# pablode/gatling

Hardware: AMD Instinct MI355X
Metric: Msamples/s (spp x pixels / s) at 8 bounces, 1920x1080 (higher is better)
Workload: dtype f32; 1 GPU; C2: cornell.usda 1920x1080 spp=1024 max-bounces=8 UsdPreviewSurface (diffuse + GGX specular), NEE off; width=1920, height=1080, spp=1024, max_bounces=8, parallelism=single, triangles=46, bvh8_nodes=4

## Files before the change

gatling_amd/build.py:

```python
from __future__ import annotations

import os
import subprocess
from concurrent.futures import ThreadPoolExecutor

_HERE = os.path.dirname(os.path.abspath(__file__))
CSRC = os.path.join(_HERE, "csrc")
OBJDIR = os.path.join(CSRC, "build")
LIB = os.path.join(_HERE, "libgatling_gi.so")
HOST_SOURCES = ["gi_c.cpp", "gi_scene.cpp", "gi_textures.cpp", "gi_lights.cpp", "gi_build.cpp", "gi_render.cpp", "gi_debug.cpp", "gi_denoise_host.cpp"]
SOURCES = HOST_SOURCES + ["gi_image.cpp", "bvh8.cpp", "leaf_lift.cpp", "gi_kernels.hip", "gi_trace.hip", "gi_shade.hip", "gi_aov.hip", "gi_aov2.hip", "gi_path.hip", "gi_bvh_build.hip", "gi_patch.hip", "gi_refit.hip", "gi_tlas.hip", "gi_blas.hip", "gi_append.hip", "gi_instances.hip", "gi_compact.hip", "gi_tlas_build.hip", "gi_tlas_build_host.cpp", "gi_blas_build.hip", "gi_blas_build_host.cpp", "gi_denoise.hip", "gi_moments.hip", "gi_denoise_var.hip", "gtl_shim.cpp"]
HEADERS = ["gi_host.h", "gi_types.h", "gi_kernels.h", "gi_device_math.h", "gi_queues.h", "gi_traversal.h", "gi_texture.h", "gi_shading.h", "gi_stages.h", "gi_image.h", "gi_options.h", "gi_miss_rect.h", "bvh8.h", "gi_bvh_build.h", "gi_refit.h", "gi_tlas.h", "gi_blas.h", "gi_pack.h", "gi_vispatch.h", "gi_aov_body.h", "gi_append.h", "gi_instances.h", "gi_compact.h", "gi_bvh_stages.h", "gi_tlas_build.h", "gi_blas_build.h", "gi_denoise.h", "gi_moments.h",
           os.path.join("..", "..", "include", "gi_c.h"), os.path.join("..", "..", "include", "gtl", "gi", "Gi.h"),
           os.path.join("..", "..", "include", "gtl", "gb", "ParamTypes.h")]
INCLUDE = os.path.join(_HERE, "..", "include")
FLAGS = ["--offload-arch=gfx950", "-O3", "-std=c++17", "-fPIC", "-ffp-contract=off", "-Wall", "-I", INCLUDE]
KERNEL_FLAGS = ["-fno-slp-vectorize"]


def materialx_include():
    roots = [os.environ.get(k) for k in ("MATERIALX_ROOT", "PXR_USD_LOCATION", "USD_ROOT")] + ["/usr", "/usr/local", "/opt/local"]
    for r in roots:
        if r and os.path.exists(os.path.join(r, "include", "MaterialXFormat", "XmlIo.h")):
            return os.path.join(r, "include")
    return None


def _mtime(path: str) -> float:
    return os.path.getmtime(path) if os.path.exists(path) else 0.0


def _headers_mtime() -> float:
    return max([_mtime(os.path.join(CSRC, h)) for h in HEADERS] + [_mtime(os.path.abspath(__file__))])


def _obj(src: str) -> str:
    return os.path.join(OBJDIR, src + ".o")


def _stale(src: str, force: bool) -> bool:
    return force or _mtime(_obj(src)) < max(_mtime(os.path.join(CSRC, src)), _headers_mtime())


def needs_build() -> bool:
    return _mtime(LIB) == 0.0 or any(_stale(s, False) or _mtime(_obj(s)) > _mtime(LIB) for s in SOURCES)


def build(force: bool = False, verbose: bool = False) -> str:
    if not (force or needs_build()):
        return LIB
    hipcc = os.environ.get("HIPCC", "/opt/rocm/bin/hipcc")
    os.makedirs(OBJDIR, exist_ok=True)

    def compile_one(src: str) -> None:
        cmd = [hipcc] + FLAGS + (KERNEL_FLAGS if src.endswith(".hip") else []) + (["-fvisibility=hidden"] if src in HOST_SOURCES else []) + (["-I", mtlx] if mtlx and src == "gtl_shim_mtlx.cpp" else []) + ["-c", src, "-o", _obj(src)]
        if verbose:
            print(" ".join(cmd))
        subprocess.check_call(cmd, cwd=CSRC)

    sources = list(SOURCES)
    mtlx = materialx_include()
    if mtlx:
        sources.append("gtl_shim_mtlx.cpp")
    todo = [s for s in sources if _stale(s, force)]
    with ThreadPoolExecutor(max_workers=min(len(todo), os.cpu_count() or 2) or 1) as pool:
        list(pool.map(compile_one, todo))
    link = [hipcc, "--offload-arch=gfx950", "-shared", "-fPIC", "-o", LIB] + [_obj(s) for s in sources] + ["-lz"]
    if verbose:
        print(" ".join(link))
    subprocess.check_call(link, cwd=CSRC)
    return LIB


if __name__ == "__main__":
    print(build(force=True, verbose=True))
```

gatling_amd/capi.py:

```python
from __future__ import annotations

import ctypes as C
import os

import numpy as np

from .scene import P_COUNT, SceneDesc, RenderSettings

_HERE = os.path.dirname(os.path.abspath(__file__))
LIB_PATH = os.path.join(_HERE, "libgatling_gi.so")
if os.environ.get("GATLING_GI_LIB"):
    LIB_PATH = os.path.abspath(os.environ["GATLING_GI_LIB"])

GI_C_OK = 0
AOV_COLOR = 0
AOV_EXT_MOMENTS = 0x100
FORMAT_INT32, FORMAT_FLOAT32, FORMAT_FLOAT32_VEC4 = 0, 1, 2
OPTION_COUNT_TRAVERSAL, OPTION_KERNEL_TIMERS, OPTION_POOL_SLOTS, OPTION_SAMPLE_BUFFER_MB, OPTION_TRACE_DYNAMIC, OPTION_TWO_LEVEL, OPTION_FUSED_PATH, OPTION_DEVICES = 1, 2, 3, 4, 5, 6, 7, 8
OPTION_SAMPLE_LOOKAHEAD = 10
OPTION_VERTEX_UPDATES = 12
OPTION_VISIBILITY_UPDATES = 11
OPTION_TOPOLOGY_UPDATES = 13
OPTION_RESYNC_REFITS = 14
OPTION_INSTANCE_UPDATES = 15
# ... 86 lines not shown
                ("scale", C.c_float * 4), ("bias", C.c_float * 4)]


class GiCPrimvarData(C.Structure):
    _fields_ = [("name", C.c_char_p), ("type", C.c_int32), ("interpolation", C.c_int32), ("data", C.c_void_p), ("dataSize", C.c_uint64)]



ASSET_OPEN = C.CFUNCTYPE(C.c_void_p, C.c_void_p, C.c_char_p)
ASSET_SIZE = C.CFUNCTYPE(C.c_uint64, C.c_void_p, C.c_void_p)
ASSET_DATA = C.CFUNCTYPE(C.c_void_p, C.c_void_p, C.c_void_p)
ASSET_CLOSE = C.CFUNCTYPE(None, C.c_void_p, C.c_void_p)


class GiCAssetReader(C.Structure):
    _fields_ = [("user", C.c_void_p), ("open", ASSET_OPEN), ("size", ASSET_SIZE), ("data", ASSET_DATA), ("close", ASSET_CLOSE)]


class GiCDecodedImage(C.Structure):
    _fields_ = [("format", C.c_uint32), ("width", C.c_uint32), ("height", C.c_uint32), ("reserved", C.c_uint32), ("pixels", C.c_void_p), ("handle", C.c_void_p)]


IMAGE_LOAD = C.CFUNCTYPE(C.c_int32, C.c_void_p, C.c_char_p, C.c_void_p, C.c_uint64, C.c_int32, C.POINTER(GiCDecodedImage))
IMAGE_RELEASE = C.CFUNCTYPE(None, C.c_void_p, C.POINTER(GiCDecodedImage))
IMAGE_RGBA8_UNORM, IMAGE_RGB16_FLOAT, IMAGE_RGBA16_FLOAT, IMAGE_R32_FLOAT, IMAGE_RGBA32_FLOAT = 1, 2, 3, 4, 5


class GiCImageLoader(C.Structure):
    _fields_ = [("user", C.c_void_p), ("load", IMAGE_LOAD), ("release", IMAGE_RELEASE)]


SYMBOLS = [
    ("giCInitialize", C.c_int, [C.c_int]), ("giCInitializeDevices", C.c_int, [C.POINTER(C.c_int32), C.c_uint32]), ("giCGetDeviceCount", C.c_uint32, []), ("giCGetApiVersion", C.c_uint32, []), ("giCGetDevicePeerAccess", C.c_int32, [C.c_uint32]), ("giCTerminate", None, []), ("giCGetLastError", C.c_char_p, []),
    ("giCCreateMaterial", _P, [_P, C.c_char_p, C.POINTER(GiCMaterialDesc)]), ("giCDestroyMaterial", None, [_P]),
    ("giCCreateMesh", _P, [_P, C.POINTER(GiCMeshDesc)]), ("giCSetMeshTransform", None, [_P, _FP]),
    ("giCSetMeshInstanceTransforms", None, [_P, _U, _FP]), ("giCSetMeshInstanceIds", None, [_P, _U, C.POINTER(C.c_int32)]),
    ("giCSetMeshMaterial", None, [_P, _P]), ("giCSetMeshVisibility", None, [_P, _I]), ("giCSetMeshVertices", C.c_int, [_P, _U, _P]), ("giCDestroyMesh", None, [_P]),
    ("giCRender", C.c_int, [C.POINTER(GiCRenderParams)]),
    ("giCCreateScene", _P, []), ("giCDestroyScene", None, [_P]),
    ("giCCreateSphereLight", _P, [_P]), ("giCDestroySphereLight", None, [_P, _P]), ("giCSetSphereLightPosition", None, [_P, _FP]),
    ("giCSetSphereLightBaseEmission", None, [_P, _FP]), ("giCSetSphereLightRadius", None, [_P, _F, _F, _F]),
    ("giCSetSphereLightDiffuseSpecular", None, [_P, _F, _F]),
    ("giCCreateDistantLight", _P, [_P]), ("giCDestroyDistantLight", None, [_P, _P]), ("giCSetDistantLightDirection", None, [_P, _FP]),
    ("giCSetDistantLightBaseEmission", None, [_P, _FP]), ("giCSetDistantLightAngle", None, [_P, _F]),
    ("giCSetDistantLightDiffuseSpecular", None, [_P, _F, _F]),
    ("giCCreateRectLight", _P, [_P]), ("giCDestroyRectLight", None, [_P, _P]), ("giCSetRectLightOrigin", None, [_P, _FP]),
    ("giCSetRectLightTangents", None, [_P, _FP, _FP]), ("giCSetRectLightBaseEmission", None, [_P, _FP]),
    ("giCSetRectLightDimensions", None, [_P, _F, _F]), ("giCSetRectLightDiffuseSpecular", None, [_P, _F, _F]),
    ("giCCreateDiskLight", _P, [_P]), ("giCDestroyDiskLight", None, [_P, _P]), ("giCSetDiskLightOrigin", None, [_P, _FP]),
    ("giCSetDiskLightTangents", None, [_P, _FP, _FP]), ("giCSetDiskLightBaseEmission", None, [_P, _FP]),
    ("giCSetDiskLightRadius", None, [_P, _F, _F]), ("giCSetDiskLightDiffuseSpecular", None, [_P, _F, _F]),
    ("giCCreateDomeLight", _P, [_P, C.c_char_p]), ("giCDestroyDomeLight", None, [_P]), ("giCSetDomeLightRotation", None, [_P, _FP]),
    ("giCSetDomeLightBaseEmission", None, [_P, _FP]), ("giCSetDomeLightDiffuseSpecular", None, [_P, _F, _F]),
    ("giCSetDomeLightTexture", None, [_P, _P]),
    ("giCCreateTexture", _P, [_P, C.POINTER(GiCTextureDesc)]), ("giCDestroyTexture", None, [_P]),
    ("giCCreateTextureFromFile", _P, [_P, C.c_char_p, _I]),
    ("giCDebugDecodeImage", C.c_int, [C.c_char_p, _I, C.POINTER(C.c_uint32), C.POINTER(C.c_uint32), _FP, C.c_uint64]),
    ("giCRegisterAssetReader", None, [C.POINTER(GiCAssetReader)]), ("giCSetImageLoader", None, [C.POINTER(GiCImageLoader)]),
    ("giCSetMaterialTexture", C.c_int, [_P, _I, C.POINTER(GiCTextureBinding)]),
    ("giCSetMaterialTextureTransform", C.c_int, [_P, _I, _FP]),
    ("giCSetMeshPrimvars", C.c_int, [_P, _U, C.POINTER(GiCPrimvarData)]), ("giCSetMeshInstancerPrimvars", C.c_int, [_P, _U, C.POINTER(GiCPrimvarData)]),
    ("giCSetMaterialPrimvarInput", C.c_int, [_P, _I, C.c_char_p]),
    ("giCCreateRenderBuffer", _P, [_U, _U, _I]), ("giCDestroyRenderBuffer", None, [_P]), ("giCGetRenderBufferMem", _P, [_P]),
    ("giCGetRenderBufferDeviceMem", _P, [_P]), ("giCSetRenderBufferDeviceOnly", None, [_P, _I]),
    ("giCCreateHostRenderBuffer", _P, [_U, _U, _I]),
    ("giCDenoiseVarianceDefaults", None, [C.POINTER(GiCDenoiseVarianceParams)]), ("giCDenoiseVariance", C.c_int, [C.POINTER(GiCDenoiseVarianceParams)]),
    ("giCDenoiseDefaults", None, [C.POINTER(GiCDenoiseParams)]), ("giCDenoise", C.c_int, [C.POINTER(GiCDenoiseParams)]),
    ("giCGetDenoiseStats", C.c_int, [C.POINTER(GiCDenoiseStats)]),
    ("giCGetRenderStats", C.c_int, [_P, C.POINTER(GiCRenderStats)]), ("giCSetSceneOption", C.c_int, [_P, _I, _I]),
    ("giCGetLookaheadStats", C.c_int, [_P, C.POINTER(GiCLookaheadStats)]),
    ("giCTraceRays", C.c_int, [_P, _U, _FP, _FP, _F, _F, _FP, C.POINTER(C.c_int32)]),
    ("giCDebugEvalBsdf", C.c_int, [C.POINTER(GiCMaterialDesc), _U, _FP, _FP]),
    ("giCDebugShadeClass", C.c_int, [C.POINTER(GiCMaterialDesc)]),
    ("giCDebugCheckSqrt", C.c_int64, [C.c_uint32, C.c_uint64]),
    ("giCDebugCheckDiv", C.c_int64, [C.c_uint32, C.c_uint64, C.c_uint32, C.POINTER(C.c_uint32)]),
    ("giCDebugValidateBvh", C.c_int, [_FP, _U, C.POINTER(C.c_uint32), C.POINTER(C.c_uint32)]),
    ("giCDebugValidatePartitionedBvh", C.c_int, [_FP, _U, _U, C.POINTER(C.c_uint32), C.POINTER(C.c_uint32)]),
    ("giCDebugValidateSceneBvh", C.c_int, [_P, _U, C.POINTER(C.c_uint32), C.POINTER(C.c_uint32), C.POINTER(C.c_int32), C.POINTER(C.c_uint64)]),
    ("giCDebugTexRuntime", C.c_int, [_FP, _U, _U, _U, _U, _FP, _FP]),
    ("giCDebugEditDirtyFlags", C.c_int32, [_I, _I]), ("giCDebugSceneUpdateCounts", C.c_int, [_P, C.POINTER(C.c_uint64)]),
    ("giCDebugSceneVisibilityUpdateCount", C.c_int, [_P, C.POINTER(C.c_uint64)]), ("giCDebugSceneClassState", C.c_int, [_P, C.POINTER(C.c_uint32)]),
    ("giCDebugSceneUpsPlain", C.c_int, [_P, C.POINTER(C.c_uint32)]), ("giCDebugUpsTraits", C.c_int, [C.POINTER(GiCMaterialDesc), _U, C.c_int, C.POINTER(C.c_uint32)]),
    ("giCDebugSceneLeafLift", C.c_int, [_P, C.POINTER(C.c_uint32)]),
    ("giCDebugLeafLift", C.c_int, [_FP, _U, C.c_int32, _P, _U, _U, _P, _U, C.POINTER(C.c_uint32), C.POINTER(C.c_uint32), C.POINTER(C.c_double)]),
    ("giCDebugSceneVertexUpdateCount", C.c_int, [_P, C.POINTER(C.c_uint64)]), ("giCDebugRefitBvh", C.c_int, [_FP, _FP, _U, C.POINTER(C.c_uint32), C.POINTER(C.c_uint32)]),
    ("giCDebugSceneRefitCheck", C.c_int, [_P, _U, C.POINTER(C.c_uint32)]),
    ("giCDebugSceneTopologyUpdateCount", C.c_int, [_P, C.POINTER(C.c_uint64)]),
    ("giCDebugSceneResyncCount", C.c_int, [_P, C.POINTER(C.c_uint64)]), ("giCDebugGatherShade", C.c_int, [_P, _U, _P, _U]),
    ("giCDebugSceneShadeCheck", C.c_int, [_P, _U, C.POINTER(C.c_uint32)]),
    ("giCDebugSceneInstanceUpdateCount", C.c_int, [_P, C.POINTER(C.c_uint64)]), ("giCDebugCloneInstance", C.c_int, [_P, _U, _P, _U, _I, _FP, _FP]),
    ("giCDebugSceneTlasUpdateCount", C.c_int, [_P, C.POINTER(C.c_uint64)]), ("giCDebugSceneTlasCheck", C.c_int, [_P, _U, C.POINTER(C.c_uint32)]),
    ("giCDebugInstanceBounds", C.c_int, [_P, _U, _P, _U, _FP, _U, _FP, C.POINTER(C.c_uint32)]),
    ("giCDebugSceneBlasUpdateCount", C.c_int, [_P, C.POINTER(C.c_uint64)]), ("giCDebugSceneBlasCheck", C.c_int, [_P, _U, C.POINTER(C.c_uint32)]),
    ("giCDebugBlasRefit", C.c_int, [_P, _P, _U, _P, _U, C.POINTER(C.c_uint32), C.POINTER(C.c_uint32)]),
    ("giCDebugBlasRefitHost", C.c_int, [_P, _P, _U, _P, _U, C.POINTER(C.c_uint32), C.POINTER(C.c_uint32)]),
    ("giCDebugSceneTlasVisibilityUpdateCount", C.c_int, [_P, C.POINTER(C.c_uint64)]), ("giCDebugSceneFlatIdCheck", C.c_int, [_P, _U, C.POINTER(C.c_uint32)]),
    ("giCDebugSceneFlatTreeState", C.c_int, [_P, _U, C.POINTER(C.c_uint64)]),
    ("giCDebugSceneTlasTopologyUpdateCount", C.c_int, [_P, C.POINTER(C.c_uint64)]),
    ("giCDebugAppendRecords", C.c_int, [_P, _U, _P, _U, _P, _U, _U, _FP, _U, _U, _U, _U, _U]),
    ("giCDebugAppendRecordsHost", C.c_int, [_P, _U, _P, _U, _P, _U, _U, _FP, _U, _U, _U, _U, _U]),
    ("giCDebugInstanceRecords", C.c_int, [_P, _U, _P, _U]),
    ("giCDebugInstanceRecordsHost", C.c_int, [_P, _U, _P, _U]),
    ("giCDebugSceneTlasInstanceUpdateStats", C.c_int, [_P, C.POINTER(C.c_uint64)]),
    ("giCDebugSceneCompactionCount", C.c_int, [_P, C.POINTER(C.c_uint64)]),
    ("giCDebugCompactRanges", C.c_int, [_U, _P, _U, _P, _U, C.POINTER(C.c_uint32)]),
    ("giCDebugCompactRangesHost", C.c_int, [_U, _P, _U, _P, _U, C.POINTER(C.c_uint32)]),
    ("giCDebugBuildTlasHost", C.c_int, [_FP, _U, _U, _U, C.POINTER(C.c_double)]),
    ("giCDebugBuildTlas", C.c_int, [_FP, _U, _U, _U, C.POINTER(C.c_double)]),
    ("giCDebugBuildBlasHost", C.c_int, [_P, _U, _P, _U, _U, _U, C.POINTER(C.c_double)]),
    ("giCDebugBuildBlas", C.c_int, [_P, _U, _P, _U, _U, _U, C.POINTER(C.c_double)]),
    ("giCDebugSceneBlasBuildStats", C.c_int, [_P, C.POINTER(C.c_uint64)]),
    ("giCDebugSceneTlasBuildStats", C.c_int, [_P, C.POINTER(C.c_uint64)]),
    ("giCDebugPatchVisibilityTwoLevel", C.c_int, [C.POINTER(C.c_uint32), C.POINTER(C.c_uint8), C.POINTER(C.c_uint8), _U, _U, C.POINTER(C.c_uint32)]),
    ("giCDebugPathWalkStats", C.c_int, [_P, C.POINTER(C.c_uint64)]),
    ("giCDebugPathLobeStats", C.c_int, [_P, C.POINTER(C.c_uint64)]),
    ("giCDebugPathRingStats", C.c_int, [_P, C.POINTER(C.c_uint64)]),
    ("giCDebugPathLot", C.c_int, [C.c_uint32, C.c_uint32, C.c_uint32, C.POINTER(C.c_uint32)]),
    ("giCDebugTraversalStackHigh", C.c_int, [_P, C.POINTER(C.c_uint32)]),
    ("giCDebugBvhStackReach", C.c_int, [_FP, _U, _FP, _FP, _U, C.POINTER(C.c_uint32)]),
    ("giCDebugSampleMoments", C.c_int, [_P, _FP, _FP, C.POINTER(C.c_uint32), _FP, _FP]),
    ("giCDebugSampleMomentsHost", C.c_int, [_P, _FP, _FP, C.POINTER(C.c_uint32), _FP, _FP]),
    ("giCDebugMissRect", C.c_int, [_FP, C.POINTER(GiCCameraDesc), C.POINTER(GiCRenderSettings), _U, _U, C.POINTER(C.c_uint32)]),
]

_lib = None


def load_library():
    global _lib
    if _lib is None:
        if not os.path.exists(LIB_PATH):
            raise RuntimeError(f"{LIB_PATH} is missing: build it with `python -c 'import __graft_entry__ as g; g.build()'` "
                               "(hipcc --offload-arch=gfx950); there is no CPU fallback")
        L = C.CDLL(LIB_PATH)
        for name, res, args in SYMBOLS:
            fn = getattr(L, name)
            fn.restype = res
            fn.argtypes = args
        _lib = L
    return _lib


def _fp(values):
    arr = (C.c_float * len(values))(*[float(v) for v in values])
    return arr


class GiError(RuntimeError):
    pass


def denoise_params(**params) -> GiCDenoiseParams:
    p = GiCDenoiseParams()
    load_library().giCDenoiseDefaults(C.byref(p))
    for k, v in params.items():
        if k not in ("iterations", "normalSquarings", "sigmaColor", "sigmaDepth", "backgroundDepth", "albedoFloor", "source"):
            raise TypeError(f"denoise: unknown parameter {k!r}")
        setattr(p, k, v)
    return p


def denoise_stats() -> dict:
    s = GiCDenoiseStats()
    if load_library().giCGetDenoiseStats(C.byref(s)) != GI_C_OK:
        raise GiError("giCGetDenoiseStats failed")
    out = {name: getattr(s, name) for name, _ in GiCDenoiseStats._fields_ if name != "passMs"}
# ... 20 lines not shown

def denoise(color, normal, depth, albedo=None, host_form=False, _moments=None, **params):
    L = load_library()
    color = np.ascontiguousarray(color, np.float32)
    h, w = color.shape[:2]
    arrays = {"color": color, "normal": np.ascontiguousarray(normal, np.float32), "depth": np.ascontiguousarray(depth, np.float32)}
    if albedo is not None:
        arrays["albedo"] = np.ascontiguousarray(albedo, np.float32)
    if _moments is not None:
        arrays["moments"] = np.ascontiguousarray(_moments, np.float32)
    create = L.giCCreateHostRenderBuffer if host_form else L.giCCreateRenderBuffer
    bufs = {}
    try:
        for name, a in list(arrays.items()) + [("output", None)]:
            fmt = FORMAT_FLOAT32 if name == "depth" else FORMAT_FLOAT32_VEC4
            if a is not None and a.shape != ((h, w) if name == "depth" else (h, w, 4)):
                raise ValueError(f"denoise: {name} has shape {a.shape}")
            rb = create(w, h, fmt)
            if not rb:
                raise GiError("render buffer creation failed: " + L.giCGetLastError().decode())
            bufs[name] = rb
            if a is not None and a.nbytes:
                C.memmove(L.giCGetRenderBufferMem(rb), a.ctypes.data, a.nbytes)
        source = DENOISE_SOURCE_HOST_FORM if host_form else DENOISE_SOURCE_HOST
        vp = denoise_variance_params(source=source, **params) if _moments is not None else None
        p = vp.base if vp is not None else denoise_params(source=source, **params)
        p.color, p.normal, p.depth, p.albedo, p.output = bufs["color"], bufs["normal"], bufs["depth"], bufs.get("albedo"), bufs["output"]
        if vp is not None:
            vp.moments = bufs["moments"]
            if L.giCDenoiseVariance(C.byref(vp)) != GI_C_OK:
                raise GiError("giCDenoiseVariance failed: " + L.giCGetLastError().decode())
        elif L.giCDenoise(C.byref(p)) != GI_C_OK:
            raise GiError("giCDenoise failed: " + L.giCGetLastError().decode())
        out = np.empty((h, w, 4), np.float32)
        if out.nbytes:
            C.memmove(out.ctypes.data, L.giCGetRenderBufferMem(bufs["output"]), out.nbytes)
        return out
    finally:
        for rb in bufs.values():
            L.giCDestroyRenderBuffer(rb)


def debug_sample_moments(samples, pixel_major, width, rows, first=0, count=None, prev=None, rect=None, miss_rgb=None, host_only=False):
    L = load_library()
    samples = np.ascontiguousarray(samples, np.float32)
    pixels = int(width) * int(rows)
    S = samples.shape[1] if pixel_major else samples.shape[0]
    assert samples.shape == ((pixels, S, 4) if pixel_major else (S, pixels, 4)), samples.shape
    d = (C.c_uint32 * 6)(int(width), int(rows), S, int(first), int(S - first if count is None else count), int(bool(pixel_major)))
    ptr = lambda a: None if a is None else a.ctypes.data_as(_FP)
    prev_a = None if prev is None else np.ascontiguousarray(prev, np.float32).reshape(pixels, 4)
    rect_a = None if rect is None else (C.c_uint32 * 4)(*[int(v) for v in rect])
    miss_a = None if miss_rgb is None else np.ascontiguousarray(miss_rgb, np.float32)
    out = np.empty((pixels, 4), np.float32)
    fn = L.giCDebugSampleMomentsHost if host_only else L.giCDebugSampleMoments
    if fn(d, ptr(samples), ptr(prev_a), rect_a, ptr(miss_a), ptr(out)) != GI_C_OK:
        raise GiError("giCDebugSampleMoments failed: " + L.giCGetLastError().decode())
    return out


def miss_rect(bounds, camera, rs: "RenderSettings", width: int, height: int):
    L = load_library()
    out = (C.c_uint32 * 4)()
    cam, st = _camera(camera), _settings(rs)
    if L.giCDebugMissRect(_fp(bounds), C.byref(cam), C.byref(st), int(width), int(height), out) != GI_C_OK:
        raise GiError("giCDebugMissRect failed: " + L.giCGetLastError().decode())
    return tuple(int(v) for v in out)


def leaf_lift(tri_verts, mode: int = 1, tree_nodes=None, tree_depth: int = 0) -> dict:
    import numpy as np
    L = load_library()
    v = np.ascontiguousarray(tri_verts, np.float32).reshape(-1, 9)
    given = None if tree_nodes is None else np.ascontiguousarray(np.frombuffer(bytes(tree_nodes), np.uint8)).reshape(-1, 80)
    cap = max(len(v), 1) + 1 if given is None else len(given)
    nodes = np.zeros((cap, 80), np.uint8); order = np.zeros(max(len(v), 1), np.uint32); info = np.zeros(4, np.uint32); cost = np.zeros(2, np.float64)
    rc = L.giCDebugLeafLift(v.ctypes.data_as(_FP), len(v), mode, None if given is None else given.ctypes.data_as(_P), 0 if given is None else len(given), tree_depth,
                            nodes.ctypes.data_as(_P), cap, order.ctypes.data_as(C.POINTER(C.c_uint32)), info.ctypes.data_as(C.POINTER(C.c_uint32)),
                            cost.ctypes.data_as(C.POINTER(C.c_double)))
    if rc < 0:
        raise GiError(f"giCDebugLeafLift failed ({rc})")
    return {"violations": rc, "nodes": nodes[:int(info[0])].copy(), "order": order[:len(v)].copy(), "depth": int(info[1]), "lifted": int(info[2]),
            "active": int(info[3]), "cost_before": float(cost[0]), "cost_after": float(cost[1])}


def bvh_stack_reach(tri_verts, origins, dirs):
    import numpy as np
    L = load_library()
    v = np.ascontiguousarray(tri_verts, np.float32).reshape(-1, 9)
    o = np.ascontiguousarray(origins, np.float32).reshape(-1, 3)
    d = np.ascontiguousarray(dirs, np.float32).reshape(-1, 3)
    assert o.shape == d.shape
    out = np.zeros(2 + len(o), np.uint32)
    if L.giCDebugBvhStackReach(v.ctypes.data_as(_FP), len(v), o.ctypes.data_as(_FP), d.ctypes.data_as(_FP), len(o), out.ctypes.data_as(C.POINTER(C.c_uint32))) != 0:
        raise GiError("giCDebugBvhStackReach failed")
    return int(out[0]), int(out[1]), out[2:].copy()


def debug_gather_shade(vertices, faces) -> int:
    from .scene import VERTEX_DTYPE
    L = load_library()
    v = np.ascontiguousarray(vertices, VERTEX_DTYPE)
    f = np.ascontiguousarray(faces, np.uint32).reshape(-1, 3)
    n = L.giCDebugGatherShade(v.ctypes.data, len(v), f.ctypes.data, len(f))
    if n < 0:
        raise GiError("giCDebugGatherShade refused the mesh")
    return int(n)


def debug_clone_instance(vertices, faces, xform_a, xform_b, left_handed=False) -> int:
    from .scene import VERTEX_DTYPE
    L = load_library()
    v = np.ascontiguousarray(vertices, VERTEX_DTYPE)
    f = np.ascontiguousarray(faces, np.uint32).reshape(-1, 3)
    a, b = (np.ascontiguousarray(x, np.float32).reshape(16) for x in (xform_a, xform_b))
    n = L.giCDebugCloneInstance(v.ctypes.data, len(v), f.ctypes.data, len(f), int(bool(left_handed)), a.ctypes.data_as(_FP), b.ctypes.data_as(_FP))
    if n < 0:
        raise GiError("giCDebugCloneInstance refused the mesh or a transform")
    return int(n)


OPTION_BLAS_DEVICE_BUILD = 23
OPTION_TLAS_COMPACTION = 24
OPTION_LEAF_LIFT = 25
TLAS_BUILD_TOO_DEEP = -2


def debug_build_tlas(boxes, depth_budget=7, radius=16, host_only=False) -> dict:
    L = load_library()
    b = np.ascontiguousarray(boxes, np.float32).reshape(-1, 6)
    out = (C.c_double * 8)()
    fn = L.giCDebugBuildTlasHost if host_only else L.giCDebugBuildTlas
    v = fn(b.ctypes.data_as(_FP), len(b), int(depth_budget), int(radius), out)
    if v < 0 and v != TLAS_BUILD_TOO_DEEP:
        raise GiError("giCDebugBuildTlas failed: " + L.giCGetLastError().decode())
    return {"violations": int(v), "nodes": int(out[0]), "depth": int(out[1]), "passes": int(out[2]), "cost": float(out[3]), "host_cost": float(out[4]),
            "host_waits": int(out[5]), "host_depth": int(out[6]), "active": int(out[7])}


def debug_build_blas(vertices, faces, depth_budget=12, radius=16, host_only=False) -> dict:
    from .scene import VERTEX_DTYPE
    L = load_library()
    v = np.ascontiguousarray(vertices, VERTEX_DTYPE)
    f = np.ascontiguousarray(faces, np.uint32).reshape(-1, 3)
    out = (C.c_double * 16)()
    fn = L.giCDebugBuildBlasHost if host_only else L.giCDebugBuildBlas
    r = fn(v.ctypes.data, len(v), f.ctypes.data, len(f), int(depth_budget), int(radius), out)
    if r < 0 and r != TLAS_BUILD_TOO_DEEP:
        raise GiError("giCDebugBuildBlas failed: " + L.giCGetLastError().decode())
    return {"violations": int(r), "nodes": int(out[0]), "depth": int(out[1]), "passes": int(out[2]), "cost": float(out[3]), "host_cost": float(out[4]),
            "host_waits": int(out[5]), "host_depth": int(out[6]), "active": int(out[7]), "conservative": int(out[8]), "rules": int(out[9]), "levels": int(out[10]),
            "bounds_bytes": int(out[11]), "tlas_records": int(out[12]), "refit_bytes": int(out[13]), "budget": int(out[14]), "differing_bytes": int(out[15])}


def debug_instance_bounds(vertices, faces, xforms):
    from .scene import VERTEX_DTYPE
    L = load_library()
    v = np.ascontiguousarray(vertices, VERTEX_DTYPE)
    f = np.ascontiguousarray(faces, np.uint32).reshape(-1, 3)
    x = np.ascontiguousarray(xforms, np.float32).reshape(-1, 16)
    boxes = np.zeros((len(x), 6), np.float32)
    status = np.zeros(len(x), np.uint32)
    n = L.giCDebugInstanceBounds(v.ctypes.data, len(v), f.ctypes.data, len(f), x.ctypes.data_as(_FP), len(x), boxes.ctypes.data_as(_FP),
                                 status.ctypes.data_as(C.POINTER(C.c_uint32)))
    if n < 0:
        raise GiError("giCDebugInstanceBounds failed: " + L.giCGetLastError().decode())
# ... 454 lines not shown
        else:
            m.primvar_inputs.pop(slot, None)
        if self.L.giCSetMaterialPrimvarInput(self.materials[material_index], int(slot), name.encode() if name else None) != GI_C_OK:
            raise GiError("giCSetMaterialPrimvarInput failed: " + self.L.giCGetLastError().decode())

    def _set_primvars(self, fn, h, pvs):
        arr, keep = (GiCPrimvarData * max(len(pvs), 1))(), []
        for k, pv in enumerate(pvs):
            d = np.ascontiguousarray(pv.data, np.int32 if int(pv.type) >= 4 else np.float32).reshape(-1)
            keep.append(d)
            arr[k] = GiCPrimvarData(pv.name.encode(), int(pv.type), int(pv.interpolation), d.ctypes.data, d.nbytes)
        if fn(h, len(pvs), arr) != GI_C_OK:
            raise GiError("giCSetMesh*Primvars failed: " + self.L.giCGetLastError().decode())

    def set_mesh_primvars(self, mesh_index: int, primvars):
        self.desc.meshes[mesh_index].primvars = list(primvars)
        self._set_primvars(self.L.giCSetMeshPrimvars, self.meshes[mesh_index], list(primvars))

    def set_mesh_instancer_primvars(self, mesh_index: int, primvars):
        self.desc.meshes[mesh_index].instancer_primvars = list(primvars)
        self._set_primvars(self.L.giCSetMeshInstancerPrimvars, self.meshes[mesh_index], list(primvars))

    def set_mesh_visibility(self, mesh_index: int, visible: bool):
        self.desc.meshes[mesh_index].visible = bool(visible)
        self.L.giCSetMeshVisibility(self.meshes[mesh_index], int(bool(visible)))

    def set_mesh_vertices(self, mesh_index: int, vertices):
        from .scene import VERTEX_DTYPE
        v = np.ascontiguousarray(vertices, VERTEX_DTYPE)
        if self.L.giCSetMeshVertices(self.meshes[mesh_index], len(v), v.ctypes.data) != GI_C_OK:
            raise GiError("giCSetMeshVertices failed: " + self.L.giCGetLastError().decode())
        self.desc.meshes[mesh_index].vertices = v.copy()

    def vertex_update_count(self) -> int:
        n = C.c_uint64(0)
        if self.L.giCDebugSceneVertexUpdateCount(self.handle, C.byref(n)) != GI_C_OK:
            raise GiError("giCDebugSceneVertexUpdateCount failed")
        return int(n.value)

    def refit_check(self, device: int = 0) -> dict:
        nodes = C.c_uint32(0)
        v = self.L.giCDebugSceneRefitCheck(self.handle, device, C.byref(nodes))
        if v < 0:
            raise GiError("giCDebugSceneRefitCheck failed: " + self.L.giCGetLastError().decode())
        return {"differing": v, "nodes": nodes.value}

    def shade_check(self, device: int = 0) -> int:
        records = C.c_uint32(0)
        v = self.L.giCDebugSceneShadeCheck(self.handle, device, C.byref(records))
        if v < 0:
            raise GiError("giCDebugSceneShadeCheck failed: " + self.L.giCGetLastError().decode())
        return int(v)

    def resync_count(self) -> int:
        n = C.c_uint64(0)
        if self.L.giCDebugSceneResyncCount(self.handle, C.byref(n)) != GI_C_OK:
            raise GiError("giCDebugSceneResyncCount failed")
        return int(n.value)

    def update_counts(self) -> dict:
        c = (C.c_uint64 * 3)()
        if self.L.giCDebugSceneUpdateCounts(self.handle, c) != GI_C_OK:
            raise GiError("giCDebugSceneUpdateCounts failed")
        return {"full": int(c[0]), "transform": int(c[1]), "material": int(c[2])}

    def visibility_update_count(self) -> int:
        n = C.c_uint64(0)
        if self.L.giCDebugSceneVisibilityUpdateCount(self.handle, C.byref(n)) != GI_C_OK:
            raise GiError("giCDebugSceneVisibilityUpdateCount failed")
        return int(n.value)

    def class_state(self) -> dict:
        c = (C.c_uint32 * 5)()
        if self.L.giCDebugSceneClassState(self.handle, c) != GI_C_OK:
            raise GiError("giCDebugSceneClassState failed")
        return {"classMask": int(c[0]), "classTextured": int(c[1]), "shadeClassMask": int(c[2]), "shadeClassTextured": int(c[3]), "hasCutouts": bool(c[4])}

    def ups_plain(self) -> dict:
        c = (C.c_uint32 * 2)()
        if self.L.giCDebugSceneUpsPlain(self.handle, c) != GI_C_OK:
            raise GiError("giCDebugSceneUpsPlain failed")
        return {"traits": int(c[0]), "launched": int(c[1])}

    def leaf_lift(self) -> dict:
        c = (C.c_uint32 * 2)()
        if self.L.giCDebugSceneLeafLift(self.handle, c) != GI_C_OK:
            raise GiError("giCDebugSceneLeafLift failed")
        return {"lifted": int(c[0]), "depth": int(c[1])}

    def path_walk_stats(self) -> dict:
        c = (C.c_uint64 * 18)()
        if self.L.giCDebugPathWalkStats(self.handle, c) != GI_C_OK:
            raise GiError("giCDebugPathWalkStats failed")
        return {"phaseTrips": int(c[0]), "stepTrips": [int(v) for v in c[1:9]], "stepLanes": [int(v) for v in c[9:17]], "fewLaneSteps": int(c[17])}

    def path_lobe_stats(self) -> dict:
        c = (C.c_uint64 * 9)()
        if self.L.giCDebugPathLobeStats(self.handle, c) != GI_C_OK:
            raise GiError("giCDebugPathLobeStats failed")
        keys = ("shaded", "glossy", "glossyTrips", "liteTrips", "fullTrips", "parked", "adopted", "reruns", "rerunHits")
        return {k: int(v) for k, v in zip(keys, c)}

    def path_ring_stats(self) -> dict:
        c = (C.c_uint64 * 5)()
        if self.L.giCDebugPathRingStats(self.handle, c) != GI_C_OK:
            raise GiError("giCDebugPathRingStats failed")
        keys = ("batches", "pairs", "partialBatches", "flushes", "ballotSteps")
        return {k: int(v) for k, v in zip(keys, c)}

    def traversal_stack_high(self) -> dict:
        c = (C.c_uint32 * 4)()
        if self.L.giCDebugTraversalStackHigh(self.handle, c) != GI_C_OK:
            raise GiError("giCDebugTraversalStackHigh failed")
        return {k: int(v) for k, v in zip(("closest", "shadow", "rows", "spill"), c)}

    def set_option(self, option: int, value: int):
        if self.L.giCSetSceneOption(self.handle, option, value) != GI_C_OK:
            raise GiError("giCSetSceneOption failed")

    def color_buffer(self, width, height):
        key = ("color", width, height)
        if key not in self._buffers:
            rb = self.L.giCCreateRenderBuffer(width, height, FORMAT_FLOAT32_VEC4)
            if not rb:
                raise GiError("giCCreateRenderBuffer failed: " + self.L.giCGetLastError().decode())
            self._buffers[key] = rb
        return self._buffers[key]

    def render(self, settings: RenderSettings, width: int, height: int, rows=None, device_only=False, row_stride=1, copy=True):
        L = self.L
        rb = self.color_buffer(width, height)
        L.giCSetRenderBufferDeviceOnly(rb, int(device_only))
        binding = GiCAovBinding()
        binding.aovId = AOV_COLOR
        clear = np.asarray(settings.clear_color, np.float32)
        C.memmove(binding.clearValue, clear.ctypes.data, 16)
        binding.renderBuffer = rb
        p = GiCRenderParams()
        p.aovBindings = C.pointer(binding)
        p.aovBindingCount = 1
        p.camera = _camera(self.desc.camera)
        p.domeLight = self.dome
        p.renderSettings = _settings(settings)
        p.scene = self.handle
        r0, r1 = rows if rows is not None else (0, height)
        p.rowBegin, p.rowEnd, p.rowStride = r0, r1, row_stride
        if L.giCRender(C.byref(p)) != GI_C_OK:
            raise GiError("giCRender failed: " + L.giCGetLastError().decode())
        if device_only:
            return None
        mem = L.giCGetRenderBufferMem(rb)
        full = np.ctypeslib.as_array(C.cast(mem, C.POINTER(C.c_float)), shape=(height, width, 4))
        return full[r0:r1:row_stride].copy() if copy else full[r0:r1:row_stride]

    AOVS = {"normal": (1, FORMAT_FLOAT32_VEC4), "nee": (2, FORMAT_FLOAT32_VEC4), "barycentrics": (3, FORMAT_FLOAT32_VEC4),
            "texcoords": (4, FORMAT_FLOAT32_VEC4), "bounces": (5, FORMAT_FLOAT32_VEC4), "clockCycles": (6, FORMAT_FLOAT32_VEC4), "opacity": (7, FORMAT_FLOAT32_VEC4),
            "tangents": (8, FORMAT_FLOAT32_VEC4), "bitangents": (9, FORMAT_FLOAT32_VEC4), "thinWalled": (10, FORMAT_FLOAT32_VEC4),
            "objectId": (11, FORMAT_INT32), "depth": (12, FORMAT_FLOAT32), "faceId": (13, FORMAT_INT32), "instanceId": (14, FORMAT_INT32),
            "doubleSided": (15, FORMAT_FLOAT32_VEC4), "albedo": (16, FORMAT_FLOAT32_VEC4),
            "moments": (AOV_EXT_MOMENTS, FORMAT_FLOAT32_VEC4)}

    def render_aovs(self, settings: RenderSettings, width: int, height: int, names, clear_values=None, with_color=True, rows=None, row_stride=1):
        L = self.L
        r0, r1 = rows if rows is not None else (0, height)
        bindings = []
        bufs = {}
# ... 163 lines not shown
```

gatling_amd/csrc/gi_debug.cpp:

```cpp
#include "gi_host.h"
#include "gi_refit.h"
#include "gi_tlas_build.h"
#include "gi_blas.h"
#include "gi_blas_build.h"
#include "gi_bvh_stages.h"
#include "gi_compact.h"
#include "gi_moments.h"
#include "bvh8.h"

static int giCTraceRaysImpl(GiCScene* s, uint32_t count, const float* origins, const float* dirs, float tMin, float tMax, float* outTUV, int32_t* outInstPrim);
extern "C" int giCTraceRays(GiCScene* s, uint32_t count, const float* origins, const float* dirs, float tMin, float tMax, float* outTUV, int32_t* outInstPrim)
{
  try { return giCTraceRaysImpl(s, count, origins, dirs, tMin, tMax, outTUV, outInstPrim); }
  catch (const std::exception& e) { setError(std::string("giCTraceRays: ") + e.what()); return -1; }
}
static int giCTraceRaysImpl(GiCScene* s, uint32_t count, const float* origins, const float* dirs, float tMin, float tMax, float* outTUV, int32_t* outInstPrim)
{
  if (!g_ctx.initialized || !s || (count && (!origins || !dirs || !outTUV || !outInstPrim))) { setError("giCTraceRays: bad arguments"); return -1; }
  if (count == 0) return 0;
  std::lock_guard<std::mutex> guard(s->mutex);
  hipStream_t st = g_ctx.stream;
  if (syncSceneGeometry(s) != GI_C_OK) return -1;
  const bool inLds = sceneFitsLds(s->nodeCount, s->triCount);
  const uint32_t blocks = std::min<uint32_t>((count + 255u) / 256u, (uint32_t)g_ctx.cuCount * (inLds ? 3u : 8u));
  if (ensurePathState(s, count, blocks, blocks) != GI_C_OK) return -1;
  const size_t qn = (size_t)s->queueCap * NSHARD;
  std::vector<uint32_t> qslot(qn, 0u); std::vector<F4> qa(qn), qb(qn);
  Counters c{};
  const uint32_t per = (count + NSHARD - 1u) / NSHARD;
  for (uint32_t k = 0; k < NSHARD; k++) { uint32_t lo = k * per; c.count[Q_TRACE_A][k].v = lo < count ? std::min(per, count - lo) : 0u; }
  for (uint32_t i = 0; i < count; i++) {
    size_t r = (size_t)(i / per) * s->queueCap + (i % per);
    qslot[r] = i;
    qa[r] = F4{origins[3 * i], origins[3 * i + 1], origins[3 * i + 2], tMin};
    qb[r] = F4{dirs[3 * i], dirs[3 * i + 1], dirs[3 * i + 2], tMax};
  }
  if (hipMemcpyAsync(s->qSlot[Q_TRACE_A].ptr, qslot.data(), qn * 4, hipMemcpyHostToDevice, st) != hipSuccess ||
      hipMemcpyAsync(s->qA[Q_TRACE_A].ptr, qa.data(), qn * sizeof(F4), hipMemcpyHostToDevice, st) != hipSuccess ||
      hipMemcpyAsync(s->qB[Q_TRACE_A].ptr, qb.data(), qn * sizeof(F4), hipMemcpyHostToDevice, st) != hipSuccess ||
      hipMemcpyAsync(s->dCounters.ptr, &c, sizeof(c), hipMemcpyHostToDevice, st) != hipSuccess) { setError("giCTraceRays: upload failed"); return -1; }
  if (hipMemsetAsync(s->slots.ptr, 0, (size_t)count * sizeof(Slot), st) != hipSuccess) { setError("giCTraceRays: clearing the slots failed"); return -1; }
  PathState ps{s->slots.ptr, nullptr, 0u, nullptr, 0u, nullptr};
  launchTrace(st, blocks, false, false, makeView(s), ps, makeQueueSet(s), s->dCounters.ptr, Q_TRACE_A, Q_REGEN_B, traceDynRefill(s), blocks, FrameUniforms{},
      nullptr);
  std::vector<TriRec> tris(s->triCount);
  if (hipMemcpyAsync(&c, s->dCounters.ptr, sizeof(c), hipMemcpyDeviceToHost, st) != hipSuccess ||
      (s->triCount && hipMemcpyAsync(tris.data(), s->dTris.ptr, s->triCount * sizeof(TriRec), hipMemcpyDeviceToHost, st) != hipSuccess) ||
      hipStreamSynchronize(st) != hipSuccess) { setError("giCTraceRays: readback failed"); return -1; }
  std::vector<F4> hit(count, F4{tMax, 0.0f, 0.0f, 0.0f});
  for (uint32_t i = 0; i < count; i++) { uint32_t m = 0xffffffffu; memcpy(&hit[i].w, &m, 4); }
  std::vector<uint32_t> hitIdx(qn);
  if (hipMemcpy(qa.data(), s->qA[Q_TRACE_A].ptr, qn * sizeof(F4), hipMemcpyDeviceToHost) != hipSuccess) {
    setError("giCTraceRays: readback failed");
    return -1;
  }
  for (uint32_t klass = 0; klass < MAT_CLASS_COUNT; klass++) {
    if (hipMemcpy(hitIdx.data(), s->qSlot[Q_HIT + klass].ptr, qn * 4, hipMemcpyDeviceToHost) != hipSuccess) {
      setError("giCTraceRays: readback failed");
      return -1;
    }
    for (uint32_t k = 0; k < NSHARD; k++)
      for (uint32_t j = 0; j < c.count[Q_HIT + klass][k].v; j++) {
        const uint32_t ri = hitIdx[(size_t)k * s->queueCap + j] & 0x3fffffffu;
        if (ri < qn && qslot[ri] < count) { F4 h = qa[ri]; uint32_t w; memcpy(&w, &h.w, 4); w &= 0x0fffffffu; memcpy(&h.w, &w, 4); hit[qslot[ri]] = h; }
      }
  }
  int hits = 0;
  for (uint32_t i = 0; i < count; i++) {
    uint32_t tri; memcpy(&tri, &hit[i].w, 4);
    outTUV[3 * i] = hit[i].x; outTUV[3 * i + 1] = hit[i].y; outTUV[3 * i + 2] = hit[i].z;
    if (tri == 0xffffffffu || tri >= s->triCount) { outInstPrim[2 * i] = -1; outInstPrim[2 * i + 1] = -1; }
    else { outInstPrim[2 * i] = (int32_t)tris[tri].instance; outInstPrim[2 * i + 1] = (int32_t)tris[tri].prim; hits++; }
  }
  return hits;
}

static int validateTree(const std::vector<Node8>& nodes, const std::vector<TriRec>& trisArr, uint32_t triCount, const std::vector<uint8_t>* left = nullptr)
{
  int violations = 0;
  std::vector<uint8_t> seen(triCount, 0);
  struct Item { uint32_t node; float lo[3], hi[3]; };
  std::vector<Item> stack;
  Item root; root.node = 0; for (int a = 0; a < 3; a++) { root.lo[a] = -3.0e38f; root.hi[a] = 3.0e38f; }
  stack.push_back(root);
  while (!stack.empty()) {
    Item it = stack.back(); stack.pop_back();
    if (it.node >= nodes.size()) { violations++; continue; }
    const Node8& n = nodes[it.node];
    uint32_t rel = 0;
    for (int s = 0; s < 8; s++) {
// ... 384 lines not shown
extern "C" int giCDebugShadeClass(const GiCMaterialDesc* desc)
{
  if (!desc) return -1;
  MaterialRec m{}; m.klass = desc->klass; m.flags = desc->flags & ~(MAT_FLAG_TEXTURED | MAT_FLAG_OPACITY_TEX); memcpy(m.p, desc->p, sizeof(m.p));
  deriveMaterialConstants(m);
  return (int)shadeClassOf(m);
}

extern "C" int giCDebugEvalBsdf(const GiCMaterialDesc* desc, uint32_t count, const float* in, float* out)
{
  if (!g_ctx.initialized || !desc || (count && (!in || !out))) { setError("giCDebugEvalBsdf: bad arguments"); return GI_C_ERROR; }
  if (count == 0) return GI_C_OK;
  MaterialRec m{}; m.klass = desc->klass; m.flags = desc->flags & ~(MAT_FLAG_TEXTURED | MAT_FLAG_OPACITY_TEX); memcpy(m.p, desc->p, sizeof(m.p));
  deriveMaterialConstants(m);
  const uint32_t shadeClass = shadeClassOf(m);
  MaterialRec* dm = nullptr; float* din = nullptr; float* dout = nullptr;
  hipStream_t st = g_ctx.stream;
  int rc = GI_C_ERROR;
  if (hipMalloc((void**)&dm, sizeof(m)) == hipSuccess && hipMalloc((void**)&din, (size_t)count * 22 * 4) == hipSuccess &&
      hipMalloc((void**)&dout, (size_t)count * 15 * 4) == hipSuccess &&
      hipMemcpyAsync(dm, &m, sizeof(m), hipMemcpyHostToDevice, st) == hipSuccess &&
      hipMemcpyAsync(din, in, (size_t)count * 22 * 4, hipMemcpyHostToDevice, st) == hipSuccess) {
    launchDebugBsdf(st, dm, shadeClass, count, din, dout);
    if (hipMemcpyAsync(out, dout, (size_t)count * 15 * 4, hipMemcpyDeviceToHost, st) == hipSuccess && hipStreamSynchronize(st) == hipSuccess) rc = GI_C_OK;
  }
  if (rc != GI_C_OK) setError("giCDebugEvalBsdf: HIP failure");
  if (dm) (void)hipFree(dm); if (din) (void)hipFree(din); if (dout) (void)hipFree(dout);
  return rc;
}

extern "C" int giCDebugTexRuntime(const float* rgba, uint32_t width, uint32_t height, uint32_t depth, uint32_t count, const float* queries, float* out)
{
  if (!g_ctx.initialized || !rgba || !width || !height || !depth || (count && (!queries || !out))) { setError("giCDebugTexRuntime: bad arguments");
      return GI_C_ERROR; }
  if (count == 0) return GI_C_OK;
  const size_t texFloats = (size_t)width * height * depth * 4;
  float* dt = nullptr; float* dq = nullptr; float* dout = nullptr;
  hipStream_t st = g_ctx.stream;
  int rc = GI_C_ERROR;
  if (hipMalloc((void**)&dt, texFloats * 4) == hipSuccess && hipMalloc((void**)&dq, (size_t)count * 32) == hipSuccess
      && hipMalloc((void**)&dout, (size_t)count * 16) == hipSuccess &&
      hipMemcpyAsync(dt, rgba, texFloats * 4, hipMemcpyHostToDevice, st) == hipSuccess
          && hipMemcpyAsync(dq, queries, (size_t)count * 32, hipMemcpyHostToDevice, st) == hipSuccess) {
    launchDebugTex(st, dt, width, height, depth, count, dq, dout);
    if (hipMemcpyAsync(out, dout, (size_t)count * 16, hipMemcpyDeviceToHost, st) == hipSuccess && hipStreamSynchronize(st) == hipSuccess) rc = GI_C_OK;
  }
  if (rc != GI_C_OK) setError("giCDebugTexRuntime: HIP failure");
  if (dt) (void)hipFree(dt); if (dq) (void)hipFree(dq); if (dout) (void)hipFree(dout);
  return rc;
}


extern "C" int64_t giCDebugCheckSqrt(uint32_t first, uint64_t count)
{
  if (!g_ctx.initialized) { setError("giCDebugCheckSqrt before giCInitialize"); return -1; }
  unsigned long long* d = nullptr; unsigned long long h = 0ull;
  if (hipMalloc(&d, sizeof(h)) != hipSuccess) { setError("giCDebugCheckSqrt: hipMalloc failed"); return -1; }
  bool ok = hipMemsetAsync(d, 0, sizeof(h), g_ctx.stream) == hipSuccess;
  if (ok) { launchDebugSqrt(g_ctx.stream, first, (unsigned long long)count, d); ok = hipMemcpyAsync(&h, d, sizeof(h), hipMemcpyDeviceToHost, g_ctx.stream) == hipSuccess; }
  ok = ok && hipStreamSynchronize(g_ctx.stream) == hipSuccess;
  (void)hipFree(d);
  if (!ok) { setError("giCDebugCheckSqrt: device error"); return -1; }
  return (int64_t)h;
}

extern "C" int64_t giCDebugCheckDiv(uint32_t mode, uint64_t count, uint32_t seed, const uint32_t* words)
{
  if (!g_ctx.initialized) { setError("giCDebugCheckDiv before giCInitialize"); return -1; }
  const bool given = mode == 0u || mode == 2u;
  if (mode > 4u || (given && (!words || count > (1ull << 28)))) { setError("giCDebugCheckDiv: bad arguments"); return -1; }
  const size_t bytes = given ? (size_t)count * (mode == 0u ? 2u : 4u) * sizeof(uint32_t) : 0u;
  unsigned long long* d = nullptr; unsigned long long h = 0ull; uint32_t* dw = nullptr;
  if (hipMalloc(&d, sizeof(h)) != hipSuccess) { setError("giCDebugCheckDiv: hipMalloc failed"); return -1; }
  bool ok = bytes == 0u || hipMalloc(&dw, bytes) == hipSuccess;
  ok = ok && (bytes == 0u || hipMemcpyAsync(dw, words, bytes, hipMemcpyHostToDevice, g_ctx.stream) == hipSuccess);
  ok = ok && hipMemsetAsync(d, 0, sizeof(h), g_ctx.stream) == hipSuccess;
  if (ok) { launchDebugDiv(g_ctx.stream, mode, (unsigned long long)count, seed, dw, d); ok = hipMemcpyAsync(&h, d, sizeof(h), hipMemcpyDeviceToHost, g_ctx.stream) == hipSuccess; }
  ok = ok && hipStreamSynchronize(g_ctx.stream) == hipSuccess;
  (void)hipFree(d); if (dw) (void)hipFree(dw);
  if (!ok) { setError("giCDebugCheckDiv: device error"); return -1; }
  return (int64_t)h;
}

extern "C" int32_t giCDebugEditDirtyFlags(int32_t edit, int32_t built)
{
  std::unique_ptr<GiCScene> scene(new GiCScene());
  GiCScene* s = scene.get();
  const float texel[4] = {1.0f, 1.0f, 1.0f, 1.0f};
  GiCTextureDesc td{1u, 1u, texel};
  GiCMaterialDesc md{}; md.klass = GI_C_MAT_USD_PREVIEW_SURFACE;
  GiCVertex verts[3] = {}; verts[1].pos[0] = 1.0f; verts[2].pos[1] = 1.0f;
  GiCFace face{}; face.v_i[0] = 0; face.v_i[1] = 1; face.v_i[2] = 2;
  GiCMeshDesc meshDesc{}; meshDesc.faceCount = 1; meshDesc.faces = &face; meshDesc.vertexCount = 3; meshDesc.vertices = verts; meshDesc.name = "debug";
  const float identity[16] = {1, 0, 0, 0, 0, 1, 0, 0, 0, 0, 1, 0, 0, 0, 0, 1};
  GiCTexture* tex = giCCreateTexture(s, &td);
  GiCMaterial* matA = giCCreateMaterial(s, "a", &md);
  GiCMaterial* matB = giCCreateMaterial(s, "b", &md);
  GiCMesh* mesh = giCCreateMesh(s, &meshDesc);
  if (!tex || !matA || !matB || !mesh) return -1;
  giCSetMeshInstanceTransforms(mesh, 1, identity);
  giCSetMeshMaterial(mesh, matA);
  if (built) { s->host.reset(new SceneHost()); mesh->builtInstances = 1; }
  s->dirty = 0;
  GiCMaterial* made = nullptr; GiCTexture* madeTex = nullptr; GiCMesh* madeMesh = nullptr;
  GiCTextureBinding binding{}; binding.texture = tex; for (int i = 0; i < 4; i++) binding.scale[i] = 1.0f;
  const float xf[6] = {1, 0, 0, 0, 1, 0};
  const float one = 1.0f; const int32_t id = 7;
  GiCPrimvarData pv{}; pv.name = "k"; pv.type = GI_C_PRIMVAR_FLOAT; pv.interpolation = GI_C_INTERP_CONSTANT; pv.data = &one; pv.dataSize = 4;
  int32_t result = 0;
  switch (edit) {
    case 0: made = giCCreateMaterial(s, "c", &md); break;
    case 1: giCDestroyMaterial(matB); matB = nullptr; break;
    case 2: giCSetMeshMaterial(mesh, matB); break;
    case 3: giCSetMaterialPrimvarInput(matA, GI_C_TEX_BASE_COLOR, "k"); break;
    case 4: giCSetMaterialTexture(matA, GI_C_TEX_BASE_COLOR, &binding); break;
    case 5: giCSetMaterialTextureTransform(matA, GI_C_TEX_BASE_COLOR, xf); break;
    case 6: madeTex = giCCreateTexture(s, &td); break;
    case 7: giCDestroyTexture(tex); tex = nullptr; break;
    case 8: giCSetMeshPrimvars(mesh, 1, &pv); break;
    case 9: giCSetMeshInstancerPrimvars(mesh, 1, &pv); break;
    case 10: giCSetMeshTransform(mesh, identity); break;
    case 11: giCSetMeshVisibility(mesh, 0); break;
    case 12: giCSetMeshInstanceIds(mesh, 1, &id); break;
    case 13: madeMesh = giCCreateMesh(s, &meshDesc); break;
    case 14: giCDestroyMesh(mesh); mesh = nullptr; break;
    case 15: giCSetMeshInstanceTransforms(mesh, 0, nullptr); break;
    case 16: if (giCSetMeshVertices(mesh, 3, verts) != GI_C_OK) result = -1; break;
    default: result = -1; break;
  }
  if (result == 0) result = (int32_t)s->dirty;
  if (madeMesh) giCDestroyMesh(madeMesh);
  if (mesh) giCDestroyMesh(mesh);
  if (made) giCDestroyMaterial(made);
  if (matA) giCDestroyMaterial(matA);
  if (matB) giCDestroyMaterial(matB);
  if (madeTex) giCDestroyTexture(madeTex);
  if (tex) giCDestroyTexture(tex);
  return result;
}

extern "C" int giCDebugSceneUpdateCounts(const GiCScene* scene, uint64_t* outCounts)
{
  GiCScene* s = const_cast<GiCScene*>(scene);
  if (!s || !outCounts) { setError("giCDebugSceneUpdateCounts: bad arguments"); return GI_C_ERROR; }
  std::lock_guard<std::mutex> guard(s->mutex);
  outCounts[0] = s->updateCounts[UPDATE_FULL]; outCounts[1] = s->updateCounts[UPDATE_TRANSFORM]; outCounts[2] = s->updateCounts[UPDATE_MATERIAL];
  return GI_C_OK;
}

extern "C" int giCDebugSceneVisibilityUpdateCount(const GiCScene* scene, uint64_t* outCount)
{
  GiCScene* s = const_cast<GiCScene*>(scene);
  if (!s || !outCount) { setError("giCDebugSceneVisibilityUpdateCount: bad arguments"); return GI_C_ERROR; }
  std::lock_guard<std::mutex> guard(s->mutex);
  *outCount = s->updateCounts[UPDATE_VISIBILITY];
  return GI_C_OK;
}

extern "C" int giCDebugSceneVertexUpdateCount(const GiCScene* scene, uint64_t* outCount)
{
  GiCScene* s = const_cast<GiCScene*>(scene);
  if (!s || !outCount) { setError("giCDebugSceneVertexUpdateCount: bad arguments"); return GI_C_ERROR; }
  std::lock_guard<std::mutex> guard(s->mutex);
  *outCount = s->updateCounts[UPDATE_VERTEX];
  return GI_C_OK;
}
// ... 577 lines not shown
```

gatling_amd/csrc/gi_host.h:

```cpp

#pragma once

#pragma GCC visibility push(default)
#include "../../include/gi_c.h"
#pragma GCC visibility pop


#include <algorithm>
#include <atomic>
#include <chrono>
#include <cmath>
#include <cstdio>
#include <cstdlib>
#include <cstring>
#include <memory>
#include <condition_variable>
#include <functional>
#include <mutex>
#include <string>
#include <thread>
#include <vector>

#include "bvh8.h"
#include "gi_tlas_build.h"
// ... 217 lines not shown
  Counters* hCounters = nullptr;
  uint64_t memTotalMb = 0;
  static constexpr uint32_t POLL_RING = 4, POLL_LAG = 2;
  PaddedCounter* hPoll = nullptr; hipEvent_t pollEvent[POLL_RING] = {};
  hipEvent_t evShade = nullptr, evShadow = nullptr;
  GiCRenderStats stats{};
  uint64_t pathWalkStats[18] = {};
  uint64_t pathLobeStats[9] = {};
  uint64_t pathRingStats[5] = {};
  uint32_t traversalStackHigh[4] = {};
  std::vector<hipEvent_t> eventPool;
  template <typename Fn> void forEachPathBuffer(Fn&& fn)
  {
    fn(slots); fn(media); fn(sampleBuf);
    for (uint32_t q = 0; q < Q_COUNT; q++) { fn(qSlot[q]); fn(qA[q]); fn(qB[q]); fn(qC[q]); }
    fn(qFresh[0]); fn(qFresh[1]);
  }
  uint64_t pathStateBytes() { uint64_t n = 0; forEachPathBuffer([&](auto& b) { n += b.bytes(); }); return n; }
  void releasePathState() { forEachPathBuffer([](auto& b) { b.release(); }); queueCap = 0; lookahead.drop(); }
  void releaseAll();
};

struct TwoLevelHost { std::vector<Node8> tlasNodes, blasNodes; std::vector<uint32_t> tlasItems; std::vector<BlasTri> blasTris; std::vector<InstTrav> instTrav;
    std::vector<float> instBoxes; std::vector<uint32_t> meshBlasTri; uint32_t tlasDepth = 0, blasDepth = 0;
    std::vector<uint32_t> meshBlasNode; std::vector<std::vector<uint32_t>> meshBlasLevels;
    bool tlasDeviceBuilt = false; uint32_t tlasBuildBudget = 0;
    std::vector<uint32_t> meshBlasBudget; };
struct MeshBuild { const GiCMesh* m; uint32_t vertexOffset, matFlags, instFirst, instCount, triFirst; uint32_t meshIdx; std::vector<int32_t> faceIdAov;
    uint32_t shadeBase = 0;
    std::vector<uint32_t> inst; uint32_t retiredInst = 0;
    struct FreeSlot { uint32_t inst, tri; };
    std::vector<uint32_t> instTri; std::vector<FreeSlot> freeSlots;
    void numberInstances() { inst.resize(instCount); instTri.resize(instCount);
        for (uint32_t ii = 0; ii < instCount; ii++) { inst[ii] = instFirst + ii; instTri[ii] = triFirst + ii * (uint32_t)m->faces.size(); } }
    bool hidden = false; uint32_t idBase = 0; };
struct InstPart { uint32_t meshBuild, instInMesh; uint32_t triFirst, nf; uint32_t nodeOff, nodeCount, nodeCap, depth; float box[6];
    uint32_t activeTris = 0; std::vector<uint32_t> levelStart;
    bool retired = false; };
struct SceneHost {
  std::vector<FVertex> verts; std::vector<InstanceRec> instances; std::vector<MaterialRec> mats; std::vector<MeshRec> meshRecs; std::vector<float> sceneData;
  Bvh8 bvh; std::vector<int32_t> triFaceId; std::vector<uint32_t> flatOfOrig; TwoLevelHost two;
  std::vector<MeshBuild> meshBuilds;
  std::vector<F4> triGeomNormal;
  std::vector<TriShade> triShade; bool shadePacked = false;
  bool partitioned = false; std::vector<InstPart> parts; uint32_t topCap = 0;
  bool deviceBuilt = false;
  bool hostTreeDropped = false;
  bool reordered = false;
  bool treeless = false;
};

enum : uint32_t { UPDATE_FULL = 0, UPDATE_TRANSFORM = 1, UPDATE_MATERIAL = 2, UPDATE_VISIBILITY = 3, UPDATE_VERTEX = 4, UPDATE_TOPOLOGY = 5, UPDATE_TLAS = 6, UPDATE_BLAS = 7, UPDATE_TLAS_VISIBILITY = 8, UPDATE_TLAS_TOPOLOGY = 9 };
struct GiCScene : SceneDevice {
  std::mutex mutex;
  uint32_t dirty = DIRTY_ALL;
  std::vector<GiCMesh*> meshes;
  std::vector<GiCMaterial*> materials;
  std::vector<GiCTexture*> textures;
  uint64_t nextTextureSerial = 1;
  DenseStore<SphereLightRec, GiCSphereLight> sphereLights;
  DenseStore<DistantLightRec, GiCDistantLight> distantLights;
  DenseStore<RectLightRec, GiCRectLight> rectLights;
  DenseStore<DiskLightRec, GiCDiskLight> diskLights;
  uint32_t lightCounts[4] = {0, 0, 0, 0};
  uint32_t sampleOffset = 0;
  uint64_t accumEpoch = 0;
  bool haveOldParams = false;
  GiCCameraDesc oldCamera{};
  GiCRenderSettings oldSettings{};
  uint8_t oldClear[GI_C_MAX_AOV_COMP_SIZE] = {0};
  uint32_t oldRowBegin = 0, oldRowEnd = 0, oldRowStride = 1;
  GiCDomeLight* oldDome = nullptr;
  float oldDomeEmission[3] = {0, 0, 0};
  uint32_t nodeCount = 0, triCount = 0, bvhDepth = 0;
  float bounds[6] = {0, 0, 0, 0, 0, 0}; bool boundsValid = false;
  int optBvhBuild = 0;
  bool twoLevel = false; int optTwoLevel = -1;
  bool hasCutouts = false;
  bool shadePacked = false;
  uint32_t classMask = 0;
  uint32_t classTextured = 0;
  uint32_t shadeClassMask = 0, shadeClassTextured = 0;
  uint32_t upsTraits = 0, upsPlainLaunched = 0;
  std::unique_ptr<SceneHost> host;
  std::vector<std::unique_ptr<SceneDevice>> replicas;
  bool countTraversal = false, kernelTimers = false;
  uint32_t kernelTimerStride = 1;
  uint64_t optPoolSlots = 0, optSampleBufferMb = 0;
  int32_t optFusedPath = -1;
  int32_t optTraceDyn = -1;
  std::atomic<int32_t> shadowOrder{-1};
       uint64_t shadowOrderRays[2] = {0, 0},
      shadowOrderSteps[2] = {0, 0};
  int32_t optDevices = 0;
  uint32_t lastRenderDevices = 0;
  int32_t optLookahead = 0;
  uint64_t generation = 0;
  uint64_t updateCounts[10] = {0, 0, 0, 0, 0, 0, 0, 0, 0, 0};
  int32_t optVisibilityUpdates = 0;
  int32_t optVertexUpdates = 0;
  bool rebuildDue = true;
  int32_t optTopologyUpdates = 0;
  bool topologyDue = false;
  int32_t optResyncRefits = 0; uint64_t resyncCount = 0;
  int32_t optInstanceUpdates = 0; uint64_t instanceCounts[4] = {0, 0, 0, 0};
  bool instancesDue = false;
  int32_t optTlasUpdates = 0;
  int32_t optBlasUpdates = 0;
  int32_t optTlasVisibility = 0;
  int32_t optTlasOnly = 0;
  int32_t optTlasTopology = 0;
  int32_t optTlasInstances = 0; uint64_t tlasInstanceCounts[4] = {0, 0, 0, 0};
  int32_t optTlasDeviceBuild = 0; uint64_t tlasBuildStats[16] = {};
  int32_t optBlasDeviceBuild = 0; uint64_t blasBuildStats[16] = {};
  int32_t optTlasCompaction = 0; uint64_t compactionStats[4] = {0, 0, 0, 0};
  int32_t optLeafLift = -1; uint32_t liftedLeafSlots = 0;
  std::vector<GiCMesh*> retiredMeshes;
  ~GiCScene() { for (GiCMesh* m : retiredMeshes) delete m; }
};
inline void raiseRebuild(GiCScene* s) { s->dirty |= DIRTY_BVH | DIRTY_FRAMEBUFFER; s->rebuildDue = true; }
inline void raiseTopology(GiCScene* s) { s->dirty |= DIRTY_BVH | DIRTY_FRAMEBUFFER; s->topologyDue = true; }
inline void raiseInstances(GiCMesh* m) { m->instEdited = true; m->scene->dirty |= DIRTY_BVH | DIRTY_FRAMEBUFFER; m->scene->instancesDue = true; }


extern "C++" bool loadImage(const char* path, bool srgbToLinear, bool keepHdr, uint32_t& w, uint32_t& h, std::vector<float>& px);
int uploadLights(GiCScene* s);
uint32_t shadeClassOf(const MaterialRec& m);
uint32_t upsTraitsOf(const MaterialRec& m);
uint32_t sceneDeviceCount(const GiCScene* s);
SceneDevice& sceneDevice(GiCScene* s, uint32_t slot);
bool usableVertexPositions(const GiCVertex* v, size_t count);
void nodeBounds(const Node8& n, float box[6]);
bool instanceUpdatesWanted(const GiCScene* s);
bool tlasUpdatesWanted(const GiCScene* s);
bool blasUpdatesWanted(const GiCScene* s);
bool leafLiftWanted(const GiCScene* s);
bool tlasOnlyWanted(const GiCScene* s);
bool tlasVisibilityWanted(const GiCScene* s);
bool topologyUpdatesWanted(const GiCScene* s);
bool tlasTopologyWanted(const GiCScene* s);
bool tlasDeviceBuildWanted(const GiCScene* s);
bool blasDeviceBuildWanted(const GiCScene* s);
void buildMeshBlas(const GiCVertex* vertices, const GiCFace* faces, size_t nf, Bvh8& b, std::vector<uint32_t>& order, float mlo[3], float mhi[3]);
BlasTri makeBlasTri(const GiCVertex* vertices, const GiCFace* faces, uint32_t f);
bool tlasCompactionWanted(const GiCScene* s);
bool tlasInstancesWanted(const GiCScene* s);
int syncSceneGeometry(GiCScene* s);
inline uint32_t materialEditFlags(bool built) { return DIRTY_MATERIALS | DIRTY_FRAMEBUFFER | (built ? 0u : (uint32_t)DIRTY_BVH); }
SceneView makeView(GiCScene* s, SceneDevice& D);
SceneView makeView(GiCScene* s);
uint32_t traceDynRefill(const GiCScene* s);
int ensurePathState(SceneDevice* s, size_t slots, uint32_t gridA, uint32_t gridB);
QueueSet makeQueueSet(SceneDevice* s);
```

gatling_amd/csrc/gi_kernels.h:

```cpp
#pragma once

#include <type_traits>
#include <hip/hip_runtime.h>

#include "gi_types.h"
#include "gi_vispatch.h"

namespace gi {

template <class F>
auto dispatchBools(F&& f) { return f(); }
template <class F, class... Bools>
auto dispatchBools(F&& f, bool b, Bools... rest)
{
  return b ? dispatchBools([&](auto... cs) { return f(std::true_type{}, cs...); }, rest...)
           : dispatchBools([&](auto... cs) { return f(std::false_type{}, cs...); }, rest...);
}

void launchInit(hipStream_t s, const PathState& st, const QueueSet& qs, Counters* cnt, uint32_t n, bool resetStats);
void launchRaygen(hipStream_t s, uint32_t blocks, const FrameUniforms& U, const PathState& st, const QueueSet& qs, Counters* cnt, uint32_t par, F4* sampleBuf);
void launchAccumulate(hipStream_t s, const FrameUniforms& U, const F4* sampleBuf, F4* accum, F4* colorOut, bool firstBatch, bool lastBatch);
void launchFoldWindow(hipStream_t s, const FrameUniforms& U, const F4* sampleBuf, F4* colorOut, uint32_t windowSamples, uint32_t first, bool pixelMajor);
bool traceBlockSync(const SceneView& sc);
bool sceneFitsLds(size_t nodeCount, size_t triCount);
uint32_t traceLdsBytes(uint32_t stackEntries, uint32_t ldsNodes, uint32_t ldsTris);
uint32_t blocksPerCuByLds(uint32_t dynamicBytes, uint32_t staticBytes);
uint32_t traceStaticLdsBytes();
void traceLdsLayout(const SceneView& sc, uint32_t& ldsNodes, uint32_t& ldsTris, uint32_t& bytes);
uint32_t traceStackRows(const SceneView& sc, bool& spills);
void launchTrace(hipStream_t s, uint32_t blocks, bool anyHit, bool count, const SceneView& sc, const PathState& st, const QueueSet& qs, Counters* cnt,
                 uint32_t qIn, uint32_t qMiss, uint32_t dynRefill, uint32_t routeBlocks, const FrameUniforms& U, F4* sampleBuf);
void launchRoute(hipStream_t s, uint32_t blocks, const SceneView& sc, const PathState& st, const QueueSet& qs, Counters* cnt, uint32_t qIn, uint32_t qMiss,
    const FrameUniforms& U,
                 F4* sampleBuf);
constexpr uint32_t APPEND_ITEMS_MAX = 4u;
constexpr uint32_t TRACE_DYN_SLOT_ORDER = 0x200u;
void launchShade(hipStream_t s, uint32_t blocks, uint32_t klass, bool textured ,
    bool volume , const FrameUniforms& U, const SceneView& sc, const PathState& st, const QueueSet& qs, Counters* cnt, uint32_t par);

bool pathKernelSupports(const SceneView& sc);
int launchPath(hipStream_t s, uint32_t cuCount, uint32_t classMask, bool textured, bool count, uint32_t chunk, uint32_t walkCarry, uint32_t lobePark,
               uint32_t ringCarry, uint32_t upsTraits, const FrameUniforms& U, const SceneView& sc, const PathState& st, Counters* cnt, F4* sampleBuf);
inline uint32_t pathUpsVariant(uint32_t classMask, bool textured, bool nee, bool cutout, bool count, uint32_t upsTraits)
{
  return (classMask == 2u && !textured && !cutout && !count && !nee) ? upsTraits : 0u;
}
constexpr long UPS_PLAIN_DEFAULT = 1;
constexpr long WALK_CARRY_DEFAULT = 8;
constexpr long LOBE_PARK_DEFAULT = 8;
constexpr long RING_CARRY_DEFAULT = 1;
constexpr long LEAF_LIFT_DEFAULT = 1;
struct PathLot { uint32_t stack, row, capacity; };
inline PathLot pathLotPlacement(uint32_t bvhDepth)
{
  const uint32_t stack = bvhDepth <= 4u ? 4u : 8u;
  const uint32_t row = bvhDepth < stack ? bvhDepth : stack;
  return PathLot{stack, row, (stack - row) * 8u};
}

void launchAov(hipStream_t s, const FrameUniforms& U, const SceneView& sc, const AovTargets& A);
void launchAov2(hipStream_t s, const FrameUniforms& U, const SceneView& sc, const AovTargets& A);
void launchResolveNee(hipStream_t s, const FrameUniforms& U, const unsigned long long* key, F4* aov, uint32_t pixelCount);
void launchZeroClosest(hipStream_t s, Counters* cnt, uint32_t par);
void launchPatchMatFlags(hipStream_t s, TriRec* tris, uint32_t triCount, const InstanceRec* instances, uint32_t instanceCount, const uint32_t* wordOfMesh,
    uint32_t meshCount);
void launchPatchVisibility(hipStream_t s, TriRec* tris, uint32_t triCount, const InstanceRec* instances, uint32_t instanceCount, const VisPatch* patchOfInstance,
    const TriShade* triShade, uint32_t shadeCount);
void launchPatchVisibility2(hipStream_t s, TriRec* tris, uint32_t triCount, const InstanceRec* instances, uint32_t instanceCount, const VisPatch* patchOfInstance,
    const TriShade* triShade, uint32_t shadeCount, uint32_t* flatOfOrig, uint32_t flatCount);
void launchPatchInstTrav(hipStream_t s, InstTrav* instTrav, uint32_t instanceCount, const VisPatch* patchOfInstance);
void launchPlacePart(hipStream_t s, const Node8* partNodes, uint32_t partNodeCount, Node8* nodes, uint32_t nodeOff, TriRec* tris, uint32_t triFirst, uint32_t nf,
    uint32_t idAdd);
struct CloneEntry { uint32_t threadBase, srcTri, dstTri, nf, srcNode, dstNode, nodeCount, instance, idBase; };
inline uint32_t cloneEntryThreads(uint32_t nf, uint32_t nodeCount) { return ((nf > nodeCount ? nf : nodeCount) + 63u) & ~63u; }
void launchCloneParts(hipStream_t s, const CloneEntry* entries, uint32_t entryCount, uint32_t threads, TriRec* tris, uint32_t triCount, int32_t* triFaceId,
    Node8* nodes, uint32_t nodeCount, const InstanceRec* instances, uint32_t instanceCount, const TriShade* triShade, uint32_t shadeCount);
struct RefitRange { uint32_t threadBase, nodeFirst; };
void launchRefitTris(hipStream_t s, TriRec* tris, uint32_t triCount, const InstanceRec* instances, uint32_t instanceCount, const uint32_t* editedOfInstance,
    const TriShade* triShade, uint32_t shadeCount);
bool gatherShadeRangeOk(uint32_t shadeCount, uint32_t first, uint32_t count);
bool launchGatherShade(hipStream_t s, TriShade* triShade, uint32_t shadeCount, uint32_t first, uint32_t count, const FVertex* verts, uint32_t vertCount);
void launchRefitLevel(hipStream_t s, Node8* nodes, uint32_t nodeCount, float* boxes, const RefitRange* ranges, uint32_t rangeCount, uint32_t threads,
    const TriRec* tris, uint32_t triCount, const InstanceRec* instances, uint32_t instanceCount, const TriShade* triShade, uint32_t shadeCount);
struct InstBoundsJob { float o2w[12]; uint32_t firstTri, faceCount, instance, pad; };
constexpr uint32_t kInstBoundsChunk = 4096u;
uint32_t instBoundsChunks(uint32_t faceCount);
bool launchInstBounds(hipStream_t s, const InstBoundsJob* jobs, uint32_t jobCount, uint32_t chunksPerJob, const BlasTri* blasTris, uint32_t blasTriCount,
    float* partials, uint32_t* out);
bool blasTrisRangeOk(uint32_t blasTriCount, uint32_t first, uint32_t count, uint32_t shadeCount, uint32_t shadeBase);
bool launchBlasTris(hipStream_t s, BlasTri* blasTris, uint32_t blasTriCount, uint32_t first, uint32_t count, const TriShade* triShade, uint32_t shadeCount,
    uint32_t shadeBase);
void launchBlasRefitLevel(hipStream_t s, Node8* nodes, uint32_t nodeCount, float* boxes, const RefitRange* ranges, uint32_t rangeCount, uint32_t threads,
    const BlasTri* blasTris, uint32_t blasTriCount);
struct AppendMesh;
bool launchAppendShadeIndex(hipStream_t s, TriShade* triShade, uint32_t shadeCount, uint32_t shadeBase, const uint32_t* faces3, uint32_t faceCount,
    uint32_t vertexOffset);
bool launchAppendBlasTris(hipStream_t s, BlasTri* blasTris, uint32_t blasTriCount, uint32_t first, const uint32_t* order, uint32_t faceCount,
    const TriShade* triShade, uint32_t shadeCount, uint32_t shadeBase);
bool launchAppendRecords(hipStream_t s, const AppendMesh& M, TriRec* tris, int32_t* triFaceId, uint32_t* flatOfOrig, const InstanceRec* instances,
    const TriShade* triShade, const int32_t* faceIdOfFace);
struct InstanceJob; struct InstanceJobSizes;
bool launchInstanceRecords(hipStream_t s, const InstanceJob* hostJobs, const InstanceJob* deviceJobs, const InstanceJobSizes& Z, TriRec* tris, int32_t* triFaceId,
    uint32_t* flatOfOrig, const InstanceRec* instances, const TriShade* triShade, const int32_t* faceIdTable);
struct CompactRange; struct CompactSizes;
bool launchCompactRanges(hipStream_t s, const CompactRange* hostRanges, const CompactRange* deviceRanges, const CompactSizes& Z, const void* src, void* dst,
    uint32_t* table);
void launchSpin(hipStream_t s, unsigned long long ns);
void launchDebugBsdf(hipStream_t s, const MaterialRec* mat, uint32_t shadeClass, uint32_t count, const float* in, float* out);
void launchDebugSqrt(hipStream_t s, uint32_t first, unsigned long long count, unsigned long long* mismatches);
void launchDebugDiv(hipStream_t s, uint32_t mode, unsigned long long count, uint32_t seed, const uint32_t* words, unsigned long long* mismatches);
void launchDebugTex(hipStream_t s, const float* texels, uint32_t w, uint32_t h, uint32_t d, uint32_t count, const float* queries, float* out);

}
```

gatling_amd/csrc/gi_path.hip:

```cpp

#include <hip/hip_runtime.h>
#include <cassert>

#define GI_LEAN_MATH 1
#include "gi_device_math.h"
#include "gi_kernels.h"
#include "gi_types.h"
#include "gi_queues.h"
#include "gi_traversal.h"
#include "gi_shading.h"
#include "gi_stages.h"

namespace gi {

constexpr uint32_t PRE_FIELDS = 10;
constexpr uint32_t PATH_STACK_MAX = 8;

constexpr int PATH_WAVES = 4;
template <uint32_t KLASS, bool TEXTURED, bool NEE, bool CUTOUT, bool COUNT, uint32_t PATH_STACK, uint32_t UPS = 0u>
__global__ __launch_bounds__(TRACE_BLOCK) __attribute__((amdgpu_waves_per_eu(PATH_WAVES, 8))) void k_path(FrameUniforms U, SceneView sc, PathState st,
    Counters* cnt, F4* __restrict__ sampleBuf, uint32_t ldsNodes, uint32_t ldsTris, uint32_t chunk, uint32_t walkCarry, uint32_t lobePark, uint32_t lotRow,
    uint32_t lotCap, uint32_t ringCarry)
{
  constexpr bool CARRY = !NEE;
  constexpr bool PARK = !NEE && (KLASS == 1u || (KLASS == KLASS_DYNAMIC && COUNT));
  constexpr bool DEFER = PARK || COUNT;
  const StagedScene S = stage_scene<PATH_STACK>(sc, ldsNodes, ldsTris);
  __shared__ WaveTri s_wave[TRACE_BLOCK / 64];
  WaveTri& W = s_wave[threadIdx.x >> 6];

  const uint32_t lane = __lane_id();
  const unsigned long long below = (1ull << lane) - 1ull;
  V3 thr = v3(0.0f, 0.0f, 0.0f), rad = thr, ro = thr, rdv = v3(0.0f, 0.0f, 1.0f);
  float tMin = 0.0f, tMax = 0.0f;
  uint32_t bitfield = 0u, rng = 0u, rec = 0u;
  bool alive = false, tAlive = false;
  uint32_t chunkNext = 0u, chunkEnd = 0u; bool exhausted = false;
  uint32_t nSeg = 0u, nShadow = 0u;
  WalkCounters<COUNT> tc{}, tcs{};
  uint2 overflow[1];
  RayTrav R; R.G = make_uint2(0u, 0u); R.sp = 0u;
  __shared__ uint32_t s_pre[TRACE_BLOCK / 64][PRE_FIELDS][128];
  GI_LDS uint32_t (*pre)[128] = (GI_LDS uint32_t (*)[128])&s_pre[threadIdx.x >> 6][0][0];
  uint32_t preHead = 0u, preTail = 0u;
  const bool boundsRetire = (U.flags & FLAG_BOUNDS_RETIRE) != 0u;

  unsigned long long pc[4] = {0ull, 0ull, 0ull, 0ull}, pl[4] = {0ull, 0ull, 0ull, 0ull}, trips = 0ull, tPrev = COUNT ? __builtin_readcyclecounter() : 0ull;
  uint32_t whLanes[8] = {0u, 0u, 0u, 0u, 0u, 0u, 0u, 0u}, whTrips[8] = {0u, 0u, 0u, 0u, 0u, 0u, 0u, 0u};
  uint32_t whFew = 0u;
  uint32_t lobeN[9] = {0u, 0u, 0u, 0u, 0u, 0u, 0u, 0u, 0u};
  RingStats ringN{0u, 0u, 0u, 0u, 0u};
  const uint32_t lotFit = (PATH_STACK - (lotRow < PATH_STACK ? lotRow : PATH_STACK)) * 8u;
  const uint32_t lotMax = PARK ? (lotCap < lotFit ? lotCap : lotFit) : 0u;
  const uint32_t parkAt = PARK ? (lobePark < lotMax ? lobePark : lotMax) : 0u;
  uint32_t lotCount = 0u;
  auto lot_record = [&](uint32_t k) __attribute__((always_inline)) {
    return (volatile GI_LDS gi_u4*)(GI_LDS gi_u4*)&S.stack[lotRow + (k >> 3)][(threadIdx.x & ~63u) + ((k & 7u) << 3)];
  };
  auto phase = [&](int k,
      unsigned long long lanes) { if (COUNT) { const unsigned long long t = __builtin_readcyclecounter(); pc[k] += t - tPrev; tPrev = t; pl[k] += lanes; } };
  for (;;) {
    __atomic_signal_fence(__ATOMIC_SEQ_CST);
    unsigned long long idle = __ballot(!alive);
    const uint32_t nIdle = (uint32_t)__popcll(idle);
    if (nIdle) {
      while (preTail - preHead < 64u && !exhausted) {
        if (chunkNext == chunkEnd) {
          uint32_t b = 0u;
          if (lane == 0u) b = atomicAdd(&cnt->cursor[0][0].v, chunk);
          b = (uint32_t)__shfl((int)b, 0);
          if (b >= U.workTotal) { exhausted = true; break; }
          chunkNext = b; chunkEnd = (U.workTotal - b) < chunk ? U.workTotal : b + chunk;
        }
        const uint32_t avail = chunkEnd - chunkNext, take = avail < 64u ? avail : 64u;
        uint32_t nKept = 0u;
        if (lane < take) {
          const uint32_t w = chunkNext + lane;
          const uint32_t sl = w / U.activeCount, a = w - sl * U.activeCount;
          const uint32_t ar = a / U.activeWidth, row = U.rectTy0 + ar, px = U.rectX0 + (a - ar * U.activeWidth);
          const uint32_t rec = sl * U.pixelCount + (row * U.imageWidth + px);
          const uint32_t py = U.rowBegin + row * U.rowStride;
          V3 o, d; float t0, t1; uint32_t r;
          make_camera_ray_at(U, px, py, py * U.imageWidth + px, U.sampleOffset + U.batchFirstSample + sl, o, d, t0, t1, r);
          float lo[3] = {U.sceneLo[0], U.sceneLo[1], U.sceneLo[2]}, hi[3] = {U.sceneHi[0], U.sceneHi[1], U.sceneHi[2]};
          asm volatile("" : "+s"(lo[0]), "+s"(lo[1]), "+s"(lo[2]), "+s"(hi[0]), "+s"(hi[1]), "+s"(hi[2]));
          const bool keep = !(boundsRetire && ray_misses_box(lo, hi, o, d, t0, t1));
          const unsigned long long kept = __ballot(keep);
          nKept = (uint32_t)__popcll(kept);
          if (keep) {
            const uint32_t slot = (preTail + (uint32_t)__popcll(kept & below)) & 127u;
            pre[0][slot] = f2u(o.x); pre[1][slot] = f2u(o.y); pre[2][slot] = f2u(o.z); pre[3][slot] = f2u(d.x); pre[4][slot] = f2u(d.y); pre[5][slot] = f2u(d.z);
            pre[6][slot] = f2u(t0); pre[7][slot] = f2u(t1); pre[8][slot] = r; pre[9][slot] = rec;
          } else {
            float bg[3] = {U.background[0], U.background[1], U.background[2]}, maxv = U.maxSampleValue;
            asm volatile("" : "+s"(bg[0]), "+s"(bg[1]), "+s"(bg[2]), "+s"(maxv));
            V3 c = v3(0.0f, 0.0f, 0.0f) + v3(1.0f, 1.0f, 1.0f) * v3(bg[0], bg[1], bg[2]);
            const float mv = fmax2(c.x, fmax2(c.y, c.z));
            if (mv > maxv) c = c * (maxv / mv);
            st4(&sampleBuf[rec], fmax2(0.0f, c.x), fmax2(0.0f, c.y), fmax2(0.0f, c.z), 0.0f);
            nSeg++;
          }
        }
        chunkNext += take; preTail += (uint32_t)__builtin_amdgcn_readfirstlane((int)nKept);
      }
      __atomic_signal_fence(__ATOMIC_SEQ_CST);
      const uint32_t have = preTail - preHead, take = nIdle < have ? nIdle : have;
      const uint32_t rank = (uint32_t)__popcll(idle & below);
      if (!alive && rank < take) {
        const uint32_t slot = (preHead + rank) & 127u;
        ro = v3(u2f(pre[0][slot]), u2f(pre[1][slot]), u2f(pre[2][slot])); rdv = v3(u2f(pre[3][slot]), u2f(pre[4][slot]), u2f(pre[5][slot]));
        tMin = u2f(pre[6][slot]); tMax = u2f(pre[7][slot]); rng = pre[8][slot];
        rec = pre[9][slot];
        thr = v3(1.0f, 1.0f, 1.0f); rad = v3(0.0f, 0.0f, 0.0f); bitfield = 0u;
        alive = true;
      }
      preHead += take;
    }
    if (!__ballot(alive) && (!PARK || lotCount == 0u)) break;
    phase(0, nIdle); trips++;

    {
      const bool carried = CARRY && tAlive;
      const uint2 G = R.G; const uint32_t sp = R.sp;
      trav_init(R, ro, rdv, tMin, alive ? tMax : 0.0f);
      if (carried) { R.G = G; R.sp = sp; R.tBest = u2f(wt_best_t(W, lane)); }
      else wave_ray_begin(W, R.tBest);
    }
    tAlive = alive;
    if (CARRY) {
      unsigned long long walking = __ballot(tAlive);
      const uint32_t stop = (uint32_t)__popcll(walking) > walkCarry ? walkCarry : 0u;
      uint32_t step = 0u;
      uint32_t pend = 0u;
      if ((uint32_t)__popcll(walking) > stop) for (;;) {
        if (COUNT) {
          const uint32_t n = (uint32_t)__popcll(walking);
          whLanes[step] += n; whTrips[step]++; step = step < 7u ? step + 1u : 7u;
          if (n < 8u) whFew++;
        }
        if (wave_step_ring<COUNT, PATH_STACK, STAGED_ALL, CUTOUT>(R, tAlive, W, sc, S, overflow, tc, rng, pend, ringN)) tAlive = false;
        walking = __ballot(tAlive);
        const bool last = (uint32_t)__popcll(walking) <= stop;
        if ((last || ringCarry == 0u) && pend != 0u) {
          if (COUNT && ringCarry != 0u) ringN.flushes++;
          wave_ring_batch<COUNT, STAGED_ALL, CUTOUT>(W, pend, pend, R, rng, sc, S, tc, ringN);
        }
        __atomic_signal_fence(__ATOMIC_SEQ_CST);
        if (alive) wave_ring_refresh(R, W);
        if (last) break;
      }
    } else {
      while (__ballot(tAlive)) {
        if (wave_step<false, COUNT, PATH_STACK, false, STAGED_ALL, CUTOUT>(R, tAlive, W, sc, S, overflow, tc, rng)) tAlive = false;
      }
    }
    const bool walked = CARRY ? alive && !tAlive : alive;
    bool ended = false;
    ShadeIO io; io.shadow = false; io.shadowFirst = false; io.cont = false;
    if (DEFER) { io.lite = false; io.glossyLobe = false; io.deferred = false; }
    phase(1, (unsigned long long)__popcll(__ballot(walked)));
    auto finish_path = [&]() __attribute__((always_inline)) {
      const uint32_t bounces = bitfield & 0x00000fffu;
      if (st.bouncesAov && U.batchFirstSample + rec / U.pixelCount == U.spp - 1u) {
        const uint32_t maxB = U.maxBounces < 0x00000fffu ? U.maxBounces : 0x00000fffu;
        const V3 c = gi_colormap_inferno((float)bounces / (float)maxB);
        F4* dst = &st.bouncesAov[tile_to_image_pixel(U, rec % U.pixelCount)];
        dst->x = c.x; dst->y = c.y; dst->z = c.z;
      }
      if (st.pathSegments) atomicAdd(&st.pathSegments[rec % U.pixelCount], bounces);
      const V3 c = finish_sample(U, rad);
      st4(&sampleBuf[rec], c.x, c.y, c.z, 0.0f);
      alive = false;
    };
    bool shaded = false;
    uint32_t nEarly = 0u;
    if (walked) {
      nSeg++;
      wave_ray_end(W, R);
      if (R.found) {
        if constexpr (!PARK) {
          io.throughput = thr; io.radiance = rad; io.bitfield = bitfield; io.rng = rng;
          const F4 h = F4{R.tBest, R.bestU, R.bestV, u2f(R.bestTri)}, rd = F4{rdv.x, rdv.y, rdv.z, 0.0f};
          shade_segment<KLASS, TEXTURED, false, NEE, false, DEFER, UPS>(U, sc, nullptr, h, rd, io);
          thr = io.throughput; rad = io.radiance; bitfield = io.bitfield; rng = io.rng;
          if (NEE && st.neeKey && io.shadowFirst && !io.shadow) nee_aov_record_px(st, rec % U.pixelCount, rec / U.pixelCount, false);
          ended = !io.cont;
          shaded = true;
        }
      } else {
        rad = rad + thr * v3(U.background);
        if (st.neeKey && (bitfield & 0x00000fffu) == 0u) nee_aov_record_px(st, rec % U.pixelCount, rec / U.pixelCount, false);
        bitfield++;
        ended = true;
      }
    }
    if constexpr (PARK) {
      bool hit = walked && R.found;
      auto shade_hit = [&]() __attribute__((always_inline)) {
        io.throughput = thr; io.radiance = rad; io.bitfield = bitfield; io.rng = rng;
        const F4 h = F4{R.tBest, R.bestU, R.bestV, u2f(R.bestTri)}, rd = F4{rdv.x, rdv.y, rdv.z, 0.0f};
        shade_segment<KLASS, TEXTURED, false, NEE, false, DEFER, UPS>(U, sc, nullptr, h, rd, io);
        if (io.deferred) return;
        thr = io.throughput; rad = io.radiance; bitfield = io.bitfield; rng = io.rng;
        ended = !io.cont;
        shaded = true;
        if (!ended) { ro = io.no; rdv = io.k2; tMin = 0.0f; tMax = io.tMaxNext; }
      };
      bool lite = lotCount < parkAt && !(exhausted && preTail == preHead) && __ballot(hit) != 0ull;
      if (COUNT && parkAt) lobeN[lite ? 3 : 4]++;
      for (;;) {
        if (!lite && lotCount) {
          nEarly += (uint32_t)__popcll(__ballot(ended));
          if (ended) { finish_path(); ended = false; }
          const unsigned long long freeLanes = __ballot(!alive);
          const uint32_t nFree = (uint32_t)__popcll(freeLanes), nAdopt = nFree < lotCount ? nFree : lotCount;
          const uint32_t rank = (uint32_t)__popcll(freeLanes & below);
          __atomic_signal_fence(__ATOMIC_SEQ_CST);
          if (!alive && rank < nAdopt) {
            volatile GI_LDS gi_u4* p = lot_record(lotCount - nAdopt + rank);
            const gi_u4 a = p[0], b = p[1], c = p[2], d = p[3];
            thr = v3(u2f(a.x), u2f(a.y), u2f(a.z)); bitfield = a.w; rad = v3(u2f(b.x), u2f(b.y), u2f(b.z)); rng = b.w;
            rdv = v3(u2f(c.x), u2f(c.y), u2f(c.z)); rec = c.w; R.tBest = u2f(d.x); R.bestU = u2f(d.y); R.bestV = u2f(d.z); R.bestTri = d.w;
            alive = true; hit = true;
// ... 23 lines not shown
        if (COUNT) { lobeN[7]++; lobeN[8] += nDeferred; }
      }
    }
    if (COUNT) {
      const unsigned long long glossy = __ballot(shaded && io.glossyLobe);
      lobeN[0] += (uint32_t)__popcll(__ballot(shaded)); lobeN[1] += (uint32_t)__popcll(glossy); lobeN[2] += glossy ? 1u : 0u;
    }
    phase(2, (unsigned long long)__popcll(__ballot(PARK ? shaded : walked && R.found)));

    if (NEE) {
      bool sAlive = alive && io.shadow;
      if (__ballot(sAlive)) {
        trav_init(R, io.no, io.sdir, 0.01f, sAlive ? io.ld : 0.0f);
        wave_ray_begin(W, R.tBest);
        const bool traced = sAlive;
        while (__ballot(sAlive)) {
          if (wave_step<true, COUNT, PATH_STACK, false, STAGED_ALL, CUTOUT>(R, sAlive, W, sc, S, overflow, tcs, io.rngShadow)) sAlive = false;
        }
        if (traced) {
          nShadow++;
          if (!R.found) rad = rad + io.nee;
          if (st.neeKey && io.shadowFirst) nee_aov_record_px(st, rec % U.pixelCount, rec / U.pixelCount, R.found);
        }
      }
    }

    if constexpr (PARK) { if (ended) finish_path(); }
    else if (walked) {
      if (!ended) { ro = io.no; rdv = io.k2; tMin = 0.0f; tMax = io.tMaxNext; }
      else {
        const uint32_t bounces = bitfield & 0x00000fffu;
        if (st.bouncesAov && U.batchFirstSample + rec / U.pixelCount == U.spp - 1u) {
          const uint32_t maxB = U.maxBounces < 0x00000fffu ? U.maxBounces : 0x00000fffu;
          const V3 c = gi_colormap_inferno((float)bounces / (float)maxB);
          F4* dst = &st.bouncesAov[tile_to_image_pixel(U, rec % U.pixelCount)];
          dst->x = c.x; dst->y = c.y; dst->z = c.z;
        }
        if (st.pathSegments) atomicAdd(&st.pathSegments[rec % U.pixelCount], bounces);
        const V3 c = finish_sample(U, rad);
        st4(&sampleBuf[rec], c.x, c.y, c.z, 0.0f);
        alive = false;
      }
    }
    phase(3, (unsigned long long)__popcll(__ballot(ended)) + nEarly);
  }

  if (COUNT
      && lane == 0u) { for (int k = 0; k < 4; k++) { atomicAdd(&cnt->phaseCycles[k], pc[k]); atomicAdd(&cnt->phaseLanes[k], pl[k]);
      } atomicAdd(&cnt->phaseTrips, trips);
      for (int k = 0; k < 8; k++) { atomicAdd(&cnt->walkStepLanes[k], (unsigned long long)whLanes[k]); atomicAdd(&cnt->walkStepTrips[k], (unsigned long long)whTrips[k]); }
      atomicAdd(&cnt->walkFewLaneSteps, (unsigned long long)whFew);
      for (int k = 0; k < 9; k++) atomicAdd(&cnt->lobeStats[k], (unsigned long long)lobeN[k]);
      if (CARRY) { atomicAdd(&cnt->ringStats[0], (unsigned long long)ringN.batches); atomicAdd(&cnt->ringStats[1], (unsigned long long)ringN.pairs);
        atomicAdd(&cnt->ringStats[2], (unsigned long long)ringN.partial); atomicAdd(&cnt->ringStats[3], (unsigned long long)ringN.flushes);
        atomicAdd(&cnt->ringStats[4], (unsigned long long)ringN.ballotSteps); } }
  unsigned long long a = nSeg, b = nShadow, c = tc.nodes, d = tc.tris, e = tcs.nodes, f = tcs.tris;
  for (int off = 32; off > 0; off >>= 1) {
    a += __shfl_down(a, off); b += __shfl_down(b, off);
    if (COUNT) { c += __shfl_down(c, off); d += __shfl_down(d, off); e += __shfl_down(e, off); f += __shfl_down(f, off); }
  }
  if (lane == 0u) {
    atomicAdd(&cnt->segments, a);
    if (NEE) atomicAdd(&cnt->shadowRays, b);
    if (COUNT) { atomicAdd(&cnt->nodesVisited, c); atomicAdd(&cnt->trisTested, d); atomicAdd(&cnt->shadowNodesVisited, e); atomicAdd(&cnt->shadowTrisTested, f);
        }
  }
  if constexpr (COUNT) {
    uint32_t hc = tc.high, hs = tcs.high;
    for (int off = 32; off > 0; off >>= 1) {
      const uint32_t oc = (uint32_t)__shfl_down((int)hc, off), os = (uint32_t)__shfl_down((int)hs, off);
      hc = oc > hc ? oc : hc; hs = os > hs ? os : hs;
    }
    if (lane == 0u) { atomicMax(&cnt->stackHigh[0], hc); if (NEE) atomicMax(&cnt->stackHigh[1], hs); }
  }
}

bool pathKernelSupports(const SceneView& sc)
{
  return sc.triCount > 0u && sceneFitsLds(sc.nodeCount, sc.triCount) && sc.bvhDepth <= PATH_STACK_MAX && sc.mediumStackSize == 0u
      && sc.domeTexture == 0u && !sc.twoLevel
         && !sc.shadePacked;
}

using PathKernel = void (*)(FrameUniforms, SceneView, PathState, Counters*, F4*, uint32_t, uint32_t, uint32_t, uint32_t, uint32_t, uint32_t, uint32_t, uint32_t);
template <uint32_t STACK>
static PathKernel pickPathKernel(uint32_t classMask, bool textured, bool nee, bool cutout, bool count, uint32_t upsTraits)
{
  const bool hot = (classMask == 1u || classMask == 2u || classMask == 4u) && !textured && !cutout && !count;
  const uint32_t ups = pathUpsVariant(classMask, textured, nee, cutout, count, upsTraits);
  return dispatchBools([&](auto neeC) -> PathKernel {
    constexpr bool NEE = decltype(neeC)::value;
    if (hot) {
      if (classMask == 1u) return k_path<0u, false, NEE, false, false, STACK>;
      if constexpr (!NEE) {
        if (ups == UPS_NOCOAT) return k_path<1u, false, false, false, false, STACK, UPS_NOCOAT>;
      }
      if (classMask == 2u) return k_path<1u, false, NEE, false, false, STACK>;
      return k_path<2u, false, NEE, false, false, STACK>;
    }
    return dispatchBools([](auto countC) -> PathKernel { return k_path<KLASS_DYNAMIC, true, NEE, true, decltype(countC)::value, STACK>; }, count);
  }, nee);
}

int launchPath(hipStream_t s, uint32_t cuCount, uint32_t classMask, bool textured, bool count, uint32_t chunk, uint32_t walkCarry, uint32_t lobePark,
               uint32_t ringCarry, uint32_t upsTraits, const FrameUniforms& U, const SceneView& sc, const PathState& st, Counters* cnt, F4* sampleBuf)
{
  if (U.workTotal == 0u) return 0;
  const uint32_t ldsNodes = sc.nodeCount, ldsTris = sc.triCount;
  const PathLot lot = pathLotPlacement(sc.bvhDepth);
  const uint32_t stack = lot.stack;
  assert(sc.bvhDepth <= stack && lot.row >= sc.bvhDepth && lot.row + (lot.capacity + 7u) / 8u <= stack);
  const uint32_t bytes = traceLdsBytes(stack, ldsNodes, ldsTris);
  const bool neeOn = (U.flags & FLAG_NEE) != 0u;
  PathKernel k = stack == 4u
      ? pickPathKernel<4u>(classMask, textured, neeOn, sc.hasCutouts != 0u, count, upsTraits)
      : pickPathKernel<8u>(classMask, textured, neeOn, sc.hasCutouts != 0u, count, upsTraits);
  int perCu = 2;
  hipFuncAttributes fa{};
  if (hipFuncGetAttributes(&fa, reinterpret_cast<const void*>(k)) == hipSuccess && fa.numRegs > 0) {
    const uint32_t regs = ((uint32_t)fa.numRegs + 7u) & ~7u, byRegs = 512u / regs;
    const uint32_t byLds = blocksPerCuByLds(bytes, (uint32_t)fa.sharedSizeBytes);
    perCu = (int)(byRegs < byLds ? byRegs : byLds);
    if (perCu > 8) perCu = 8;
    if (perCu < 1) perCu = 1;
  }
  const uint64_t chunks = ((uint64_t)U.workTotal + chunk - 1u) / chunk;
  uint64_t blocks = (uint64_t)cuCount * (uint64_t)perCu;
  const uint64_t needed = (chunks + (TRACE_BLOCK / 64u) - 1u) / (TRACE_BLOCK / 64u);
  if (blocks > needed) blocks = needed;
  if (blocks == 0u) blocks = 1u;
  hipLaunchKernelGGL(k, dim3((uint32_t)blocks), dim3(TRACE_BLOCK), bytes, s, U, sc, st, cnt, sampleBuf, ldsNodes, ldsTris, chunk, walkCarry, lobePark, lot.row, lot.capacity, ringCarry);
  return perCu;
}

__global__ void k_debug_sqrt(uint32_t first, unsigned long long count, unsigned long long* mismatches)
{
  unsigned long long bad = 0ull;
  for (unsigned long long i = blockIdx.x * (unsigned long long)blockDim.x + threadIdx.x; i < count; i += (unsigned long long)gridDim.x * blockDim.x) {
    const float x = u2f(first + (uint32_t)i);
    const float a = gi_sqrt(x), b = sqrtf(x);
    if (f2u(a) != f2u(b) && !(a != a && b != b)) bad++;
  }
  if (bad) atomicAdd(mismatches, bad);
}

void launchDebugSqrt(hipStream_t s, uint32_t first, unsigned long long count, unsigned long long* mismatches)
{
  hipLaunchKernelGGL(k_debug_sqrt, dim3(4096), dim3(256), 0, s, first, count, mismatches);
}

__device__ __forceinline__ bool debug_same(float a, float b) { return f2u(a) == f2u(b) || (a != a && b != b); }
__device__ __forceinline__ bool debug_same(V3 a, V3 b) { return debug_same(a.x, b.x) && debug_same(a.y, b.y) && debug_same(a.z, b.z); }
__global__ void k_debug_div(uint32_t mode, unsigned long long count, uint32_t seed, const uint32_t* __restrict__ words, unsigned long long* mismatches)
{
  unsigned long long bad = 0ull;
  for (unsigned long long i = blockIdx.x * (unsigned long long)blockDim.x + threadIdx.x; i < count; i += (unsigned long long)gridDim.x * blockDim.x) {
    uint32_t w[4];
    if (mode == 4u) { w[0] = w[1] = w[2] = w[3] = 0u; }
    else if (mode == 0u) { w[0] = words[2ull * i]; w[1] = words[2ull * i + 1ull]; w[2] = w[3] = 0u; }
    else if (mode == 2u) { for (int k = 0; k < 4; k++) w[k] = words[4ull * i + k]; }
    else {
      for (uint32_t k = 0; k < 4u; k++) w[k] = gi_hash_init(gi_hash_init(seed + k) ^ (uint32_t)i) + gi_hash_init((uint32_t)(i >> 32) + 0x9e3779b9u * (k + 1u));
      if (mode == 3u && (w[3] & 3u)) {
        const uint32_t sel = gi_hash_init(w[0] ^ w[3]);
        for (uint32_t k = 0; k < 4u; k++) {
          const uint32_t e = 103u + ((w[k] >> 23) & 0xffu) % 49u;
          w[k] = (w[k] & 0x807fffffu) | (e << 23);
          const uint32_t c = (sel >> (8u * k)) & 0xffu;
          if ((c & 7u) == 0u) w[k] &= (c & 8u) ? 0x80000000u : 0x807fffffu;
        }
      }
    }
    bool same;
    if (mode == 4u) {
      const float d = u2f(seed + (uint32_t)i), q = 1.0f / d, rs = 1.0f / sqrtf(d);
      same = debug_same(gi_rcp<true>(d), q) && debug_same(gi_rcp<false>(d), q) && debug_same(gi_rsqrt<true>(d), rs) && debug_same(gi_rsqrt<false>(d), rs);
    } else if (mode < 2u) {
      const float n = u2f(w[0]), d = u2f(w[1]), q = n / d, rq = 1.0f / d;
      same = debug_same(gi_div<true>(n, d), q) && debug_same(gi_div<false>(n, d), q) && debug_same(gi_rcp<true>(d), rq) && debug_same(gi_rcp<false>(d), rq);
    } else {
      const V3 a = v3(u2f(w[0]), u2f(w[1]), u2f(w[2])); const float s = u2f(w[3]);
      const V3 nrm = a * (1.0f / sqrtf(dot(a, a))), quo = V3{a.x / s, a.y / s, a.z / s};
      same = debug_same(normalize<true>(a), nrm) && debug_same(normalize<false>(a), nrm) && debug_same(gi_div3<true>(a, s), quo) && debug_same(gi_div3<false>(a, s), quo);
    }
    if (!same) bad++;
  }
  if (bad) atomicAdd(mismatches, bad);
}

void launchDebugDiv(hipStream_t s, uint32_t mode, unsigned long long count, uint32_t seed, const uint32_t* words, unsigned long long* mismatches)
{
  hipLaunchKernelGGL(k_debug_div, dim3(4096), dim3(256), 0, s, mode, count, seed, words, mismatches);
}

}
```

gatling_amd/csrc/gi_render.cpp:

```cpp
#include "gi_host.h"
#include "gi_miss_rect.h"
#include "gi_moments.h"

bool settingsEqual(const GiCRenderSettings& a, const GiCRenderSettings& b) { return memcmp(&a, &b, sizeof(a)) == 0; }

SceneView makeView(GiCScene* s, SceneDevice& D)
{
  SceneView v{};
  v.textures = D.dTextures.ptr; v.meshes = D.dMeshes.ptr; v.sceneData = D.dSceneData.ptr;
  v.nodes = D.dNodes.ptr; v.tris = D.dTris.ptr; v.instances = D.dInstances.ptr;
  v.verts = D.dVerts.ptr; v.triShade = D.dTriShade.ptr; v.triGeomNormal = D.dTriGeomNormal.ptr; v.shadePacked = s->shadePacked ? 1u : 0u;
      v.materials = D.dMaterials.ptr;
      v.sphereLights = D.dSphere.ptr; v.distantLights = D.dDistant.ptr;
  v.tlasNodes = D.dTlasNodes.ptr; v.tlasItems = D.dTlasItems.ptr; v.blasNodes = D.dBlasNodes.ptr; v.blasTris = D.dBlasTris.ptr; v.instTrav = D.dInstTrav.ptr;
      v.flatOfOrig = D.dFlatOfOrig.ptr; v.twoLevel = s->twoLevel ? 1u : 0u;
  v.rectLights = D.dRect.ptr; v.diskLights = D.dDisk.ptr; v.rectFrames = D.dRectFrames.ptr; v.diskFrames = D.dDiskFrames.ptr; v.triFaceId = D.dTriFaceId.ptr;
      v.nodeCount = s->nodeCount; v.triCount = s->triCount;
      v.bvhDepth = s->bvhDepth; v.hasCutouts = s->hasCutouts ? 1u : 0u;
  return v;
}
SceneView makeView(GiCScene* s) { return makeView(s, *s); }

uint32_t traceDynRefill(const GiCScene* s)
{
// ... 274 lines not shown
  p.mediaStride = rs.mediumStackSize ? rs.mediumStackSize * MEDIUM_FLOATS + 4u : 0u;
  p.pinned = optionSet("pool_slots") || s->optPoolSlots || optionSet("sample_buffer_mb") || s->optSampleBufferMb;
  if (!p.pinned) while (planBytes(p, pixels) > (availMb << 20) - std::min<uint64_t>(availMb << 19, 512ull << 20) && shrinkPlan(p, pixels)) sizeGrids(p, in);
  return p;
}

static int allocatePathPlan(GiCScene* s, SceneDevice& D, const GiCRenderSettings& rs, uint64_t samples, const SceneView& view, const PlanInputs& in,
                            PathPlan& plan)
{
  size_t memFree = 0, memTotal = 0; (void)hipMemGetInfo(&memFree, &memTotal);
  if (optionSet("assume_free_mb")) memFree = (size_t)optionValue("assume_free_mb", 0) << 20;
  if (!D.memTotalMb) D.memTotalMb = std::max<uint64_t>(1, (uint64_t)(memTotal >> 20));
  plan = planPathMemory(s, rs, samples, view, in, memFree, D.pathStateBytes(), D.memTotalMb);
  for (int attempt = 0;; attempt++) {
    int rc = plan.fused ? GI_C_OK : ensurePathState(&D, plan.slots, plan.wideBlocks, plan.traceBlocks);
    if (rc == GI_C_OK) rc = D.sampleBuf.alloc(in.pixels * plan.batchSamples);
    if (rc == GI_C_OK) rc = D.accum.alloc(in.pixels);
    if (rc == GI_C_OK && plan.mediaStride) rc = D.media.alloc(plan.slots * plan.mediaStride);
    if (rc == GI_C_OK) { if (attempt > 0) t_lastError.clear(); return GI_C_OK; }
    if (rc != GI_C_OUT_OF_MEMORY_INTERNAL) return GI_C_ERROR;
    D.releasePathState();
    if (attempt >= 40 || !shrinkPlan(plan, in.pixels)) {
      setError("giCRender: out of device memory even with the smallest sample buffer and path pool");
      return GI_C_ERROR;
    }
    sizeGrids(plan, in);
  }
}

struct StageTimers {
  enum Kind { RAYGEN = 0, TRACE = 1, SHADE = 2, SHADOW = 3 };
  struct IterRow { size_t evEnd; uint64_t traced, hits, shadow, ended, cont; };
  SceneDevice& D;
  bool on; uint32_t stride;
  bool iterLog;
  bool sampling = false;
  size_t ev = 0; std::vector<int> evKind;
  std::vector<IterRow> iterRows;
  uint64_t totalIters = 0, sampledIters = 0;

  StageTimers(const GiCScene* s, SceneDevice& d) : D(d), on(s->kernelTimers), stride(std::max(1u, s->kernelTimerStride)),
      iterLog(on && stride == 1u && getenv("GATLING_ITER_LOG") && atoi(getenv("GATLING_ITER_LOG")) != 0) {}
  void beginIteration(bool always = false) { sampling = on && (always || (totalIters % stride) == 0u); if (sampling) sampledIters++; }
  template <typename Fn> void timed(hipStream_t stream, int kind, Fn&& fn)
  {
    if (!sampling) { fn(); return; }
    (void)hipEventRecord(poolEvent(&D, ev), stream); fn(); (void)hipEventRecord(poolEvent(&D, ev + 1), stream);
    ev += 2; evKind.push_back(kind);
  }
  void finish(GiCRenderStats& S) const;
};

void StageTimers::finish(GiCRenderStats& S) const
{
  S.traceMs = S.shadeMs = S.raygenMs = S.shadowMs = 0.0;
  if (!on) return;
  auto elapsed = [&](size_t k) { float ms = 0.0f; (void)hipEventElapsedTime(&ms, D.eventPool[2 * k], D.eventPool[2 * k + 1]); return ms; };
  for (size_t k = 0; k < evKind.size(); k++) {
    const float ms = elapsed(k);
    if (evKind[k] == RAYGEN) S.raygenMs += ms; else if (evKind[k] == TRACE) S.traceMs += ms; else if (evKind[k] == SHADE) S.shadeMs += ms;
    else S.shadowMs += ms;
  }
  size_t k = 0;
  for (size_t r = 0; r < iterRows.size(); r++) {
    const IterRow& row = iterRows[r];
    double ms4[4] = {0.0, 0.0, 0.0, 0.0};
    for (; 2 * k < row.evEnd && k < evKind.size(); k++) ms4[evKind[k]] += elapsed(k);
    fprintf(stderr, "[gatling_gi] iter %3zu: rays %9llu hits %9llu shadow %9llu ended %9llu continuing %9llu | raygen %7.3f trace+route %7.3f shade %7.3f "
                    "shadow %7.3f ms\n", r,
            (unsigned long long)row.traced, (unsigned long long)row.hits, (unsigned long long)row.shadow, (unsigned long long)row.ended,
            (unsigned long long)row.cont, ms4[0], ms4[1], ms4[2], ms4[3]);
  }
  const double scale = sampledIters ? (double)totalIters / (double)sampledIters : 1.0;
  S.raygenMs *= scale; S.traceMs *= scale; S.shadeMs *= scale; S.shadowMs *= scale;
}

struct Schedule {
  bool twoStreamOk = false;
  long twoStreamDelay = 0;
  uint32_t dynRefill = 8u;
  uint32_t walkCarry = 0u;
  uint32_t lobePark = 0u;
  uint32_t ringCarry = 0u;
  uint32_t upsTraits = 0u;
  int32_t shadowOrderNow = -1;
};
struct Frame {
  GiCScene* s; SceneDevice& D; const DevCtx& ctx; const RenderJob& job; const GiCRenderSettings& rs;
  hipStream_t st;
  size_t pixels;
  StageTimers tm;
  FrameUniforms U{}; SceneView view{};
  PathPlan plan; PathState ps{}; QueueSet qs{}; Schedule sch;
  F4* colorOut = nullptr;
  GiCRenderBuffer* moments = nullptr;
  bool stackHighCounted = false;
  uint32_t numBatches = 0;
  uint32_t iters = 0, traceLaunches = 0;
  double tStart = 0.0;
  uint32_t windowCalls = 0;
  bool served = false;
  uint64_t skippedSegments = 0;
};

static int bindPathAovs(Frame& f, const BoundAovs& A)
{
  SceneDevice& D = f.D;
  f.ps = PathState{D.slots.ptr, D.media.ptr, f.plan.mediaStride, nullptr, 0u, nullptr};
  if (A.nee && f.rs.nextEventEstimation) {
    if (D.neeKey.alloc(f.pixels)) return GI_C_ERROR;
    HIP_TRY(hipMemsetAsync(D.neeKey.ptr, 0, f.pixels * sizeof(unsigned long long), f.st));
    f.ps.neeKey = D.neeKey.ptr;
  }
  if (A.bounces) f.ps.bouncesAov = reinterpret_cast<F4*>(rbMem(A.bounces, D.slot));
  if (A.clock) {
    if (D.pathSegments.alloc(f.pixels)) return GI_C_ERROR;
    HIP_TRY(hipMemsetAsync(D.pathSegments.ptr, 0, f.pixels * sizeof(uint32_t), f.st));
    f.ps.pathSegments = D.pathSegments.ptr;
  }
  return GI_C_OK;
}

static Schedule scheduleFrame(Frame& f)
{
  const GiCScene* s = f.s; const GiCRenderSettings& rs = f.rs; FrameUniforms& U = f.U;
  const bool fused = f.plan.fused;
  if (!fused && optionValue("work_order", WORK_ORDER_PIXEL_MAJOR_DEFAULT ? 1 : 0) != 0) U.flags |= FLAG_PIXEL_MAJOR;
  if (!fused && optionValue("defer_slot", 1) != 0 && !f.ps.neeKey && !f.ps.bouncesAov && !f.ps.pathSegments) U.flags |= FLAG_DEFER_SLOT;
  if ((U.flags & FLAG_DEFER_SLOT) && !traceBlockSync(f.view) && !f.view.twoLevel && f.view.domeTexture == 0u && rs.mediumStackSize == 0u && !s->countTraversal
      && s->boundsValid && optionValue("bounds_retire", 1) != 0) {
    U.flags |= FLAG_BOUNDS_RETIRE;
    for (int a = 0; a < 3; a++) { U.sceneLo[a] = s->bounds[a]; U.sceneHi[a] = s->bounds[3 + a]; }
  }
  if (fused && s->boundsValid && optionValue("bounds_retire", 1) != 0 && !s->countTraversal && !f.ps.neeKey && !f.ps.bouncesAov && !f.ps.pathSegments) {
    U.flags |= FLAG_BOUNDS_RETIRE;
    for (int a = 0; a < 3; a++) { U.sceneLo[a] = s->bounds[a]; U.sceneHi[a] = s->bounds[3 + a]; }
  }
  if (fused) {
    U.rectX0 = 0u; U.rectX1 = U.imageWidth; U.rectTy0 = 0u; U.rectTy1 = f.job.tileRows;
    if ((U.flags & FLAG_BOUNDS_RETIRE) && U.maxBounces > 0u && f.windowCalls < 2u && optionValue("miss_rect", 1) != 0) {
      const MissRect r = computeMissRect(U.sceneLo, U.sceneHi, U, U.imageWidth, U.imageHeight);
      uint32_t ty0, ty1; missRectTileRows(r, U.rowBegin, U.rowStride, f.job.tileRows, ty0, ty1);
      if (r.empty() || ty1 <= ty0) { U.rectX0 = U.rectX1 = U.rectTy0 = U.rectTy1 = 0u; }
      else { U.rectX0 = r.x0; U.rectX1 = r.x1; U.rectTy0 = ty0; U.rectTy1 = ty1; }
    }
    U.activeWidth = U.rectX1 - U.rectX0; U.activeCount = U.activeWidth * (U.rectTy1 - U.rectTy0);
    if (U.activeCount < U.pixelCount) U.flags |= FLAG_MISS_RECT;
  }
  Schedule sch;
  sch.walkCarry = s->countTraversal && !optionSet("walk_carry") ? 0u : (uint32_t)std::min(std::max(optionValue("walk_carry", WALK_CARRY_DEFAULT), 0L), 63L);
  sch.lobePark = s->countTraversal && !optionSet("lobe_park") ? 0u : (uint32_t)std::min(std::max(optionValue("lobe_park", LOBE_PARK_DEFAULT), 0L), 64L);
  sch.ringCarry = s->countTraversal && !optionSet("ring_carry") ? 0u : (optionValue("ring_carry", RING_CARRY_DEFAULT) != 0 ? 1u : 0u);
  f.s->upsPlainLaunched = 0u;
  sch.upsTraits = !s->countTraversal && optionValue("ups_plain", UPS_PLAIN_DEFAULT) != 0 ? s->upsTraits : 0u;
  sch.dynRefill = traceDynRefill(s);
  sch.shadowOrderNow = optionSet("shadow_order") ? (int32_t)optionValue("shadow_order", -1) : s->shadowOrder.load();
  sch.twoStreamOk = rs.nextEventEstimation != 0 && rs.mediumStackSize == 0u && f.view.domeTexture == 0u && optionValue("two_stream", 1) != 0
                    && f.ctx.stream2 != nullptr;
  sch.twoStreamDelay = optionValue("two_stream_delay", 0);
  return sch;
}
static bool scheduleBatch(Frame& f, uint64_t rounds)
{
  const GiCScene* s = f.s; FrameUniforms& U = f.U;
  const long mergeOpt = optionValue("merge_shade_variants", -1);
  const bool thinBatch = rounds == 1 && U.workTotal <= (8u << 20);
  if ((mergeOpt < 0 ? thinBatch : mergeOpt != 0) && (s->shadeClassMask & (1u << SHADE_CLASS_OPBR_BASE)) && (s->shadeClassMask & 4u)) {
    U.flags |= FLAG_MERGE_SHADE_VARIANTS;
  } else U.flags &= ~FLAG_MERGE_SHADE_VARIANTS;
  const bool two = f.sch.twoStreamOk && rounds == 1 && !f.tm.iterLog;
  if (two) U.flags |= FLAG_TWO_STREAM; else U.flags &= ~FLAG_TWO_STREAM;
  return two;
}

static void accumulateBatch(Frame& f, uint32_t batch)
{
  if (f.moments) launchMoments(f.st, f.U, f.D.sampleBuf.ptr, reinterpret_cast<F4*>(rbMem(f.moments, f.D.slot)), f.U.batchSamples, 0u,
                               f.windowCalls >= 2u ? f.U.spp : f.U.batchSamples, (f.U.flags & FLAG_PIXEL_MAJOR) != 0u, batch > 0u || f.job.momentsContinue);
  if (f.windowCalls >= 2u) {
    launchFoldWindow(f.st, f.U, f.D.sampleBuf.ptr, f.colorOut, f.U.batchSamples, 0u, (f.U.flags & FLAG_PIXEL_MAJOR) != 0u);
    return;
  }
  launchAccumulate(f.st, f.U, f.D.sampleBuf.ptr, f.D.accum.ptr, f.colorOut, batch == 0, batch + 1 == f.numBatches);
}

static int runFusedBatch(Frame& f, uint32_t batch)
{
  GiCScene* s = f.s; SceneDevice& D = f.D; const FrameUniforms& U = f.U;
  uint32_t chunk = 2048u;
  const uint64_t waves = (uint64_t)f.ctx.cuCount * 16u;
  chunk = (uint32_t)std::min<uint64_t>(chunk, std::max<uint64_t>(64u, ((uint64_t)U.workTotal / (waves * 16u)) & ~63ull));
  f.tm.beginIteration(true);
  f.tm.timed(f.st, StageTimers::TRACE, [&] {
    launchPath(f.st, (uint32_t)f.ctx.cuCount, s->classMask, s->classTextured != 0u, s->countTraversal, chunk, f.sch.walkCarry, f.sch.lobePark, f.sch.ringCarry,
               f.sch.upsTraits, U, f.view, f.ps, D.dCounters.ptr, D.sampleBuf.ptr);
  });
  s->upsPlainLaunched = pathUpsVariant(s->classMask, s->classTextured != 0u, (U.flags & FLAG_NEE) != 0u, f.view.hasCutouts != 0u, s->countTraversal, f.sch.upsTraits);
  f.iters++; f.tm.totalIters++; f.traceLaunches++;
  accumulateBatch(f, batch);
  return GI_C_OK;
}

static int runZeroBounceBatch(Frame& f, uint32_t batch)
{
  HIP_TRY(hipMemsetAsync(f.D.sampleBuf.ptr, 0, f.pixels * f.U.batchSamples * sizeof(F4), f.st));
  accumulateBatch(f, batch);
  return GI_C_OK;
}

static int runWavefrontBatch(Frame& f, uint32_t batch, uint32_t poolNow)
{
  GiCScene* s = f.s; SceneDevice& D = f.D; FrameUniforms& U = f.U; StageTimers& tm = f.tm;
  const GiCRenderSettings& rs = f.rs; const PathPlan& plan = f.plan; const Schedule& sch = f.sch;
  hipStream_t st = f.st, st2 = f.ctx.stream2;
  const uint64_t rounds = ((uint64_t)U.workTotal + poolNow - 1) / poolNow;
  const uint64_t maxIters = (rounds + 2) * (std::max(1u, U.maxBounces) + 1) + 8;
  const bool two = scheduleBatch(f, rounds);
  const bool nee = rs.nextEventEstimation != 0;
  bool shadowInFlight = false;
  struct JoinShadow {
    hipStream_t st2; const bool& inFlight;
    ~JoinShadow() { if (inFlight) (void)hipStreamSynchronize(st2); }
  } joinOnError{st2, shadowInFlight};
  auto joinShadow = [&]() -> hipError_t {
    if (!shadowInFlight) return hipSuccess;
    const hipError_t e = hipStreamWaitEvent(st, D.evShadow, 0);
    if (e == hipSuccess) shadowInFlight = false;
    return e;
  };
  for (uint64_t it = 0; it < maxIters; it++) {
    const uint32_t par = (uint32_t)(it & 1u);
    tm.beginIteration();
    auto raygen = [&] { tm.timed(st, StageTimers::RAYGEN, [&] { launchRaygen(st, plan.wideBlocks, U, f.ps, f.qs, D.dCounters.ptr, par, D.sampleBuf.ptr); }); };
    if (two) launchZeroClosest(st, D.dCounters.ptr, par);
    if (!two || it == 0) raygen();
    else if (rounds == 1 && it == (uint64_t)std::max(1u, U.maxBounces)) { HIP_TRY(joinShadow()); raygen(); }
    if (rounds == 1 && it == (uint64_t)std::max(1u, U.maxBounces) && rs.mediumStackSize == 0u) { tm.totalIters++; break; }
    if (it >= rounds) {
      constexpr uint32_t R = SceneDevice::POLL_RING, LAG = SceneDevice::POLL_LAG;
      constexpr size_t snapshot = (size_t)Q_COUNT * NSHARD;
      HIP_TRY(hipMemcpyAsync(D.hPoll + (it % R) * snapshot, D.dCounters.ptr, sizeof(PaddedCounter) * snapshot, hipMemcpyDeviceToHost, st));
      HIP_TRY(hipEventRecord(D.pollEvent[it % R], st));
      if (it >= rounds + LAG) {
        const uint64_t j = it - LAG;
        HIP_TRY(hipEventSynchronize(D.pollEvent[j % R]));
        const PaddedCounter* snap = D.hPoll + (j % R) * snapshot + (size_t)(Q_TRACE_A + (uint32_t)(j & 1u)) * NSHARD;
        const PaddedCounter* again = D.hPoll + (j % R) * snapshot + (size_t)(Q_REGEN_A + (uint32_t)((j & 1u) ^ 1u)) * NSHARD;
        uint32_t pending = 0; for (uint32_t k = 0; k < NSHARD; k++) pending += snap[k].v + again[k].v;
        if (pending == 0) { tm.totalIters++; break; }
      }
    }
    if (two && sch.twoStreamDelay == 1) launchSpin(st, 300000ull);
    tm.timed(st, StageTimers::TRACE, [&] {
      launchTrace(st, plan.traceBlocks, false, s->countTraversal, f.view, f.ps, f.qs, D.dCounters.ptr, Q_TRACE_A + par, Q_REGEN_A + (par ^ 1u), sch.dynRefill,
                  plan.wideBlocks, U, D.sampleBuf.ptr);
    });
    f.traceLaunches++;
    if (two && it > 0) { HIP_TRY(joinShadow()); raygen(); }
    uint32_t shadeMask = s->shadeClassMask | ((rs.mediumStackSize != 0u && (s->shadeClassMask & (1u << SHADE_CLASS_OPBR_BASE))) ? 4u : 0u);
    if (U.flags & FLAG_MERGE_SHADE_VARIANTS) shadeMask = (shadeMask & ~(1u << SHADE_CLASS_OPBR_BASE)) | ((shadeMask >> SHADE_CLASS_OPBR_BASE) & 1u) << 2;
    for (uint32_t klass = 0; klass < MAT_CLASS_COUNT; klass++) {
      if (!(shadeMask & (1u << klass))) continue;
      tm.timed(st, StageTimers::SHADE, [&] {
        launchShade(st, plan.wideBlocks, klass, (s->shadeClassTextured & (1u << klass)) != 0u, rs.mediumStackSize != 0u, U, f.view, f.ps, f.qs, D.dCounters.ptr,
                    par);
      });
    }
    if (nee) {
      const int32_t order = sch.shadowOrderNow >= 0 ? sch.shadowOrderNow : (int32_t)(tm.totalIters & 1u);
      hipStream_t on = st;
      if (two) {
        HIP_TRY(hipEventRecord(D.evShade, st)); HIP_TRY(hipStreamWaitEvent(st2, D.evShade, 0));
        if (sch.twoStreamDelay == 2) launchSpin(st2, 300000ull);
        on = st2;
      }
      tm.timed(on, StageTimers::SHADOW, [&] {
        launchTrace(on, plan.traceBlocks, true, s->countTraversal, f.view, f.ps, f.qs, D.dCounters.ptr, Q_SHADOW, Q_SHADOW,
                    sch.dynRefill | (order ? TRACE_DYN_SLOT_ORDER : 0u), plan.wideBlocks, U, D.sampleBuf.ptr);
      });
// ... 493 lines not shown
```

gatling_amd/csrc/gi_traversal.h:

```cpp
#pragma once

#include "gi_queues.h"
#include "gi_texture.h"

namespace gi {
GI_MATH_BEGIN

constexpr uint32_t LDS_NODES = 384;
constexpr uint32_t LDS_TRIS = 128;
constexpr uint32_t LDS_NODE_BYTES = 80;
constexpr uint32_t LDS_TRI_BYTES = 48;
constexpr uint32_t OVF_STACK = 40;
constexpr uint32_t TRACE_BLOCK = 256;

struct TraceCounters { uint32_t nodes, tris; };
struct TraceCountersHigh : TraceCounters { uint32_t high; };
template <bool COUNT> struct WalkCountersOf { using type = TraceCounters; };
template <> struct WalkCountersOf<true> { using type = TraceCountersHigh; };
template <bool COUNT> using WalkCounters = typename WalkCountersOf<COUNT>::type;

struct StagedScene {
  uint2 (*stack)[TRACE_BLOCK];
  const uint4* nodes;
  const uint4* tris;
  uint32_t ldsNodes, ldsTris;
};
enum Staged : uint32_t { STAGED_NONE, STAGED_SOME, STAGED_ALL };
__device__ __forceinline__ StagedScene stage_stack()
{
  extern __shared__ uint4 s_dyn[];
  return StagedScene{reinterpret_cast<uint2 (*)[TRACE_BLOCK]>(s_dyn), nullptr, nullptr, 0u, 0u};
}
template <uint32_t STACK>
__device__ __forceinline__ StagedScene stage_scene(const SceneView& sc, uint32_t ldsNodes, uint32_t ldsTris)
{
  extern __shared__ uint4 s_dyn[];
  uint4* s_nodes = s_dyn + (STACK * TRACE_BLOCK * sizeof(uint2)) / sizeof(uint4);
  uint4* s_tris = s_nodes + ldsNodes * 5u;
  for (uint32_t i = threadIdx.x; i < ldsNodes * 5u; i += TRACE_BLOCK) s_nodes[i] = reinterpret_cast<const uint4*>(sc.nodes)[i];
  for (uint32_t i = threadIdx.x; i < ldsTris * 3u; i += TRACE_BLOCK) s_tris[i] = reinterpret_cast<const uint4*>(sc.tris)[(i / 3u) * 4u + (i % 3u)];
  __syncthreads();
  return StagedScene{reinterpret_cast<uint2 (*)[TRACE_BLOCK]>(s_dyn), s_nodes, s_tris, ldsNodes, ldsTris};
}

__device__ __forceinline__ float cutout_random(uint32_t rng, uint32_t triId)
{
  uint32_t st = (rng ^ (triId * 0x9e3779b9u + 0x85ebca6bu)) * 747796405u + 2891336453u;
  uint32_t word = ((st >> ((st >> 28) + 4u)) ^ st) * 277803737u;
  return u2f(0x3f800000u | (((word >> 22) ^ word) >> 9)) - 1.0f;
}

struct RayWalk { V3 o, d; float idx, idy, idz, tMin, tBest; uint32_t octinv; uint2 G; uint32_t sp; };
struct RayTrav : RayWalk {
  uint32_t bestTri, bestOrig, bestMat; float bestU, bestV;
  bool found;
};

__device__ __forceinline__ void walk_set_ray(RayWalk& R, V3 o, V3 d)
{
  R.o = o; R.d = d;
  const float gx = (fabsf(d.x) < 1e-30f) ? (d.x < 0.0f ? -1e-30f : 1e-30f) : d.x;
  const float gy = (fabsf(d.y) < 1e-30f) ? (d.y < 0.0f ? -1e-30f : 1e-30f) : d.y;
  const float gz = (fabsf(d.z) < 1e-30f) ? (d.z < 0.0f ? -1e-30f : 1e-30f) : d.z;
  R.idx = __builtin_amdgcn_rcpf(gx); R.idy = __builtin_amdgcn_rcpf(gy); R.idz = __builtin_amdgcn_rcpf(gz);
  R.octinv = ((d.x >= 0.0f ? 1u : 0u) | (d.y >= 0.0f ? 2u : 0u) | (d.z >= 0.0f ? 4u : 0u)) * 0x01010101u;
}
__device__ __forceinline__ void walk_init(RayWalk& R, V3 o, V3 d, float tMin, float tMax)
{
  R.tMin = tMin; R.tBest = tMax;
  walk_set_ray(R, o, d);
  R.G = make_uint2(0u, 0x80000000u);
  R.sp = 0u;
}
__device__ __forceinline__ void trav_init(RayTrav& R, V3 o, V3 d, float tMin, float tMax)
{
  walk_init(R, o, d, tMin, tMax);
  R.bestTri = 0xffffffffu; R.bestOrig = 0xffffffffu; R.bestMat = 0u; R.bestU = 0.0f; R.bestV = 0.0f; R.found = false;
}

template <uint32_t STACK, bool OVERFLOW, bool ORDERED = true>
__device__ __forceinline__ uint32_t trav_node_pick(RayWalk& R, uint2 (*s_stack)[TRACE_BLOCK], uint2 (&overflow)[OVERFLOW ? OVF_STACK : 1])
{
  const uint32_t tid = threadIdx.x;
  uint2 G = R.G;
  uint32_t sp = R.sp;
  const uint32_t bit = 31u - (uint32_t)__clz((int)(G.y & 0xff000000u));
  G.y &= ~(1u << bit);
  if (G.y & 0xff000000u) {
    if (!OVERFLOW || sp < STACK) s_stack[sp < STACK ? sp : STACK - 1u][tid] = G; else overflow[sp - STACK] = G;
    sp++;
  }
  const uint32_t slot = ORDERED ? (bit - 24u) ^ (R.octinv & 7u) : bit - 24u;
  const uint32_t rel = (uint32_t)__popc((G.y & 0xffu) & ((1u << slot) - 1u));
  R.sp = sp;
  return G.x + rel;
}

typedef float gi_f2 __attribute__((ext_vector_type(2)));
template <bool SLACK = false, bool ORDERED = true>
__device__ __forceinline__ uint2 trav_node_test(RayWalk& R, const uint4& n0, const uint4& n1, const uint4& n2, const uint4& n3, const uint4& n4,
    float slack = 0.0f)
{
  const V3 o = R.o, d = R.d;
  constexpr float WIDEN = 1.00001f;
  const float sx = u2f((n0.w & 0xffu) << 23), sy = u2f(((n0.w >> 8) & 0xffu) << 23), sz = u2f(((n0.w >> 16) & 0xffu) << 23);
  const float ax = sx * R.idx, ay = sy * R.idy, az = sz * R.idz;
  const float bx = (u2f(n0.x) - o.x) * R.idx, by = (u2f(n0.y) - o.y) * R.idy, bz = (u2f(n0.z) - o.z) * R.idz;
  const gi_f2 Ax = {ax, ax * WIDEN}, Ay = {ay, ay * WIDEN}, Az = {az, az * WIDEN};
  const float ex = SLACK ? slack * fabsf(R.idx) : 0.0f, ey = SLACK ? slack * fabsf(R.idy) : 0.0f, ez = SLACK ? slack * fabsf(R.idz) : 0.0f;
  const gi_f2 Bx = SLACK ? gi_f2{bx - ex, (bx + ex) * WIDEN} : gi_f2{bx, bx * WIDEN}, By = SLACK ? gi_f2{by - ey, (by + ey) * WIDEN} : gi_f2{by, by * WIDEN},
              Bz = SLACK ? gi_f2{bz - ez, (bz + ez) * WIDEN} : gi_f2{bz, bz * WIDEN};
  const float tFar = R.tBest * WIDEN, tNear = R.tMin;
  const bool nxn = d.x < 0.0f, nyn = d.y < 0.0f, nzn = d.z < 0.0f;
  const uint32_t qlox[2] = {n2.x, n2.y}, qloy[2] = {n2.z, n2.w}, qloz[2] = {n3.x, n3.y};
  const uint32_t qhix[2] = {n3.z, n3.w}, qhiy[2] = {n4.x, n4.y}, qhiz[2] = {n4.z, n4.w};
  const uint32_t metaw[2] = {n1.z, n1.w};
  const uint32_t oct4 = R.octinv;
  uint32_t hitmask = 0u;
#pragma unroll
  for (int h = 0; h < 2; h++) {
    const uint32_t nearx = nxn ? qhix[h] : qlox[h], farx = nxn ? qlox[h] : qhix[h];
    const uint32_t neary = nyn ? qhiy[h] : qloy[h], fary = nyn ? qloy[h] : qhiy[h];
    const uint32_t nearz = nzn ? qhiz[h] : qloz[h], farz = nzn ? qloz[h] : qhiz[h];
    const uint32_t m4 = metaw[h];
    uint32_t idx4 = m4 & 0x1f1f1f1fu;
    if (ORDERED) {
      const uint32_t inner4 = ((m4 & (m4 << 1)) >> 4) & 0x01010101u;
      uint32_t hi4 = inner4 << 8;
      asm volatile("" : "+v"(hi4));
      idx4 = (m4 ^ (oct4 & (hi4 - inner4))) & 0x1f1f1f1fu;
    }
    const uint32_t bits4 = (m4 >> 5) & 0x07070707u;
#pragma unroll
    for (int k = 0; k < 4; k++) {
      const uint32_t sh = 8u * (uint32_t)k;
      const gi_f2 qx = {(float)((nearx >> sh) & 0xffu), (float)((farx >> sh) & 0xffu)};
      const gi_f2 qy = {(float)((neary >> sh) & 0xffu), (float)((fary >> sh) & 0xffu)};
      const gi_f2 qz = {(float)((nearz >> sh) & 0xffu), (float)((farz >> sh) & 0xffu)};
      const gi_f2 tx = __builtin_elementwise_fma(qx, Ax, Bx), ty = __builtin_elementwise_fma(qy, Ay, By), tz = __builtin_elementwise_fma(qz, Az, Bz);
      const float tn = fmaxf(fmaxf(tx.x, ty.x), fmaxf(tz.x, tNear));
      const float tf = fminf(fminf(tx.y, ty.y), fminf(tz.y, tFar));
      const uint32_t pos = (idx4 >> sh) & 0xffu;
      const uint32_t contrib = ((bits4 >> sh) & 0xffu) << pos;
      hitmask |= (tn <= tf) ? contrib : 0u;
    }
  }
  R.G = make_uint2(n1.x, (hitmask & 0xff000000u) | (n0.w >> 24));
  return make_uint2(n1.y, hitmask & 0x00ffffffu);
}

__device__ __forceinline__ void node_load(const SceneView& sc, uint32_t nodeIdx, uint4& n0, uint4& n1, uint4& n2, uint4& n3, uint4& n4)
{
  uint32_t off = nodeIdx << 4;
  asm volatile("" : "+v"(off));
  off += nodeIdx << 6;
  const uint4* p = reinterpret_cast<const uint4*>(reinterpret_cast<const char*>(sc.nodes) + off);
  n0 = p[0]; n1 = p[1]; n2 = p[2]; n3 = p[3]; n4 = p[4];
}

template <bool COUNT, uint32_t STACK, bool OVERFLOW, Staged STAGED, bool ORDERED = true>
__device__ __forceinline__ uint2 trav_node(RayWalk& R, const SceneView& sc, StagedScene S, uint2 (&overflow)[OVERFLOW ? OVF_STACK : 1],
                                           WalkCounters<COUNT>& tc)
{
  const uint32_t nodeIdx = trav_node_pick<STACK, OVERFLOW, ORDERED>(R, S.stack, overflow);
  uint4 n0, n1, n2, n3, n4;
  if (STAGED == STAGED_ALL || (STAGED == STAGED_SOME && nodeIdx < S.ldsNodes)) { const uint4* p = S.nodes + nodeIdx * 5u; n0 = p[0]; n1 = p[1]; n2 = p[2]; n3 = p[3]; n4 = p[4]; }
  else node_load(sc, nodeIdx, n0, n1, n2, n3, n4);
  if (COUNT) tc.nodes++;
  if constexpr (COUNT) tc.high = R.sp > tc.high ? R.sp : tc.high;
  return trav_node_test<false, ORDERED>(R, n0, n1, n2, n3, n4);
}

template <uint32_t STACK, bool OVERFLOW>
__device__ __forceinline__ bool trav_pop(RayWalk& R, uint2 (*s_stack)[TRACE_BLOCK], uint2 (&overflow)[OVERFLOW ? OVF_STACK : 1], uint32_t base = 0u)
{
  if (R.G.y & 0xff000000u) return false;
  if (R.sp == base) return true;
  const uint32_t sp = --R.sp;
  R.G = (!OVERFLOW || sp < STACK) ? s_stack[sp < STACK ? sp : STACK - 1u][threadIdx.x] : overflow[sp - STACK];
  return false;
}

__device__ __forceinline__ bool tri_test(V3 o, V3 d, float tMin, const uint4& a, const uint4& b, const uint4& c, float& t, float& u, float& v)
{
  const V3 v0 = v3(u2f(a.x), u2f(a.y), u2f(a.z)), e1 = v3(u2f(a.w), u2f(b.x), u2f(b.y)), e2 = v3(u2f(b.z), u2f(b.w), u2f(c.x));
  const V3 pv = cross(d, e2);
  const float det = dot(e1, pv);
  const float inv = gi_rcp(det);
  const V3 tv = o - v0;
  u = dot(tv, pv) * inv;
  const V3 qv = cross(tv, e1);
  v = dot(d, qv) * inv;
  t = dot(e2, qv) * inv;
  return (det != 0.0f) & (u >= 0.0f) & (v >= 0.0f) & (u + v <= 1.0f) & (t > tMin);
}

template <bool ANYHIT, bool COUNT, uint32_t STACK, bool OVERFLOW, Staged STAGED, bool CUTOUT>
__device__ __forceinline__ bool trav_step(RayTrav& R, const SceneView& sc, StagedScene S, uint2 (&overflow)[OVERFLOW ? OVF_STACK : 1], WalkCounters<COUNT>& tc,
                                          uint32_t rng)
{
  uint2 Gt;
  if (R.G.y & 0xff000000u) Gt = trav_node<COUNT, STACK, OVERFLOW, STAGED>(R, sc, S, overflow, tc);
  else { Gt = R.G; R.G = make_uint2(0u, 0u); }
  while (Gt.y) {
    const uint32_t k = (uint32_t)__ffs((int)Gt.y) - 1u;
    Gt.y &= Gt.y - 1u;
    const uint32_t triIdx = Gt.x + k;
    uint4 a, b, c;
    if (STAGED == STAGED_ALL || (STAGED == STAGED_SOME && triIdx < S.ldsTris)) { const uint4* p = S.tris + triIdx * 3u; a = p[0]; b = p[1]; c = p[2]; }
    else { const uint4* p = reinterpret_cast<const uint4*>(sc.tris) + (size_t)triIdx * 4u; a = p[0]; b = p[1]; c = p[2]; }
    if (COUNT) tc.tris++;
    const uint32_t orig = c.y;
    float t, u, v;
    const bool inside = tri_test(R.o, R.d, R.tMin, a, b, c, t, u, v);
    const bool better = (t < R.tBest) | ((t == R.tBest) & (R.bestOrig != 0xffffffffu) & (orig < R.bestOrig));
    bool accept = inside & better;
    if (CUTOUT && accept && (c.w & (1u << 28))) {
      const float opacity = cutout_opacity_at(sc, c.w, triIdx, u, v);
      accept = !(cutout_random(rng, orig) > opacity);
    }
    if (accept) {
      R.tBest = t; R.bestU = u; R.bestV = v; R.bestTri = triIdx; R.bestOrig = orig; R.bestMat = c.w; R.found = true;
      if (ANYHIT) { R.G.y = 0u; R.sp = 0u; break; }
    }
  }
  return trav_pop<STACK, OVERFLOW>(R, S.stack, overflow);
}

constexpr uint32_t TRI_ID_BITS = 26;
struct WaveTri {
  unsigned long long best[64];
  uint4 hit[64];
  uint32_t queue[128];
};
#define GI_LDS __attribute__((address_space(3)))
typedef uint32_t gi_u4 __attribute__((ext_vector_type(4)));
__device__ __forceinline__ void wt_queue_put(WaveTri& W, uint32_t i, uint32_t v) { *(volatile GI_LDS uint32_t*)&((GI_LDS WaveTri*)&W)->queue[i] = v; }
__device__ __forceinline__ uint32_t wt_queue_get(WaveTri& W, uint32_t i) { return *(volatile GI_LDS uint32_t*)&((GI_LDS WaveTri*)&W)->queue[i]; }
__device__ __forceinline__ void wt_best_put(WaveTri& W, uint32_t i, unsigned long long v)
{ *(volatile GI_LDS unsigned long long*)&((GI_LDS WaveTri*)&W)->best[i] = v; }
__device__ __forceinline__ unsigned long long wt_best_get(WaveTri& W, uint32_t i)
{ return *(volatile GI_LDS unsigned long long*)&((GI_LDS WaveTri*)&W)->best[i]; }
__device__ __forceinline__ uint32_t wt_best_t(WaveTri& W, uint32_t i) { return ((volatile GI_LDS uint32_t*)&((GI_LDS WaveTri*)&W)->best[i])[1]; }
__device__ __forceinline__ uint32_t wt_best_id(WaveTri& W, uint32_t i) { return ((volatile GI_LDS uint32_t*)&((GI_LDS WaveTri*)&W)->best[i])[0]; }
__device__ __forceinline__ void wt_best_min(WaveTri& W, uint32_t i, unsigned long long v)
{ __hip_atomic_fetch_min((GI_LDS unsigned long long*)&((GI_LDS WaveTri*)&W)->best[i], v, __ATOMIC_RELAXED, __HIP_MEMORY_SCOPE_WORKGROUP); }
__device__ __forceinline__ void wt_hit_put(WaveTri& W, uint32_t i, uint32_t x, uint32_t y, uint32_t z, uint32_t w)
{ gi_u4 v = {x, y, z, w}; *(volatile GI_LDS gi_u4*)&((GI_LDS WaveTri*)&W)->hit[i] = v; }
typedef uint32_t gi_u3 __attribute__((ext_vector_type(3)));
__device__ __forceinline__ void wt_hit_put3(WaveTri& W, uint32_t i, uint32_t x, uint32_t y, uint32_t z)
{ gi_u3 v = {x, y, z}; *(volatile GI_LDS gi_u3*)&((GI_LDS WaveTri*)&W)->hit[i] = v; }
__device__ __forceinline__ uint32_t wt_helpers_add(WaveTri& W, uint32_t i, uint32_t v)
{ return __hip_atomic_fetch_add(&((GI_LDS uint32_t*)&((GI_LDS WaveTri*)&W)->hit[i])[3], v, __ATOMIC_RELAXED, __HIP_MEMORY_SCOPE_WORKGROUP); }
__device__ __forceinline__ uint4 wt_hit_get(WaveTri& W, uint32_t i)
{ const gi_u4 v = *(volatile GI_LDS gi_u4*)&((GI_LDS WaveTri*)&W)->hit[i]; return make_uint4(v.x, v.y, v.z, v.w); }

template <bool CUTOUT>
__device__ __forceinline__ void owner_ray(uint32_t rl, V3 ro, V3 rd, float rtMin, uint32_t rng, V3& o, V3& d, float& tMin, uint32_t& rrng)
{
  o = v3(__shfl(ro.x, (int)rl), __shfl(ro.y, (int)rl), __shfl(ro.z, (int)rl));
  d = v3(__shfl(rd.x, (int)rl), __shfl(rd.y, (int)rl), __shfl(rd.z, (int)rl));
  tMin = __shfl(rtMin, (int)rl);
  rrng = CUTOUT ? (uint32_t)__shfl((int)rng, (int)rl) : 0u;
}

template <bool CUTOUT, bool RESULT_RECORD>
__device__ __forceinline__ void wave_tri_accept(WaveTri& W, uint32_t rl, uint32_t rrng, const SceneView& sc, bool accept, float t, float u, float v,
                                                const uint4& c, uint32_t flatTri, uint32_t recTri)
{
  if (CUTOUT && accept && (c.w & (1u << 28))) {
    const float opacity = cutout_opacity_at(sc, c.w, flatTri, u, v);
    accept = !(cutout_random(rrng, c.y) > opacity);
  }
  if (accept) {
    const unsigned long long key = ((unsigned long long)f2u(t) << 32) | (unsigned long long)(c.y + 1u);
    wt_best_min(W, rl, key);
    if (wt_best_get(W, rl) == key) {
      if (RESULT_RECORD) wt_hit_put3(W, rl, f2u(u), f2u(v), recTri | (((c.w >> 24) & 0xfu) << 28));
      else wt_hit_put(W, rl, recTri, f2u(u), f2u(v), c.w);
    }
  }
}

template <bool COUNT, Staged STAGED, bool CUTOUT, bool RESULT_RECORD = false, bool LINEAR = false>
__device__ __forceinline__ void wave_tri_batch(WaveTri& W, uint32_t head, uint32_t cnt, const RayWalk& R, uint32_t rng, const SceneView& sc,
                                               StagedScene S, TraceCounters& tc)
{
  const uint32_t lane = __lane_id();
  const bool act = lane < cnt;
  const uint32_t e = act ? wt_queue_get(W, LINEAR ? head + lane : (head + lane) & 127u) : 0u;
  const uint32_t rl = e >> TRI_ID_BITS, triIdx = e & ((1u << TRI_ID_BITS) - 1u);
  V3 o, d; float tMin; uint32_t rrng;
  owner_ray<CUTOUT>(rl, R.o, R.d, R.tMin, rng, o, d, tMin, rrng);
  if (act) {
    uint4 a, b, c;
    if (STAGED == STAGED_ALL || (STAGED == STAGED_SOME && triIdx < S.ldsTris)) { const uint4* p = S.tris + triIdx * 3u; a = p[0]; b = p[1]; c = p[2]; }
    else { const uint4* p = reinterpret_cast<const uint4*>(sc.tris) + (size_t)triIdx * 4u; a = p[0]; b = p[1]; c = p[2]; }
    if (COUNT) tc.tris++;
    float t, u, v;
    const bool inside = tri_test(o, d, tMin, a, b, c, t, u, v);
    wave_tri_accept<CUTOUT, RESULT_RECORD>(W, rl, rrng, sc, inside, t, u, v, c, triIdx, triIdx);
  }
}

__device__ __forceinline__ uint32_t wave_scan_inclusive(uint32_t v)
{
  int scan = (int)v;
  scan += __builtin_amdgcn_update_dpp(0, scan, 0x111, 0xf, 0xf, false);
  scan += __builtin_amdgcn_update_dpp(0, scan, 0x112, 0xf, 0xf, false);
  scan += __builtin_amdgcn_update_dpp(0, scan, 0x114, 0xf, 0xf, false);
  scan += __builtin_amdgcn_update_dpp(0, scan, 0x118, 0xf, 0xf, false);
  scan += __builtin_amdgcn_update_dpp(0, scan, 0x142, 0xa, 0xf, false);
  scan += __builtin_amdgcn_update_dpp(0, scan, 0x143, 0xc, 0xf, false);
  return (uint32_t)scan;
}

template <bool ANYHIT, bool COUNT, uint32_t STACK, bool OVERFLOW, Staged STAGED, bool CUTOUT>
__device__ __forceinline__ bool wave_step(RayTrav& R, bool alive, WaveTri& W, const SceneView& sc, StagedScene S,
                                          uint2 (&overflow)[OVERFLOW ? OVF_STACK : 1], WalkCounters<COUNT>& tc, uint32_t rng)
{
  const uint32_t lane = __lane_id();
  uint2 Gt = make_uint2(0u, 0u);
  if (alive) Gt = trav_node<COUNT, STACK, OVERFLOW, STAGED>(R, sc, S, overflow, tc);
  uint32_t head = 0u, tail = 0u;
  {
    const uint32_t cntL = (uint32_t)__popc(Gt.y);
    const uint32_t scan = wave_scan_inclusive(cntL);
    const uint32_t total = (uint32_t)__builtin_amdgcn_readlane((int)scan, 63);
    if (total <= 128u) {
      uint32_t pos = scan - cntL;
      while (Gt.y) {
        const uint32_t k = (uint32_t)__ffs((int)Gt.y) - 1u;
        Gt.y &= Gt.y - 1u;
        wt_queue_put(W, pos, (lane << TRI_ID_BITS) | (Gt.x + k));
        pos++;
      }
      tail = total;
      while (tail - head >= 64u) { wave_tri_batch<COUNT, STAGED, CUTOUT>(W, head, 64u, R, rng, sc, S, tc); head += 64u; }
    }
  }
  for (;;) {
    const unsigned long long m = __ballot(Gt.y != 0u);
    if (!m) break;
    if (Gt.y) {
      const uint32_t k = (uint32_t)__ffs((int)Gt.y) - 1u;
      Gt.y &= Gt.y - 1u;
      wt_queue_put(W, (tail + (uint32_t)__popcll(m & ((1ull << lane) - 1ull))) & 127u, (lane << TRI_ID_BITS) | (Gt.x + k));
    }
    tail += (uint32_t)__popcll(m);
    if (tail - head >= 64u) { wave_tri_batch<COUNT, STAGED, CUTOUT>(W, head, 64u, R, rng, sc, S, tc); head += 64u; }
  }
  if (tail != head) wave_tri_batch<COUNT, STAGED, CUTOUT>(W, head, tail - head, R, rng, sc, S, tc);
  bool done = false;
  if (alive) {
    const unsigned long long key = wt_best_get(W, lane);
    R.tBest = u2f((uint32_t)(key >> 32));
    R.found = (uint32_t)key != 0u;
    done = (ANYHIT && R.found) ? true : trav_pop<STACK, OVERFLOW>(R, S.stack, overflow);
  }
  return done;
}

struct RingStats { uint32_t batches, pairs, partial, flushes, ballotSteps; };
template <bool COUNT, Staged STAGED, bool CUTOUT>
__device__ __forceinline__ void wave_ring_batch(WaveTri& W, uint32_t& pend, uint32_t n, const RayWalk& R, uint32_t rng, const SceneView& sc, StagedScene S,
                                                TraceCounters& tc, RingStats& rs)
{
  pend -= n;
  wave_tri_batch<COUNT, STAGED, CUTOUT, false, true>(W, pend, n, R, rng, sc, S, tc);
  if (COUNT) { rs.batches++; rs.pairs += n; if (n < 64u) rs.partial++; }
}
template <bool COUNT, uint32_t STACK, Staged STAGED, bool CUTOUT>
__device__ __forceinline__ bool wave_step_ring(RayTrav& R, bool alive, WaveTri& W, const SceneView& sc, StagedScene S, uint2 (&overflow)[1], WalkCounters<COUNT>& tc,
                                               uint32_t rng, uint32_t& pend, RingStats& rs)
{
  const uint32_t lane = __lane_id();
  uint2 Gt = make_uint2(0u, 0u);
  if (alive) Gt = trav_node<COUNT, STACK, false, STAGED>(R, sc, S, overflow, tc);
  const uint32_t cntL = (uint32_t)__popc(Gt.y);
  const uint32_t scan = wave_scan_inclusive(cntL);
  const uint32_t total = (uint32_t)__builtin_amdgcn_readlane((int)scan, 63);
  if (pend + total <= 128u) {
    uint32_t pos = pend + scan - cntL;
    while (Gt.y) {
      const uint32_t k = (uint32_t)__ffs((int)Gt.y) - 1u;
      Gt.y &= Gt.y - 1u;
      wt_queue_put(W, pos, (lane << TRI_ID_BITS) | (Gt.x + k));
      pos++;
    }
    pend += total;
    while (pend >= 64u) wave_ring_batch<COUNT, STAGED, CUTOUT>(W, pend, 64u, R, rng, sc, S, tc, rs);
  } else {
    if (COUNT) rs.ballotSteps++;
    for (;;) {
      const unsigned long long m = __ballot(Gt.y != 0u);
      if (!m) break;
      if (Gt.y) {
        const uint32_t k = (uint32_t)__ffs((int)Gt.y) - 1u;
        Gt.y &= Gt.y - 1u;
        wt_queue_put(W, pend + (uint32_t)__popcll(m & ((1ull << lane) - 1ull)), (lane << TRI_ID_BITS) | (Gt.x + k));
      }
      pend += (uint32_t)__popcll(m);
      if (pend >= 64u) wave_ring_batch<COUNT, STAGED, CUTOUT>(W, pend, 64u, R, rng, sc, S, tc, rs);
    }
  }
  pend = (uint32_t)__builtin_amdgcn_readfirstlane((int)pend);
  return alive ? trav_pop<STACK, false>(R, S.stack, overflow) : false;
}
__device__ __forceinline__ void wave_ring_refresh(RayTrav& R, WaveTri& W)
{
  const unsigned long long key = wt_best_get(W, __lane_id());
  R.tBest = u2f((uint32_t)(key >> 32));
  R.found = (uint32_t)key != 0u;
}

__device__ __forceinline__ void wave_ray_begin(WaveTri& W, float tMax) { wt_best_put(W, __lane_id(), (unsigned long long)f2u(tMax) << 32); }
__device__ __forceinline__ void wave_ray_end(WaveTri& W, RayTrav& R)
{
  __atomic_signal_fence(__ATOMIC_SEQ_CST);
  if (R.found) { const uint4 h = wt_hit_get(W, __lane_id()); R.bestTri = h.x; R.bestU = u2f(h.y); R.bestV = u2f(h.z); R.bestMat = h.w; }
}

template <bool ANYHIT, bool COUNT, uint32_t STACK, bool OVERFLOW, Staged STAGED, bool CUTOUT>
__device__ __forceinline__ bool traverse(const SceneView& sc, StagedScene S, V3 o, V3 d, float tMin, float tMax, float& outT, float& outU, float& outV,
                                         uint32_t& outTri, uint32_t& outMat, WalkCounters<COUNT>& tc, uint32_t rng = 0u)
{
  RayTrav R; trav_init(R, o, d, tMin, tMax);
  uint2 overflow[OVERFLOW ? OVF_STACK : 1];
  while (!trav_step<ANYHIT, COUNT, STACK, OVERFLOW, STAGED, CUTOUT>(R, sc, S, overflow, tc, rng)) {}
  outT = R.tBest; outU = R.bestU; outV = R.bestV; outTri = R.bestTri; outMat = R.bestMat;
  return R.found;
}

constexpr uint32_t TLAS_ITEM_TAG = 0x80000000u, NO_INSTANCE = 0xffffffffu;
struct RayTrav2 : RayWalk { V3 wo, wd; uint32_t inst, spBase; float slack; };

__device__ __forceinline__ void trav2_init(RayTrav2& R, V3 o, V3 d, float tMin, float tMax)
{
  walk_init(R, o, d, tMin, tMax);
  R.wo = o; R.wd = d; R.inst = NO_INSTANCE; R.spBase = 0u; R.slack = 0.0f;
}
__device__ __forceinline__ void trav2_enter(RayTrav2& R, const SceneView& sc, uint32_t inst)
{
  const float4* ip = reinterpret_cast<const float4*>(&sc.instTrav[inst]);
  const float4 r0 = ip[0], r1 = ip[1], r2 = ip[2], r3 = ip[3], r4 = ip[4], r5 = ip[5], r6 = ip[6];
  const V3 rel = v3(R.wo.x - r0.w, R.wo.y - r1.w, R.wo.z - r2.w);
  const float w[9] = {r3.x, r3.y, r3.z, r3.w, r4.x, r4.y, r4.z, r4.w, r5.x};
  const V3 o = v3((w[0] * rel.x + w[1] * rel.y) + w[2] * rel.z, (w[3] * rel.x + w[4] * rel.y) + w[5] * rel.z, (w[6] * rel.x + w[7] * rel.y) + w[8] * rel.z);
  const V3 d = v3((w[0] * R.wd.x + w[1] * R.wd.y) + w[2] * R.wd.z, (w[3] * R.wd.x + w[4] * R.wd.y) + w[5] * R.wd.z,
      (w[6] * R.wd.x + w[7] * R.wd.y) + w[8] * R.wd.z);
  const float m0 = (fabsf(w[0] * rel.x) + fabsf(w[1] * rel.y)) + fabsf(w[2] * rel.z), m1 = (fabsf(w[3] * rel.x) + fabsf(w[4] * rel.y)) + fabsf(w[5] * rel.z),
              m2 = (fabsf(w[6] * rel.x) + fabsf(w[7] * rel.y)) + fabsf(w[8] * rel.z);
  R.slack = 4.0e-6f * ((m0 + m1) + (m2 + r6.x));
  walk_set_ray(R, o, d);
  R.inst = inst; R.spBase = R.sp;
  R.G = make_uint2(f2u(r5.y), 0x80000000u);
}
__device__ __forceinline__ void trav2_leave(RayTrav2& R)
{
  walk_set_ray(R, R.wo, R.wd);
  R.inst = NO_INSTANCE; R.slack = 0.0f;
// ... 96 lines not shown
```

include/gi_c.h:

```cpp
#ifndef GATLING_GI_C_H
#define GATLING_GI_C_H

#include <stdint.h>
#include <stddef.h>

#ifdef __cplusplus
extern "C" {
#endif

#define GI_C_OK 0
#define GI_C_ERROR 1

#define GI_C_MAX_AOV_COMP_SIZE 16

typedef enum GiCAovId {
  GI_C_AOV_COLOR = 0, GI_C_AOV_NORMAL, GI_C_AOV_NEE, GI_C_AOV_BARYCENTRICS, GI_C_AOV_TEXCOORDS, GI_C_AOV_BOUNCES,
  GI_C_AOV_CLOCK_CYCLES, GI_C_AOV_OPACITY, GI_C_AOV_TANGENTS, GI_C_AOV_BITANGENTS, GI_C_AOV_THIN_WALLED,
  GI_C_AOV_OBJECT_ID, GI_C_AOV_DEPTH, GI_C_AOV_FACE_ID, GI_C_AOV_INSTANCE_ID, GI_C_AOV_DOUBLE_SIDED, GI_C_AOV_ALBEDO,
  GI_C_AOV_COUNT
} GiCAovId;

#define GI_C_AOV_EXT_MOMENTS 0x100

typedef enum GiCRenderBufferFormat { GI_C_FORMAT_INT32 = 0, GI_C_FORMAT_FLOAT32 = 1, GI_C_FORMAT_FLOAT32_VEC4 = 2 } GiCRenderBufferFormat;
// ... 364 lines not shown
#define GI_C_SCENE_OPTION_BLAS_UPDATES 17
#define GI_C_SCENE_OPTION_TLAS_VISIBILITY 18
#define GI_C_SCENE_OPTION_TLAS_ONLY 19
#define GI_C_SCENE_OPTION_TLAS_TOPOLOGY 20
#define GI_C_SCENE_OPTION_TLAS_INSTANCES 21
#define GI_C_SCENE_OPTION_TLAS_DEVICE_BUILD 22
#define GI_C_SCENE_OPTION_BLAS_DEVICE_BUILD 23
#define GI_C_SCENE_OPTION_TLAS_COMPACTION 24
#define GI_C_SCENE_OPTION_LEAF_LIFT 25
int giCGetLookaheadStats(const GiCScene* scene, GiCLookaheadStats* out);
int giCSetSceneOption(GiCScene* scene, int32_t option, int32_t value);
int giCTraceRays(GiCScene* scene, uint32_t count, const float* origins , const float* dirs ,
                 float tMin, float tMax, float* outTUV , int32_t* outInstPrim );

int giCDebugEvalBsdf(const GiCMaterialDesc* desc, uint32_t count, const float* in, float* out);
int giCDebugShadeClass(const GiCMaterialDesc* desc);
int64_t giCDebugCheckSqrt(uint32_t first, uint64_t count);
int64_t giCDebugCheckDiv(uint32_t mode, uint64_t count, uint32_t seed, const uint32_t* words);
int giCDebugTexRuntime(const float* rgba, uint32_t width, uint32_t height, uint32_t depth, uint32_t count, const float* queries, float* out);
int giCDebugValidateBvh(const float* triVerts, uint32_t triCount, uint32_t* outNodeCount, uint32_t* outMaxDepth);
int giCDebugBvhStackReach(const float* triVerts, uint32_t triCount, const float* origins, const float* dirs, uint32_t rayCount, uint32_t* out );
int giCDebugValidatePartitionedBvh(const float* triVerts, uint32_t triCount, uint32_t partCount, uint32_t* outNodeCount, uint32_t* outMaxDepth);
int giCDebugRefitBvh(const float* triVertsA, const float* triVertsB, uint32_t triCount, uint32_t* outNodeCount, uint32_t* outMaxDepth);
int giCDebugSceneRefitCheck(const GiCScene* scene, uint32_t deviceIndex, uint32_t* outNodes);
int giCDebugValidateSceneBvh(const GiCScene* scene, uint32_t deviceIndex, uint32_t* outNodeCount, uint32_t* outMaxDepth, int32_t* outBuiltOnDevice,
                             uint64_t* outDigest);

int32_t giCDebugEditDirtyFlags(int32_t edit, int32_t built);
int giCDebugSceneUpdateCounts(const GiCScene* scene, uint64_t* outCounts );
int giCDebugSceneVisibilityUpdateCount(const GiCScene* scene, uint64_t* outCount);
int giCDebugSceneVertexUpdateCount(const GiCScene* scene, uint64_t* outCount);
int giCDebugSceneTopologyUpdateCount(const GiCScene* scene, uint64_t* outCount);
int giCDebugSceneResyncCount(const GiCScene* scene, uint64_t* outCount);
int giCDebugGatherShade(const GiCVertex* vertices, uint32_t vertexCount, const GiCFace* faces, uint32_t faceCount);
int giCDebugSceneInstanceUpdateCount(const GiCScene* scene, uint64_t* out );
int giCDebugCloneInstance(const GiCVertex* vertices, uint32_t vertexCount, const GiCFace* faces, uint32_t faceCount, int32_t isLeftHanded, const float* xformA,
                          const float* xformB);
int giCDebugSceneShadeCheck(const GiCScene* scene, uint32_t deviceIndex, uint32_t* outRecords);
int giCDebugSceneTlasUpdateCount(const GiCScene* scene, uint64_t* outCount);
int giCDebugSceneTlasCheck(const GiCScene* scene, uint32_t deviceIndex, uint32_t* out );
#define GI_C_TLAS_BUILD_TOO_DEEP (-2)
int giCDebugBuildTlasHost(const float* boxes6, uint32_t count, uint32_t depthBudget, uint32_t radius, double* out );
int giCDebugBuildTlas(const float* boxes6, uint32_t count, uint32_t depthBudget, uint32_t radius, double* out );
int giCDebugSceneTlasBuildStats(const GiCScene* scene, uint64_t out[16]);
int giCDebugBuildBlasHost(const GiCVertex* vertices, uint32_t vertexCount, const GiCFace* faces, uint32_t faceCount, uint32_t depthBudget, uint32_t radius,
                          double* out );
int giCDebugBuildBlas(const GiCVertex* vertices, uint32_t vertexCount, const GiCFace* faces, uint32_t faceCount, uint32_t depthBudget, uint32_t radius,
                      double* out );
int giCDebugSceneBlasBuildStats(const GiCScene* scene, uint64_t out[16]);
int giCDebugInstanceBounds(const GiCVertex* vertices, uint32_t vertexCount, const GiCFace* faces, uint32_t faceCount, const float* xforms16, uint32_t xformCount,
                           float* outBoxes6, uint32_t* outStatus);
int giCDebugSceneBlasUpdateCount(const GiCScene* scene, uint64_t* outCount);
int giCDebugSceneBlasCheck(const GiCScene* scene, uint32_t deviceIndex, uint32_t* out );
int giCDebugBlasRefit(const GiCVertex* a, const GiCVertex* b, uint32_t vertexCount, const GiCFace* faces, uint32_t faceCount, uint32_t* outNodes,
                      uint32_t* outViolations);
int giCDebugBlasRefitHost(const GiCVertex* a, const GiCVertex* b, uint32_t vertexCount, const GiCFace* faces, uint32_t faceCount, uint32_t* outNodes,
                          uint32_t* outViolations);
int giCDebugSceneTlasVisibilityUpdateCount(const GiCScene* scene, uint64_t* outCount);
int giCDebugSceneTlasTopologyUpdateCount(const GiCScene* scene, uint64_t* outCount);
int giCDebugAppendRecords(const GiCVertex* vertices, uint32_t vertexCount, const GiCFace* faces, uint32_t faceCount, const int32_t* faceIds, uint32_t maxFaceId,
                          uint32_t flags, const float* xforms16, uint32_t xformCount, uint32_t vertexOffset, uint32_t shadeBase, uint32_t idBase, uint32_t matFlags);
int giCDebugAppendRecordsHost(const GiCVertex* vertices, uint32_t vertexCount, const GiCFace* faces, uint32_t faceCount, const int32_t* faceIds, uint32_t maxFaceId,
                              uint32_t flags, const float* xforms16, uint32_t xformCount, uint32_t vertexOffset, uint32_t shadeBase, uint32_t idBase,
                              uint32_t matFlags);
typedef struct GiCDebugInstanceMesh { const GiCVertex* vertices; const GiCFace* faces; const int32_t* faceIds; uint32_t vertexCount, faceCount, maxFaceId, flags; } GiCDebugInstanceMesh;
typedef struct GiCDebugInstanceJob { uint32_t mesh, instanceSlot, recordSlot, idBase; float transform[16]; } GiCDebugInstanceJob;
int giCDebugInstanceRecords(const GiCDebugInstanceMesh* meshes, uint32_t meshCount, const GiCDebugInstanceJob* jobs, uint32_t jobCount);
int giCDebugInstanceRecordsHost(const GiCDebugInstanceMesh* meshes, uint32_t meshCount, const GiCDebugInstanceJob* jobs, uint32_t jobCount);
int giCDebugSceneTlasInstanceUpdateStats(const GiCScene* scene, uint64_t out[4]);
int giCDebugSceneCompactionCount(const GiCScene* scene, uint64_t out[4]);
typedef struct GiCDebugCompactRange { uint32_t count, live, delta[3], hidden; } GiCDebugCompactRange;
int giCDebugCompactRanges(uint32_t kind, const void* records, uint32_t recordCount, const GiCDebugCompactRange* ranges, uint32_t rangeCount, uint32_t outInfo[4]);
int giCDebugCompactRangesHost(uint32_t kind, const void* records, uint32_t recordCount, const GiCDebugCompactRange* ranges, uint32_t rangeCount, uint32_t outInfo[4]);
int giCDebugSceneFlatTreeState(const GiCScene* scene, uint32_t device, uint64_t out[4]);
int giCDebugSceneFlatIdCheck(const GiCScene* scene, uint32_t deviceIndex, uint32_t* out );
int giCDebugPatchVisibilityTwoLevel(const uint32_t* faceCounts, const uint8_t* hiddenBefore, const uint8_t* hiddenAfter, uint32_t instanceCount, uint32_t seed,
                                    uint32_t* outTris);
int giCDebugSceneClassState(const GiCScene* scene, uint32_t* out );
int giCDebugSceneUpsPlain(const GiCScene* scene, uint32_t* out );
int giCDebugUpsTraits(const GiCMaterialDesc* descs, uint32_t count, int derive, uint32_t* out );
int giCDebugSceneLeafLift(const GiCScene* scene, uint32_t* out );
int giCDebugLeafLift(const float* triVerts, uint32_t triCount, int32_t mode, const void* treeNodes, uint32_t treeNodeCount, uint32_t treeDepth,
                     void* outNodes, uint32_t nodeCap, uint32_t* outOrder, uint32_t* outInfo , double* outCost );
int giCDebugPathWalkStats(const GiCScene* scene, uint64_t* out );
int giCDebugPathLobeStats(const GiCScene* scene, uint64_t* out );
int giCDebugPathRingStats(const GiCScene* scene, uint64_t* out );
int giCDebugTraversalStackHigh(const GiCScene* scene, uint32_t* out );
int giCDebugPathLot(uint32_t bvhDepth, uint32_t nodeCount, uint32_t triCount, uint32_t* out );
int giCDebugMissRect(const float* bounds , const GiCCameraDesc* camera, const GiCRenderSettings* settings, uint32_t width, uint32_t height,
                     uint32_t* out );
typedef struct GiCDebugMomentsDesc {
  uint32_t width, rows, bufferSamples, first, count, pixelMajor;
} GiCDebugMomentsDesc;
int giCDebugSampleMoments(const GiCDebugMomentsDesc* desc, const float* samples, const float* prevM, const uint32_t* rect , const float* missRgb ,
                          float* outM);
int giCDebugSampleMomentsHost(const GiCDebugMomentsDesc* desc, const float* samples, const float* prevM, const uint32_t* rect ,
                              const float* missRgb , float* outM);

#ifdef __cplusplus
}
#endif
#endif
```

Baseline: 14240 Msamples/s.

## Cook BVH8 nodes into LDS records with sorted slots and per-octant child tables

Adds a cooked LDS node layout for the fused path kernel. When it stages the tree, the kernel reorders child slots so occupied ones come first and precomputes per-octant child-bit contribution tables. The node test then reads a table by ray octant instead of decoding meta bits per child, and skips the upper half and the last child pairs when they are empty across the wave. This costs a larger LDS image, extra cooking work at block start, and a new kernel variant.

New measurement: 14850 Msamples/s (median of 6 runs). 4.2% higher.

```diff
diff --git a/gatling_amd/build.py b/gatling_amd/build.py
--- a/gatling_amd/build.py
+++ b/gatling_amd/build.py
@@ -10,7 +10,7 @@
 LIB = os.path.join(_HERE, "libgatling_gi.so")
 HOST_SOURCES = ["gi_c.cpp", "gi_scene.cpp", "gi_textures.cpp", "gi_lights.cpp", "gi_build.cpp", "gi_render.cpp", "gi_debug.cpp", "gi_denoise_host.cpp"]
 SOURCES = HOST_SOURCES + ["gi_image.cpp", "bvh8.cpp", "leaf_lift.cpp", "gi_kernels.hip", "gi_trace.hip", "gi_shade.hip", "gi_aov.hip", "gi_aov2.hip", "gi_path.hip", "gi_bvh_build.hip", "gi_patch.hip", "gi_refit.hip", "gi_tlas.hip", "gi_blas.hip", "gi_append.hip", "gi_instances.hip", "gi_compact.hip", "gi_tlas_build.hip", "gi_tlas_build_host.cpp", "gi_blas_build.hip", "gi_blas_build_host.cpp", "gi_denoise.hip", "gi_moments.hip", "gi_denoise_var.hip", "gtl_shim.cpp"]
-HEADERS = ["gi_host.h", "gi_types.h", "gi_kernels.h", "gi_device_math.h", "gi_queues.h", "gi_traversal.h", "gi_texture.h", "gi_shading.h", "gi_stages.h", "gi_image.h", "gi_options.h", "gi_miss_rect.h", "bvh8.h", "gi_bvh_build.h", "gi_refit.h", "gi_tlas.h", "gi_blas.h", "gi_pack.h", "gi_vispatch.h", "gi_aov_body.h", "gi_append.h", "gi_instances.h", "gi_compact.h", "gi_bvh_stages.h", "gi_tlas_build.h", "gi_blas_build.h", "gi_denoise.h", "gi_moments.h",
+HEADERS = ["gi_host.h", "gi_types.h", "gi_kernels.h", "gi_device_math.h", "gi_queues.h", "gi_traversal.h", "gi_texture.h", "gi_shading.h", "gi_stages.h", "gi_image.h", "gi_options.h", "gi_miss_rect.h", "bvh8.h", "gi_bvh_build.h", "gi_refit.h", "gi_tlas.h", "gi_blas.h", "gi_pack.h", "gi_vispatch.h", "gi_aov_body.h", "gi_append.h", "gi_instances.h", "gi_compact.h", "gi_bvh_stages.h", "gi_tlas_build.h", "gi_blas_build.h", "gi_denoise.h", "gi_moments.h", "gi_node_cook.h",
            os.path.join("..", "..", "include", "gi_c.h"), os.path.join("..", "..", "include", "gtl", "gi", "Gi.h"),
            os.path.join("..", "..", "include", "gtl", "gb", "ParamTypes.h")]
 INCLUDE = os.path.join(_HERE, "..", "include")
diff --git a/gatling_amd/capi.py b/gatling_amd/capi.py
--- a/gatling_amd/capi.py
+++ b/gatling_amd/capi.py
@@ -192,6 +192,9 @@
     ("giCDebugSceneVisibilityUpdateCount", C.c_int, [_P, C.POINTER(C.c_uint64)]), ("giCDebugSceneClassState", C.c_int, [_P, C.POINTER(C.c_uint32)]),
     ("giCDebugSceneUpsPlain", C.c_int, [_P, C.POINTER(C.c_uint32)]), ("giCDebugUpsTraits", C.c_int, [C.POINTER(GiCMaterialDesc), _U, C.c_int, C.POINTER(C.c_uint32)]),
     ("giCDebugSceneLeafLift", C.c_int, [_P, C.POINTER(C.c_uint32)]),
+    ("giCDebugSceneNodeCook", C.c_int, [_P, C.POINTER(C.c_uint32)]),
+    ("giCDebugNodeCook", C.c_int, [_P, _U, C.c_int32, _P, _U, C.POINTER(C.c_uint32)]),
+    ("giCDebugCheckNodeCook", C.c_int64, [_P, _U, _FP, C.c_uint64]),
     ("giCDebugLeafLift", C.c_int, [_FP, _U, C.c_int32, _P, _U, _U, _P, _U, C.POINTER(C.c_uint32), C.POINTER(C.c_uint32), C.POINTER(C.c_double)]),
     ("giCDebugSceneVertexUpdateCount", C.c_int, [_P, C.POINTER(C.c_uint64)]), ("giCDebugRefitBvh", C.c_int, [_FP, _FP, _U, C.POINTER(C.c_uint32), C.POINTER(C.c_uint32)]),
     ("giCDebugSceneRefitCheck", C.c_int, [_P, _U, C.POINTER(C.c_uint32)]),
@@ -378,6 +381,31 @@
         raise GiError(f"giCDebugLeafLift failed ({rc})")
     return {"violations": rc, "nodes": nodes[:int(info[0])].copy(), "order": order[:len(v)].copy(), "depth": int(info[1]), "lifted": int(info[2]),
             "active": int(info[3]), "cost_before": float(cost[0]), "cost_after": float(cost[1])}
+
+
+def node_cook(nodes, oct_blocks: int = -1) -> dict:
+    import numpy as np
+    L = load_library()
+    given = np.ascontiguousarray(np.frombuffer(bytes(nodes), np.uint8)).reshape(-1, 80)
+    n = len(given)
+    blocks = max(n - 1, 0) if oct_blocks < 0 else int(oct_blocks)
+    image = np.zeros(n * 28 + blocks * 64, np.uint32); info = np.zeros(3, np.uint32)
+    if L.giCDebugNodeCook(given.ctypes.data_as(_P), n, int(oct_blocks), image.ctypes.data_as(_P), image.nbytes, info.ctypes.data_as(C.POINTER(C.c_uint32))) != GI_C_OK:
+        raise GiError("giCDebugNodeCook failed: " + L.giCGetLastError().decode())
+    assert int(info[0]) == image.nbytes and int(info[1]) == 112 and int(info[2]) == 256
+    return {"records": image[:n * 28].reshape(n, 28).copy(), "oct": image[n * 28:].reshape(blocks, 8, 8).copy(), "stride": int(info[1]),
+            "oct_block_bytes": int(info[2])}
+
+
+def check_node_cook(nodes, rays) -> int:
+    import numpy as np
+    L = load_library()
+    given = np.ascontiguousarray(np.frombuffer(bytes(nodes), np.uint8)).reshape(-1, 80)
+    r = np.ascontiguousarray(rays, np.float32).reshape(-1, 8)
+    bad = L.giCDebugCheckNodeCook(given.ctypes.data_as(_P), len(given), r.ctypes.data_as(_FP), len(r))
+    if bad < 0:
+        raise GiError("giCDebugCheckNodeCook failed: " + L.giCGetLastError().decode())
+    return int(bad)
 
 
 def bvh_stack_reach(tri_verts, origins, dirs):
@@ -998,6 +1026,12 @@
             raise GiError("giCDebugSceneUpsPlain failed")
         return {"traits": int(c[0]), "launched": int(c[1])}
 
+    def node_cook(self) -> bool:
+        c = (C.c_uint32 * 1)()
+        if self.L.giCDebugSceneNodeCook(self.handle, c) != GI_C_OK:
+            raise GiError("giCDebugSceneNodeCook failed")
+        return bool(c[0])
+
     def leaf_lift(self) -> dict:
         c = (C.c_uint32 * 2)()
         if self.L.giCDebugSceneLeafLift(self.handle, c) != GI_C_OK:
diff --git a/gatling_amd/csrc/gi_debug.cpp b/gatling_amd/csrc/gi_debug.cpp
--- a/gatling_amd/csrc/gi_debug.cpp
+++ b/gatling_amd/csrc/gi_debug.cpp
@@ -6,6 +6,7 @@
 #include "gi_bvh_stages.h"
 #include "gi_compact.h"
 #include "gi_moments.h"
+#include "gi_node_cook.h"
 #include "bvh8.h"
 
 static int giCTraceRaysImpl(GiCScene* s, uint32_t count, const float* origins, const float* dirs, float tMin, float tMax, float* outTUV, int32_t* outInstPrim);
@@ -556,6 +557,52 @@
   return (int64_t)h;
 }
 
+extern "C" int giCDebugSceneNodeCook(const GiCScene* scene, uint32_t* out)
+{
+  const GiCScene* s = scene;
+  if (!s || !out) { setError("giCDebugSceneNodeCook: bad arguments"); return GI_C_ERROR; }
+  out[0] = s->nodeCookLaunched;
+  return GI_C_OK;
+}
+
+extern "C" int giCDebugNodeCook(const void* nodes, uint32_t nodeCount, int32_t octBlocks, void* outImage, uint32_t imageCap, uint32_t* outInfo)
+{
+  if (!nodes || !outImage || !outInfo || nodeCount == 0u || nodeCount > (1u << 16)) { setError("giCDebugNodeCook: bad arguments"); return GI_C_ERROR; }
+  const uint32_t blocks = octBlocks < 0 ? gi::cook_oct_blocks_max(nodeCount) : (uint32_t)octBlocks;
+  if (blocks > (1u << 16)) { setError("giCDebugNodeCook: bad arguments"); return GI_C_ERROR; }
+  const uint32_t bytes = nodeCount * gi::COOK_NODE_BYTES + blocks * gi::COOK_OCT_DWORDS * 4u;
+  if (imageCap < bytes) { setError("giCDebugNodeCook: the image needs more room"); return GI_C_ERROR; }
+  std::vector<gi::Node8> in(nodeCount);
+  memcpy(in.data(), nodes, (size_t)nodeCount * sizeof(gi::Node8));
+  std::vector<uint32_t> image(bytes / 4u, 0u);
+  for (uint32_t i = 0; i < nodeCount; i++) gi::cook_place(in.data(), i, nodeCount, blocks, image.data());
+  memcpy(outImage, image.data(), bytes);
+  outInfo[0] = bytes; outInfo[1] = gi::COOK_NODE_BYTES; outInfo[2] = gi::COOK_OCT_DWORDS * 4u;
+  return GI_C_OK;
+}
+
+extern "C" int64_t giCDebugCheckNodeCook(const void* nodes, uint32_t nodeCount, const float* rays, uint64_t count)
+{
+  if (!g_ctx.initialized) { setError("giCDebugCheckNodeCook before giCInitialize"); return -1; }
+  if (!nodes || !rays || nodeCount == 0u || nodeCount > 64u || count == 0u || count > (1ull << 26)) { setError("giCDebugCheckNodeCook: bad arguments"); return -1; }
+  const size_t nodeBytes = (size_t)nodeCount * sizeof(gi::Node8), rayBytes = (size_t)count * 8u * sizeof(float);
+  unsigned long long* d = nullptr; unsigned long long h = 0ull; gi::Node8* dn = nullptr; float* dr = nullptr;
+  bool ok = hipMalloc(&d, sizeof(h)) == hipSuccess && hipMalloc(&dn, nodeBytes) == hipSuccess && hipMalloc(&dr, rayBytes) == hipSuccess;
+  ok = ok && hipMemcpyAsync(dn, nodes, nodeBytes, hipMemcpyHostToDevice, g_ctx.stream) == hipSuccess;
+  ok = ok && hipMemcpyAsync(dr, rays, rayBytes, hipMemcpyHostToDevice, g_ctx.stream) == hipSuccess;
+  ok = ok && hipMemsetAsync(d, 0, sizeof(h), g_ctx.stream) == hipSuccess;
+  if (ok) {
+    ok = launchDebugNodeCook(g_ctx.stream, dn, nodeCount, dr, (unsigned long long)count, d) == 0;
+    ok = ok && hipMemcpyAsync(&h, d, sizeof(h), hipMemcpyDeviceToHost, g_ctx.stream) == hipSuccess;
+  }
+  ok = hipStreamSynchronize(g_ctx.stream) == hipSuccess && ok;
+  if (d) (void)hipFree(d);
+  if (dn) (void)hipFree(dn);
+  if (dr) (void)hipFree(dr);
+  if (!ok) { setError("giCDebugCheckNodeCook: device error"); return -1; }
+  return (int64_t)h;
+}
+
 extern "C" int32_t giCDebugEditDirtyFlags(int32_t edit, int32_t built)
 {
   std::unique_ptr<GiCScene> scene(new GiCScene());
diff --git a/gatling_amd/csrc/gi_host.h b/gatling_amd/csrc/gi_host.h
--- a/gatling_amd/csrc/gi_host.h
+++ b/gatling_amd/csrc/gi_host.h
@@ -323,6 +323,7 @@
   uint32_t classTextured = 0;
   uint32_t shadeClassMask = 0, shadeClassTextured = 0;
   uint32_t upsTraits = 0, upsPlainLaunched = 0;
+  uint32_t nodeCookLaunched = 0;
   std::unique_ptr<SceneHost> host;
   std::vector<std::unique_ptr<SceneDevice>> replicas;
   bool countTraversal = false, kernelTimers = false;
diff --git a/gatling_amd/csrc/gi_kernels.h b/gatling_amd/csrc/gi_kernels.h
--- a/gatling_amd/csrc/gi_kernels.h
+++ b/gatling_amd/csrc/gi_kernels.h
@@ -40,7 +40,14 @@
 
 bool pathKernelSupports(const SceneView& sc);
 int launchPath(hipStream_t s, uint32_t cuCount, uint32_t classMask, bool textured, bool count, uint32_t chunk, uint32_t walkCarry, uint32_t lobePark,
-               uint32_t ringCarry, uint32_t upsTraits, const FrameUniforms& U, const SceneView& sc, const PathState& st, Counters* cnt, F4* sampleBuf);
+               uint32_t ringCarry, uint32_t upsTraits, uint32_t nodeCook, const FrameUniforms& U, const SceneView& sc, const PathState& st, Counters* cnt,
+               F4* sampleBuf, uint32_t* cooked);
+inline bool pathCookVariant(uint32_t classMask, bool textured, bool nee, bool cutout, bool count)
+{
+  return (classMask == 1u || classMask == 2u) && !textured && !cutout && !count && !nee;
+}
+uint32_t pathCookedLdsBytes(uint32_t stackEntries, uint32_t ldsNodes, uint32_t ldsTris);
+constexpr long NODE_COOK_DEFAULT = 1;
 inline uint32_t pathUpsVariant(uint32_t classMask, bool textured, bool nee, bool cutout, bool count, uint32_t upsTraits)
 {
   return (classMask == 2u && !textured && !cutout && !count && !nee) ? upsTraits : 0u;
@@ -109,6 +116,7 @@
 void launchDebugBsdf(hipStream_t s, const MaterialRec* mat, uint32_t shadeClass, uint32_t count, const float* in, float* out);
 void launchDebugSqrt(hipStream_t s, uint32_t first, unsigned long long count, unsigned long long* mismatches);
 void launchDebugDiv(hipStream_t s, uint32_t mode, unsigned long long count, uint32_t seed, const uint32_t* words, unsigned long long* mismatches);
+int launchDebugNodeCook(hipStream_t s, const Node8* nodes, uint32_t nodeCount, const float* rays, unsigned long long count, unsigned long long* mismatches);
 void launchDebugTex(hipStream_t s, const float* texels, uint32_t w, uint32_t h, uint32_t d, uint32_t count, const float* queries, float* out);
 
 }
diff --git a/gatling_amd/csrc/gi_node_cook.h b/gatling_amd/csrc/gi_node_cook.h
--- /dev/null
+++ b/gatling_amd/csrc/gi_node_cook.h
@@ -0,0 +1,76 @@
+#pragma once
+
+#include <stdint.h>
+
+#include "gi_types.h"
+
+#if defined(__HIP__)
+#define GI_COOK_HD __host__ __device__
+#else
+#define GI_COOK_HD
+#endif
+
+namespace gi {
+
+constexpr uint32_t COOK_NODE_DWORDS = 28, COOK_NODE_BYTES = COOK_NODE_DWORDS * 4u;
+constexpr uint32_t COOK_TABLE_DWORDS = 8, COOK_OCT_DWORDS = 8u * COOK_TABLE_DWORDS;
+constexpr uint32_t COOK_OCT_MASK = 0xe0u;
+constexpr uint32_t COOK_TABLE_AT = 20;
+
+GI_COOK_HD inline uint32_t cook_meta(const uint32_t* w, uint32_t slot) { return (w[6u + (slot >> 2)] >> (8u * (slot & 3u))) & 0xffu; }
+GI_COOK_HD inline bool cook_meta_inner(uint32_t m) { return (m & 0x18u) == 0x18u; }
+GI_COOK_HD inline bool cook_has_inner(const uint32_t* w)
+{
+  for (uint32_t s = 0; s < 8u; s++) if (cook_meta_inner(cook_meta(w, s))) return true;
+  return false;
+}
+GI_COOK_HD inline uint32_t cook_inner_before(const Node8* nodes, uint32_t i)
+{
+  uint32_t n = 0;
+  for (uint32_t j = 0; j < i; j++) n += cook_has_inner(reinterpret_cast<const uint32_t*>(&nodes[j])) ? 1u : 0u;
+  return n;
+}
+GI_COOK_HD inline uint32_t cook_oct_blocks_max(uint32_t n) { return n ? n - 1u : 0u; }
+GI_COOK_HD inline uint32_t cook_image_bytes(uint32_t n) { return n * COOK_NODE_BYTES + cook_oct_blocks_max(n) * COOK_OCT_DWORDS * 4u; }
+GI_COOK_HD inline uint32_t cook_contrib(uint32_t m, uint32_t oct)
+{
+  const uint32_t idx = cook_meta_inner(m) ? (m ^ oct) & 0x1fu : m & 0x1fu;
+  return (m >> 5) << idx;
+}
+
+GI_COOK_HD inline void cook_node(const Node8& node, uint32_t tableOff, uint32_t* rec, uint32_t* oct)
+{
+  const uint32_t* w = reinterpret_cast<const uint32_t*>(&node);
+  uint32_t perm[8], meta[8], n = 0;
+  for (uint32_t s = 0; s < 8u; s++) if (cook_meta(w, s) != 0u) perm[n++] = s;
+  const uint32_t occupied = n;
+  for (uint32_t s = 0; s < 8u; s++) if (cook_meta(w, s) == 0u) perm[n++] = s;
+  for (uint32_t k = 0; k < 8u; k++) meta[k] = cook_meta(w, perm[k]);
+  const bool inner = oct != nullptr && cook_has_inner(w);
+  for (uint32_t i = 0; i < 6u; i++) rec[i] = w[i];
+  rec[6] = (((occupied + 1u) & ~1u) << 16) | (inner ? COOK_OCT_MASK : 0u);
+  rec[7] = tableOff;
+  for (uint32_t plane = 0; plane < 6u; plane++) {
+    for (uint32_t h = 0; h < 2u; h++) {
+      uint32_t v = 0u;
+      for (uint32_t k = 0; k < 4u; k++) {
+        const uint32_t s = perm[4u * h + k];
+        v |= ((w[8u + 2u * plane + (s >> 2)] >> (8u * (s & 3u))) & 0xffu) << (8u * k);
+      }
+      rec[8u + 2u * plane + h] = v;
+    }
+  }
+  for (uint32_t k = 0; k < 8u; k++) rec[COOK_TABLE_AT + k] = inner ? 0u : cook_contrib(meta[k], 0u);
+  if (inner) for (uint32_t o = 0; o < 8u; o++) for (uint32_t k = 0; k < 8u; k++) oct[o * COOK_TABLE_DWORDS + k] = cook_contrib(meta[k], o);
+}
+
+GI_COOK_HD inline void cook_place(const Node8* nodes, uint32_t i, uint32_t n, uint32_t blocks, uint32_t* image)
+{
+  uint32_t* rec = image + i * COOK_NODE_DWORDS;
+  const uint32_t block = cook_has_inner(reinterpret_cast<const uint32_t*>(&nodes[i])) ? cook_inner_before(nodes, i) : 0xffffffffu;
+  if (block >= blocks) { cook_node(nodes[i], COOK_TABLE_AT * 4u, rec, nullptr); return; }
+  uint32_t* oct = image + n * COOK_NODE_DWORDS + block * COOK_OCT_DWORDS;
+  cook_node(nodes[i], (uint32_t)(oct - rec) * 4u, rec, oct);
+}
+
+}
diff --git a/gatling_amd/csrc/gi_path.hip b/gatling_amd/csrc/gi_path.hip
--- a/gatling_amd/csrc/gi_path.hip
+++ b/gatling_amd/csrc/gi_path.hip
@@ -17,7 +17,7 @@
 constexpr uint32_t PATH_STACK_MAX = 8;
 
 constexpr int PATH_WAVES = 4;
-template <uint32_t KLASS, bool TEXTURED, bool NEE, bool CUTOUT, bool COUNT, uint32_t PATH_STACK, uint32_t UPS = 0u>
+template <uint32_t KLASS, bool TEXTURED, bool NEE, bool CUTOUT, bool COUNT, uint32_t PATH_STACK, uint32_t UPS = 0u, bool COOK = false>
 __global__ __launch_bounds__(TRACE_BLOCK) __attribute__((amdgpu_waves_per_eu(PATH_WAVES, 8))) void k_path(FrameUniforms U, SceneView sc, PathState st,
     Counters* cnt, F4* __restrict__ sampleBuf, uint32_t ldsNodes, uint32_t ldsTris, uint32_t chunk, uint32_t walkCarry, uint32_t lobePark, uint32_t lotRow,
     uint32_t lotCap, uint32_t ringCarry)
@@ -25,7 +25,8 @@
   constexpr bool CARRY = !NEE;
   constexpr bool PARK = !NEE && (KLASS == 1u || (KLASS == KLASS_DYNAMIC && COUNT));
   constexpr bool DEFER = PARK || COUNT;
-  const StagedScene S = stage_scene<PATH_STACK>(sc, ldsNodes, ldsTris);
+  static_assert(!COOK || (!NEE && !COUNT), "cooked nodes: the hot variants without NEE (wave_step_ring)");
+  const StagedScene S = COOK ? stage_scene_cooked<PATH_STACK>(sc, ldsNodes, ldsTris) : stage_scene<PATH_STACK>(sc, ldsNodes, ldsTris);
   __shared__ WaveTri s_wave[TRACE_BLOCK / 64];
   WaveTri& W = s_wave[threadIdx.x >> 6];
 
@@ -138,7 +139,7 @@
           whLanes[step] += n; whTrips[step]++; step = step < 7u ? step + 1u : 7u;
           if (n < 8u) whFew++;
         }
-        if (wave_step_ring<COUNT, PATH_STACK, STAGED_ALL, CUTOUT>(R, tAlive, W, sc, S, overflow, tc, rng, pend, ringN)) tAlive = false;
+        if (wave_step_ring<COUNT, PATH_STACK, STAGED_ALL, CUTOUT, COOK>(R, tAlive, W, sc, S, overflow, tc, rng, pend, ringN)) tAlive = false;
         walking = __ballot(tAlive);
         const bool last = (uint32_t)__popcll(walking) <= stop;
         if ((last || ringCarry == 0u) && pend != 0u) {
@@ -328,12 +329,23 @@
          && !sc.shadePacked;
 }
 
+uint32_t pathCookedLdsBytes(uint32_t stackEntries, uint32_t ldsNodes, uint32_t ldsTris)
+{
+  return stackEntries * TRACE_BLOCK * (uint32_t)sizeof(uint2) + cook_image_bytes(ldsNodes) + ldsTris * LDS_TRI_BYTES;
+}
+
 using PathKernel = void (*)(FrameUniforms, SceneView, PathState, Counters*, F4*, uint32_t, uint32_t, uint32_t, uint32_t, uint32_t, uint32_t, uint32_t, uint32_t);
 template <uint32_t STACK>
-static PathKernel pickPathKernel(uint32_t classMask, bool textured, bool nee, bool cutout, bool count, uint32_t upsTraits)
+static PathKernel pickPathKernel(uint32_t classMask, bool textured, bool nee, bool cutout, bool count, uint32_t upsTraits, bool cook = false)
 {
   const bool hot = (classMask == 1u || classMask == 2u || classMask == 4u) && !textured && !cutout && !count;
   const uint32_t ups = pathUpsVariant(classMask, textured, nee, cutout, count, upsTraits);
+  if (cook) {
+    if (!pathCookVariant(classMask, textured, nee, cutout, count)) return nullptr;
+    if (classMask == 1u) return k_path<0u, false, false, false, false, STACK, 0u, true>;
+    if (ups == UPS_NOCOAT) return k_path<1u, false, false, false, false, STACK, UPS_NOCOAT, true>;
+    return k_path<1u, false, false, false, false, STACK, 0u, true>;
+  }
   return dispatchBools([&](auto neeC) -> PathKernel {
     constexpr bool NEE = decltype(neeC)::value;
     if (hot) {
@@ -349,18 +361,34 @@
 }
 
 int launchPath(hipStream_t s, uint32_t cuCount, uint32_t classMask, bool textured, bool count, uint32_t chunk, uint32_t walkCarry, uint32_t lobePark,
-               uint32_t ringCarry, uint32_t upsTraits, const FrameUniforms& U, const SceneView& sc, const PathState& st, Counters* cnt, F4* sampleBuf)
-{
+               uint32_t ringCarry, uint32_t upsTraits, uint32_t nodeCook, const FrameUniforms& U, const SceneView& sc, const PathState& st, Counters* cnt,
+               F4* sampleBuf, uint32_t* cooked)
+{
+  if (cooked) *cooked = 0u;
   if (U.workTotal == 0u) return 0;
   const uint32_t ldsNodes = sc.nodeCount, ldsTris = sc.triCount;
   const PathLot lot = pathLotPlacement(sc.bvhDepth);
   const uint32_t stack = lot.stack;
   assert(sc.bvhDepth <= stack && lot.row >= sc.bvhDepth && lot.row + (lot.capacity + 7u) / 8u <= stack);
-  const uint32_t bytes = traceLdsBytes(stack, ldsNodes, ldsTris);
+  uint32_t bytes = traceLdsBytes(stack, ldsNodes, ldsTris);
   const bool neeOn = (U.flags & FLAG_NEE) != 0u;
   PathKernel k = stack == 4u
       ? pickPathKernel<4u>(classMask, textured, neeOn, sc.hasCutouts != 0u, count, upsTraits)
       : pickPathKernel<8u>(classMask, textured, neeOn, sc.hasCutouts != 0u, count, upsTraits);
+  if (nodeCook != 0u) {
+    PathKernel kc = stack == 4u
+        ? pickPathKernel<4u>(classMask, textured, neeOn, sc.hasCutouts != 0u, count, upsTraits, true)
+        : pickPathKernel<8u>(classMask, textured, neeOn, sc.hasCutouts != 0u, count, upsTraits, true);
+    hipFuncAttributes fr{}, fc{};
+    if (kc && hipFuncGetAttributes(&fr, reinterpret_cast<const void*>(k)) == hipSuccess
+        && hipFuncGetAttributes(&fc, reinterpret_cast<const void*>(kc)) == hipSuccess) {
+      const uint32_t cookedBytes = pathCookedLdsBytes(stack, ldsNodes, ldsTris);
+      if (blocksPerCuByLds(cookedBytes, (uint32_t)fc.sharedSizeBytes) >= blocksPerCuByLds(bytes, (uint32_t)fr.sharedSizeBytes)) {
+        k = kc; bytes = cookedBytes;
+        if (cooked) *cooked = 1u;
+      }
+    }
+  }
   int perCu = 2;
   hipFuncAttributes fa{};
   if (hipFuncGetAttributes(&fa, reinterpret_cast<const void*>(k)) == hipSuccess && fa.numRegs > 0) {
@@ -439,4 +467,34 @@
   hipLaunchKernelGGL(k_debug_div, dim3(4096), dim3(256), 0, s, mode, count, seed, words, mismatches);
 }
 
-}
+constexpr uint32_t DEBUG_COOK_NODES = 64;
+__global__ __launch_bounds__(TRACE_BLOCK) void k_debug_node_cook(const Node8* __restrict__ nodes, uint32_t nodeCount, const float* __restrict__ rays,
+                                                                 unsigned long long count, unsigned long long* mismatches)
+{
+  __shared__ uint4 s_image[(DEBUG_COOK_NODES * COOK_NODE_BYTES + DEBUG_COOK_NODES * COOK_OCT_DWORDS * 4u) / sizeof(uint4)];
+  if (nodeCount == 0u || nodeCount > DEBUG_COOK_NODES) return;
+  for (uint32_t i = threadIdx.x; i < nodeCount; i += TRACE_BLOCK) cook_place(nodes, i, nodeCount, DEBUG_COOK_NODES, reinterpret_cast<uint32_t*>(s_image));
+  __syncthreads();
+  unsigned long long bad = 0ull;
+  for (unsigned long long i = blockIdx.x * (unsigned long long)blockDim.x + threadIdx.x; i < count; i += (unsigned long long)gridDim.x * blockDim.x) {
+    const float* r = rays + 8ull * i;
+    const uint32_t nodeIdx = (uint32_t)(i % nodeCount);
+    RayWalk A, B;
+    walk_init(A, v3(r[0], r[1], r[2]), v3(r[3], r[4], r[5]), r[6], r[7]);
+    B = A;
+    const uint4* p = reinterpret_cast<const uint4*>(nodes) + nodeIdx * 5u;
+    const uint2 ga = trav_node_test<false, true>(A, p[0], p[1], p[2], p[3], p[4]);
+    const uint2 gb = trav_node_test_cooked(B, (const GI_LDS gi_u4*)((const GI_LDS char*)s_image + __umul24(nodeIdx, COOK_NODE_BYTES)));
+    if (A.G.x != B.G.x || A.G.y != B.G.y || ga.x != gb.x || ga.y != gb.y) bad++;
+  }
+  if (bad) atomicAdd(mismatches, bad);
+}
+
+int launchDebugNodeCook(hipStream_t s, const Node8* nodes, uint32_t nodeCount, const float* rays, unsigned long long count, unsigned long long* mismatches)
+{
+  if (nodeCount == 0u || nodeCount > DEBUG_COOK_NODES) return -1;
+  hipLaunchKernelGGL(k_debug_node_cook, dim3(256), dim3(TRACE_BLOCK), 0, s, nodes, nodeCount, rays, count, mismatches);
+  return 0;
+}
+
+}
diff --git a/gatling_amd/csrc/gi_render.cpp b/gatling_amd/csrc/gi_render.cpp
--- a/gatling_amd/csrc/gi_render.cpp
+++ b/gatling_amd/csrc/gi_render.cpp
@@ -380,6 +380,7 @@
   uint32_t walkCarry = 0u;
   uint32_t lobePark = 0u;
   uint32_t ringCarry = 0u;
+  uint32_t nodeCook = 0u;
   uint32_t upsTraits = 0u;
   int32_t shadowOrderNow = -1;
 };
@@ -451,6 +452,8 @@
   sch.ringCarry = s->countTraversal && !optionSet("ring_carry") ? 0u : (optionValue("ring_carry", RING_CARRY_DEFAULT) != 0 ? 1u : 0u);
   f.s->upsPlainLaunched = 0u;
   sch.upsTraits = !s->countTraversal && optionValue("ups_plain", UPS_PLAIN_DEFAULT) != 0 ? s->upsTraits : 0u;
+  f.s->nodeCookLaunched = 0u;
+  sch.nodeCook = optionValue("node_cook", NODE_COOK_DEFAULT) != 0 ? 1u : 0u;
   sch.dynRefill = traceDynRefill(s);
   sch.shadowOrderNow = optionSet("shadow_order") ? (int32_t)optionValue("shadow_order", -1) : s->shadowOrder.load();
   sch.twoStreamOk = rs.nextEventEstimation != 0 && rs.mediumStackSize == 0u && f.view.domeTexture == 0u && optionValue("two_stream", 1) != 0
@@ -489,10 +492,12 @@
   const uint64_t waves = (uint64_t)f.ctx.cuCount * 16u;
   chunk = (uint32_t)std::min<uint64_t>(chunk, std::max<uint64_t>(64u, ((uint64_t)U.workTotal / (waves * 16u)) & ~63ull));
   f.tm.beginIteration(true);
+  uint32_t cooked = 0u;
   f.tm.timed(f.st, StageTimers::TRACE, [&] {
     launchPath(f.st, (uint32_t)f.ctx.cuCount, s->classMask, s->classTextured != 0u, s->countTraversal, chunk, f.sch.walkCarry, f.sch.lobePark, f.sch.ringCarry,
-               f.sch.upsTraits, U, f.view, f.ps, D.dCounters.ptr, D.sampleBuf.ptr);
+               f.sch.upsTraits, f.sch.nodeCook, U, f.view, f.ps, D.dCounters.ptr, D.sampleBuf.ptr, &cooked);
   });
+  s->nodeCookLaunched = cooked;
   s->upsPlainLaunched = pathUpsVariant(s->classMask, s->classTextured != 0u, (U.flags & FLAG_NEE) != 0u, f.view.hasCutouts != 0u, s->countTraversal, f.sch.upsTraits);
   f.iters++; f.tm.totalIters++; f.traceLaunches++;
   accumulateBatch(f, batch);
diff --git a/gatling_amd/csrc/gi_traversal.h b/gatling_amd/csrc/gi_traversal.h
--- a/gatling_amd/csrc/gi_traversal.h
+++ b/gatling_amd/csrc/gi_traversal.h
@@ -1,5 +1,6 @@
 #pragma once
 
+#include "gi_node_cook.h"
 #include "gi_queues.h"
 #include "gi_texture.h"
 
@@ -38,6 +39,18 @@
   uint4* s_nodes = s_dyn + (STACK * TRACE_BLOCK * sizeof(uint2)) / sizeof(uint4);
   uint4* s_tris = s_nodes + ldsNodes * 5u;
   for (uint32_t i = threadIdx.x; i < ldsNodes * 5u; i += TRACE_BLOCK) s_nodes[i] = reinterpret_cast<const uint4*>(sc.nodes)[i];
+  for (uint32_t i = threadIdx.x; i < ldsTris * 3u; i += TRACE_BLOCK) s_tris[i] = reinterpret_cast<const uint4*>(sc.tris)[(i / 3u) * 4u + (i % 3u)];
+  __syncthreads();
+  return StagedScene{reinterpret_cast<uint2 (*)[TRACE_BLOCK]>(s_dyn), s_nodes, s_tris, ldsNodes, ldsTris};
+}
+
+template <uint32_t STACK>
+__device__ __forceinline__ StagedScene stage_scene_cooked(const SceneView& sc, uint32_t ldsNodes, uint32_t ldsTris)
+{
+  extern __shared__ uint4 s_dyn[];
+  uint4* s_nodes = s_dyn + (STACK * TRACE_BLOCK * sizeof(uint2)) / sizeof(uint4);
+  uint4* s_tris = s_nodes + cook_image_bytes(ldsNodes) / sizeof(uint4);
+  for (uint32_t i = threadIdx.x; i < ldsNodes; i += TRACE_BLOCK) cook_place(sc.nodes, i, ldsNodes, cook_oct_blocks_max(ldsNodes), reinterpret_cast<uint32_t*>(s_nodes));
   for (uint32_t i = threadIdx.x; i < ldsTris * 3u; i += TRACE_BLOCK) s_tris[i] = reinterpret_cast<const uint4*>(sc.tris)[(i / 3u) * 4u + (i % 3u)];
   __syncthreads();
   return StagedScene{reinterpret_cast<uint2 (*)[TRACE_BLOCK]>(s_dyn), s_nodes, s_tris, ldsNodes, ldsTris};
@@ -149,6 +162,51 @@
   return make_uint2(n1.y, hitmask & 0x00ffffffu);
 }
 
+#define GI_LDS __attribute__((address_space(3)))
+typedef uint32_t gi_u4 __attribute__((ext_vector_type(4)));
+
+__device__ __forceinline__ uint2 trav_node_test_cooked(RayWalk& R, const GI_LDS gi_u4* p)
+{
+  const V3 o = R.o, d = R.d;
+  constexpr float WIDEN = 1.00001f;
+  const gi_u4 n0 = p[0], n1 = p[1], n2 = p[2], n3 = p[3], n4 = p[4];
+  const GI_LDS gi_u4* table = (const GI_LDS gi_u4*)((const GI_LDS char*)p + (n1.w + ((R.octinv >> 3) & n1.z)));
+  const float sx = u2f((n0.w & 0xffu) << 23), sy = u2f(((n0.w >> 8) & 0xffu) << 23), sz = u2f(((n0.w >> 16) & 0xffu) << 23);
+  const float ax = sx * R.idx, ay = sy * R.idy, az = sz * R.idz;
+  const float bx = (u2f(n0.x) - o.x) * R.idx, by = (u2f(n0.y) - o.y) * R.idy, bz = (u2f(n0.z) - o.z) * R.idz;
+  const gi_f2 Ax = {ax, ax * WIDEN}, Ay = {ay, ay * WIDEN}, Az = {az, az * WIDEN};
+  const gi_f2 Bx = {bx, bx * WIDEN}, By = {by, by * WIDEN}, Bz = {bz, bz * WIDEN};
+  const float tFar = R.tBest * WIDEN, tNear = R.tMin;
+  const bool nxn = d.x < 0.0f, nyn = d.y < 0.0f, nzn = d.z < 0.0f;
+  const uint32_t qlox[2] = {n2.x, n2.y}, qloy[2] = {n2.z, n2.w}, qloz[2] = {n3.x, n3.y};
+  const uint32_t qhix[2] = {n3.z, n3.w}, qhiy[2] = {n4.x, n4.y}, qhiz[2] = {n4.z, n4.w};
+  const uint32_t occupied = n1.z;
+  uint32_t hitmask = 0u;
+#pragma unroll
+  for (int h = 0; h < 2; h++) {
+    if (h == 1 && !__ballot(occupied >= (5u << 16))) break;
+    const uint32_t nearx = nxn ? qhix[h] : qlox[h], farx = nxn ? qlox[h] : qhix[h];
+    const uint32_t neary = nyn ? qhiy[h] : qloy[h], fary = nyn ? qloy[h] : qhiy[h];
+    const uint32_t nearz = nzn ? qhiz[h] : qloz[h], farz = nzn ? qloz[h] : qhiz[h];
+    const gi_u4 c4 = table[h];
+    const uint32_t contribs[4] = {c4.x, c4.y, c4.z, c4.w};
+#pragma unroll
+    for (int k = 0; k < 4; k++) {
+      if (k == 2 && !__ballot(occupied >= ((uint32_t)(4 * h + 3) << 16))) break;
+      const uint32_t sh = 8u * (uint32_t)k;
+      const gi_f2 qx = {(float)((nearx >> sh) & 0xffu), (float)((farx >> sh) & 0xffu)};
+      const gi_f2 qy = {(float)((neary >> sh) & 0xffu), (float)((fary >> sh) & 0xffu)};
+      const gi_f2 qz = {(float)((nearz >> sh) & 0xffu), (float)((farz >> sh) & 0xffu)};
+      const gi_f2 tx = __builtin_elementwise_fma(qx, Ax, Bx), ty = __builtin_elementwise_fma(qy, Ay, By), tz = __builtin_elementwise_fma(qz, Az, Bz);
+      const float tn = fmaxf(fmaxf(tx.x, ty.x), fmaxf(tz.x, tNear));
+      const float tf = fminf(fminf(tx.y, ty.y), fminf(tz.y, tFar));
+      hitmask |= (tn <= tf) ? contribs[k] : 0u;
+    }
+  }
+  R.G = make_uint2(n1.x, (hitmask & 0xff000000u) | (n0.w >> 24));
+  return make_uint2(n1.y, hitmask & 0x00ffffffu);
+}
+
 __device__ __forceinline__ void node_load(const SceneView& sc, uint32_t nodeIdx, uint4& n0, uint4& n1, uint4& n2, uint4& n3, uint4& n4)
 {
   uint32_t off = nodeIdx << 4;
@@ -158,11 +216,15 @@
   n0 = p[0]; n1 = p[1]; n2 = p[2]; n3 = p[3]; n4 = p[4];
 }
 
-template <bool COUNT, uint32_t STACK, bool OVERFLOW, Staged STAGED, bool ORDERED = true>
+template <bool COUNT, uint32_t STACK, bool OVERFLOW, Staged STAGED, bool ORDERED = true, bool COOK = false>
 __device__ __forceinline__ uint2 trav_node(RayWalk& R, const SceneView& sc, StagedScene S, uint2 (&overflow)[OVERFLOW ? OVF_STACK : 1],
                                            WalkCounters<COUNT>& tc)
 {
   const uint32_t nodeIdx = trav_node_pick<STACK, OVERFLOW, ORDERED>(R, S.stack, overflow);
+  if constexpr (COOK) {
+    static_assert(STAGED == STAGED_ALL && ORDERED && !COUNT, "the cooked walk: the whole tree in LDS, near-to-far, no counters");
+    return trav_node_test_cooked(R, (const GI_LDS gi_u4*)((const GI_LDS char*)S.nodes + __umul24(nodeIdx, COOK_NODE_BYTES)));
+  }
   uint4 n0, n1, n2, n3, n4;
   if (STAGED == STAGED_ALL || (STAGED == STAGED_SOME && nodeIdx < S.ldsNodes)) { const uint4* p = S.nodes + nodeIdx * 5u; n0 = p[0]; n1 = p[1]; n2 = p[2]; n3 = p[3]; n4 = p[4]; }
   else node_load(sc, nodeIdx, n0, n1, n2, n3, n4);
@@ -233,8 +295,6 @@
   uint4 hit[64];
   uint32_t queue[128];
 };
-#define GI_LDS __attribute__((address_space(3)))
-typedef uint32_t gi_u4 __attribute__((ext_vector_type(4)));
 __device__ __forceinline__ void wt_queue_put(WaveTri& W, uint32_t i, uint32_t v) { *(volatile GI_LDS uint32_t*)&((GI_LDS WaveTri*)&W)->queue[i] = v; }
 __device__ __forceinline__ uint32_t wt_queue_get(WaveTri& W, uint32_t i) { return *(volatile GI_LDS uint32_t*)&((GI_LDS WaveTri*)&W)->queue[i]; }
 __device__ __forceinline__ void wt_best_put(WaveTri& W, uint32_t i, unsigned long long v)
@@ -370,13 +430,13 @@
   wave_tri_batch<COUNT, STAGED, CUTOUT, false, true>(W, pend, n, R, rng, sc, S, tc);
   if (COUNT) { rs.batches++; rs.pairs += n; if (n < 64u) rs.partial++; }
 }
-template <bool COUNT, uint32_t STACK, Staged STAGED, bool CUTOUT>
+template <bool COUNT, uint32_t STACK, Staged STAGED, bool CUTOUT, bool COOK = false>
 __device__ __forceinline__ bool wave_step_ring(RayTrav& R, bool alive, WaveTri& W, const SceneView& sc, StagedScene S, uint2 (&overflow)[1], WalkCounters<COUNT>& tc,
                                                uint32_t rng, uint32_t& pend, RingStats& rs)
 {
   const uint32_t lane = __lane_id();
   uint2 Gt = make_uint2(0u, 0u);
-  if (alive) Gt = trav_node<COUNT, STACK, false, STAGED>(R, sc, S, overflow, tc);
+  if (alive) Gt = trav_node<COUNT, STACK, false, STAGED, true, COOK>(R, sc, S, overflow, tc);
   const uint32_t cntL = (uint32_t)__popc(Gt.y);
   const uint32_t scan = wave_scan_inclusive(cntL);
   const uint32_t total = (uint32_t)__builtin_amdgcn_readlane((int)scan, 63);
diff --git a/include/gi_c.h b/include/gi_c.h
--- a/include/gi_c.h
+++ b/include/gi_c.h
@@ -470,6 +470,9 @@
 int giCDebugSceneLeafLift(const GiCScene* scene, uint32_t* out );
 int giCDebugLeafLift(const float* triVerts, uint32_t triCount, int32_t mode, const void* treeNodes, uint32_t treeNodeCount, uint32_t treeDepth,
                      void* outNodes, uint32_t nodeCap, uint32_t* outOrder, uint32_t* outInfo , double* outCost );
+int giCDebugSceneNodeCook(const GiCScene* scene, uint32_t* out );
+int giCDebugNodeCook(const void* nodes, uint32_t nodeCount, int32_t octBlocks, void* outImage, uint32_t imageCap, uint32_t* outInfo );
+int64_t giCDebugCheckNodeCook(const void* nodes, uint32_t nodeCount, const float* rays, uint64_t count);
 int giCDebugPathWalkStats(const GiCScene* scene, uint64_t* out );
 int giCDebugPathLobeStats(const GiCScene* scene, uint64_t* out );
 int giCDebugPathRingStats(const GiCScene* scene, uint64_t* out );
```
